# MichaelVorndran/InconsistencyMasks

Hardware: AMD Instinct MI355X
Metric: images/sec per IM generation (ensemble infer + IM build + 1 train epoch), 256x256 (higher is better)
Workload: dtype f16; 1 GPU; ISIC-2018 binary 256x256x3, 2-model IM ensemble, tiny U-Net alpha=0.5 on MI355X (configs[1]); outputs=1, unlabeled_images=2335, unlabeled_images_per_gpu=2335, labeled_images=259, n_models=2, infer_batch=584, infer_batch_rule=functions.infer_batch_size: 584 at alpha<=0.5 else 128; short tail spread, train_batch_per_gpu=32, global_batch=32, parallelism=dp1, epoch_steps=80, kept=2307, train_images=2566

## Files before the change

include/imk.h:

```cpp
#ifndef IMK_H
#define IMK_H

#include <stddef.h>
#include <stdint.h>

#ifdef __cplusplus
extern "C" {
#endif

#define IMK_VERSION 100

#define IMK_API __attribute__((visibility("default")))

enum {
    IMK_OK = 0,
    IMK_EINVAL = -1,
    IMK_EUNSUPPORTED = -2,
    IMK_EWORKSPACE = -3,
};

IMK_API int imk_version(void);
IMK_API const char *imk_error_string(int code);


IMK_API int imk_im_binary(const float *preds, int n_models, int batch, int h, int w, int kb,
                  float thr, int cmp_ge,
                  const uint8_t *img, int c, int block_in, int block_out,
                  uint8_t *img_out, uint8_t *masks_out, uint8_t *im_out,
                  int64_t *im_size, int64_t *pred_size, void *stream);

IMK_API int imk_im_multiclass(const float *probs, int n_models, int batch, int h, int w, int k,
                      const uint8_t *img, int c, int block_in, int block_out,
                      uint8_t *img_out, uint8_t *final_out, uint8_t *im_out,
                      int64_t *im_size, uint8_t *presence, void *stream);

IMK_API int imk_morph(const uint8_t *src, uint8_t *dst, int batch, int h, int w, int ksize, int op, void *stream);

IMK_API int imk_block_apply(const uint8_t *im, uint8_t *img, int c, uint8_t *masks, int n_masks,
                    int batch, int h, int w, void *stream);

enum { IMK_VOTE_HARD = 0, IMK_VOTE_SOFT = 1 };
IMK_API int imk_vote_binary(const float *preds, int n_models, int batch, int h, int w, int kb, double thr, int mode,
                    uint8_t *masks_out, void *stream);

IMK_API int imk_vote_multiclass(const float *probs, int n_models, int batch, int h, int w, int k, int mode,
                        uint8_t *final_out, void *stream);


typedef struct imk_unet_cfg {
    int h, w;
    int c_in;
    int n_out;
    int ch[5];
    int act_out;
} imk_unet_cfg;

typedef struct imk_unet_plan imk_unet_plan;

typedef struct imk_evalnet_cfg {
    int h, w;
    int ca, cb;
    int n_out;
    int two_heads;
    int normalize_a, normalize_b;
    int ch[5];
    int b_onehot;
} imk_evalnet_cfg;

IMK_API int imk_unet_plan_create(const imk_unet_cfg *cfg, imk_unet_plan **out);
IMK_API void imk_unet_plan_destroy(imk_unet_plan *plan);

IMK_API int imk_unet_param_count(const imk_unet_plan *plan, int64_t *total, int64_t *trainable);

typedef struct imk_layer_info {
    char name[16];
    int kind;
    int ksize, cin, cout;
    int64_t off_w, off_b;
    int64_t off_mean, off_var;
} imk_layer_info;
IMK_API int imk_unet_num_layers(const imk_unet_plan *plan);
IMK_API int imk_unet_layer_info(const imk_unet_plan *plan, int idx, imk_layer_info *out);

IMK_API int64_t imk_unet_packed_bytes(const imk_unet_plan *plan);
IMK_API int imk_unet_pack_weights(const imk_unet_plan *plan, const float *params, void *packed, void *stream);

IMK_API int64_t imk_unet_workspace_bytes(const imk_unet_plan *plan, int batch, int mode);

IMK_API int imk_unet_forward(const imk_unet_plan *plan, const float *params, const void *packed,
                     const uint8_t *x, int batch, float *probs, void *workspace, int64_t workspace_bytes,
                     void *stream);

IMK_API int imk_unet_tensor_info(const imk_unet_plan *plan, int batch, int mode, int layer_idx, int which,
                         int64_t *byte_offset, int *h, int *w, int *c, int *c_stride);

IMK_API int64_t imk_unet_forward_im_workspace_bytes(const imk_unet_plan *plan, int n_models, int batch, int n_streams);
IMK_API int imk_unet_forward_im(const imk_unet_plan *plan, int n_models,
                        const float *const *params, const void *const *packed,
                        const uint8_t *x, int batch, float thr, int cmp_ge,
                        const uint8_t *img, int block_in, int block_out,
                        uint8_t *img_out, uint8_t *masks_out, uint8_t *im_out,
                        int64_t *im_size, int64_t *pred_size, uint8_t *presence,
                        void *workspace, int64_t workspace_bytes, void *stream);

IMK_API int imk_unet_forward_vote(const imk_unet_plan *plan, int n_models,
                          const float *const *params, const void *const *packed,
                          const uint8_t *x, int batch, double thr, int mode, uint8_t *masks_out,
                          void *workspace, int64_t workspace_bytes, void *stream);

IMK_API int64_t imk_unet_state_bytes(const imk_unet_plan *plan);
IMK_API int imk_unet_state_init(const imk_unet_plan *plan, void *state, void *stream);
IMK_API int imk_unet_fwd_bwd(const imk_unet_plan *plan, float *params, void *packed, void *state,
                     const uint8_t *x, const uint8_t *y, int batch, int loss_kind,
                     float *grads, float *stats, void *workspace, int64_t workspace_bytes, void *stream);

IMK_API int imk_unet_adamw_step(const imk_unet_plan *plan, float *params, void *packed, void *state,
                        const float *grads, const float *stats, float grad_scale,
                        float lr, float wd, float beta1, float beta2, float eps, void *stream);

IMK_API int64_t imk_unet_consistency_workspace_bytes(const imk_unet_plan *plan, int batch);
IMK_API int imk_unet_consistency_fwd_bwd(const imk_unet_plan *plan, float *params, void *packed, void *state,
                                 const uint8_t *x1, const uint8_t *x2, int batch,
                                 float *grads, float *stats, void *workspace, int64_t workspace_bytes, void *stream);

typedef struct imk_aug_params {
    int flip_v, flip_h;
    int rot;
    int bright_on;
    float alpha, beta;
    int blur_k;
    int noise_max;
    uint32_t seed;
} imk_aug_params;

IMK_API int imk_gather_pairs(const uint8_t *img, int64_t row_img, const uint8_t *mask, int planes, int64_t hw, int div255,
                             const uint8_t *mul, const int64_t *idx, int64_t n, uint8_t *img_out, uint8_t *mask_out,
                             void *stream);

IMK_API int imk_augment(const uint8_t *img, const uint8_t *mask, int batch, int h, int w, int c, int cm,
                const imk_aug_params *params, uint8_t *img_out, uint8_t *mask_out, int any_quarter_turn, void *stream);

#define IMK_VIEWS_MAX 16
typedef struct imk_view_params {
    int op;
    int blur_k;
    int noise_max;
    uint32_t seed;
    int bright_on;
    float alpha, beta;
} imk_view_params;

IMK_API int imk_views(const uint8_t *img, int batch, int h, int w, int c, int n_views, const imk_view_params *params,
                      int chain, int any_quarter_turn, uint8_t *views_out, void *stream);

IMK_API int imk_vote_views_binary(const float *preds, int n_views, int batch, int h, int w, int k, const int *ops,
                                  int any_quarter_turn, double thr, int cmp_ge, uint8_t *masks_out, void *stream);

IMK_API int imk_vote_views_majority(const float *probs, int n_views, int batch, int h, int w, int k, uint8_t *final_out,
                                    void *stream);

enum { IMK_VOTE_MAJORITY = 2 };
IMK_API int64_t imk_unet_forward_views_vote_workspace_bytes(const imk_unet_plan *plan, int n_views, int batch);
IMK_API int imk_unet_forward_views_vote(const imk_unet_plan *plan, const float *params, const void *packed,
                                        const uint8_t *views, int n_views, int batch, const int *ops, int any_quarter_turn,
                                        double thr, int mode, int cmp_ge, uint8_t *masks_out, void *workspace,
                                        int64_t workspace_bytes, void *stream);

IMK_API int64_t imk_unet_forward_student_workspace_bytes(const imk_unet_plan *plan, int batch);
IMK_API int imk_unet_forward_student(const imk_unet_plan *plan, const float *params, const void *packed, const uint8_t *x,
                                     const uint8_t *img, int batch, float thr, int cmp_ge, const imk_aug_params *aug,
                                     int any_quarter_turn, uint8_t *img_out, uint8_t *labels_out, void *workspace,
                                     int64_t workspace_bytes, void *stream);

IMK_API int imk_eval_binary(const float *probs, float thr, int cmp_ge, const uint8_t *gt, int batch, int h, int w,
                    uint8_t *pred_out, int64_t *counts, void *stream);

IMK_API int imk_eval_multiclass(const float *probs, const uint8_t *gt, int batch, int h, int w, int k, uint8_t *pred_out,
                        int64_t *counts, void *stream);

IMK_API int64_t imk_eval_soft_out_doubles(int k);
IMK_API int imk_eval_soft_sums(const float *probs, const uint8_t *gt, int64_t n_pix, int k, int mode, double *out, void *stream);

IMK_API int64_t imk_im_depth_workspace_bytes(int batch, int h, int w);
IMK_API int imk_im_depth(const float *preds, int n_models, int batch, int h, int w, float mult, const uint8_t *img, int c,
                         int block_in, uint8_t *img_out, uint8_t *im_out, int64_t *im_size, float *thr_out, float *std_out,
                         void *workspace, int64_t workspace_bytes, void *stream);

IMK_API int64_t imk_unet_forward_im_depth_workspace_bytes(const imk_unet_plan *plan, int n_models, int batch, int n_streams);
IMK_API int imk_unet_forward_im_depth(const imk_unet_plan *plan, int n_models, const float *const *params,
                                      const void *const *packed, const uint8_t *x, int batch, float mult, const uint8_t *img,
                                      int block_in, uint8_t *img_out, uint8_t *im_out, int64_t *im_size, float *thr_out,
                                      float *std_out, void *workspace, int64_t workspace_bytes, void *stream);

IMK_API int imk_eval_depth(const float *probs, const uint8_t *gt, int batch, int h, int w, uint8_t *pred_out, double *sums,
                           void *stream);

IMK_API int imk_evalnet_plan_create(const imk_evalnet_cfg *cfg, imk_unet_plan **out);
IMK_API int64_t imk_evalnet_workspace_bytes(const imk_unet_plan *plan, int batch, int mode );

IMK_API int imk_evalnet_forward(const imk_unet_plan *plan, const float *params, const void *packed, const uint8_t *xa,
                        const uint8_t *xb, int batch, float *out, void *workspace, int64_t workspace_bytes, void *stream);

IMK_API int imk_evalnet_fwd_bwd(const imk_unet_plan *plan, float *params, void *packed, void *state, const uint8_t *xa,
                        const uint8_t *xb, const float *y, int batch, float *out, float *grads, float *stats,
                        void *workspace, int64_t workspace_bytes, void *stream);

IMK_API int imk_evalnet_tensor_info(const imk_unet_plan *plan, int batch, int mode, int layer_idx, int which,
                            int64_t *byte_offset, int *h, int *w, int *c, int *c_stride);

#define IMK_SELECT_MAX_CAND 16
#define IMK_SELECT_MAX_MODELS 8
enum { IMK_SELECT_IOU = 0, IMK_SELECT_MIOU = 1, IMK_SELECT_CONF_GATED = 2 };

IMK_API int imk_evalnet_select(const float *scores, int n_models, int batch, int n_cand, int n_heads, int n_out,
                               const int32_t *counts, const uint8_t *cand, int64_t cand_bytes, double thr, int mode,
                               int32_t *best_idx, float *best_score, uint8_t *keep, uint8_t *out, void *stream);

IMK_API int64_t imk_evalnet_forward_candidates_workspace_bytes(const imk_unet_plan *plan, int batch, int n_cand);
IMK_API int imk_evalnet_forward_candidates(const imk_unet_plan *plan, int n_models, const float *const *params,
                                           const void *const *packed, const uint8_t *xa, const uint8_t *xb, int batch, int n_cand,
                                           float *scores, void *workspace, int64_t workspace_bytes, void *stream);

IMK_API int imk_evalnet_forward_select(const imk_unet_plan *plan, int n_models, const float *const *params,
                                       const void *const *packed, const uint8_t *xa, const uint8_t *xb, int batch, int n_cand,
                                       const int32_t *counts, const uint8_t *cand, int64_t cand_bytes, double thr, int mode,
                                       float *scores, int32_t *best_idx, float *best_score, uint8_t *keep, uint8_t *out,
                                       void *workspace, int64_t workspace_bytes, void *stream);

IMK_API int imk_unet_plan_set_bn_momentum(imk_unet_plan *plan, float momentum);
IMK_API int imk_unet_plan_get_bn_momentum(const imk_unet_plan *plan, float *momentum);

IMK_API int imk_unet_plan_debug(imk_unet_plan *plan, int materialize, int single_stream);

IMK_API int imk_png_info(const char *path, int *h, int *w, int *color_type, int *bit_depth);
IMK_API int imk_png_read_file(const char *path, int want_c, uint8_t *out, int64_t out_cap, int *h_out, int *w_out);
IMK_API int imk_png_decode(const uint8_t *data, int64_t len, int want_c, uint8_t *out, int64_t out_cap, int *h_out, int *w_out);
IMK_API int imk_png_encode(const uint8_t *pixels, int h, int w, int c, int level, uint8_t *out, int64_t out_cap, int64_t *out_len);
IMK_API int imk_png_write_file(const char *path, const uint8_t *pixels, int h, int w, int c, int level);
// ... 42 lines not shown
```

inconsistencymasks_amd/_lib.py:

```python
import ctypes
import os

PKG = os.path.dirname(os.path.abspath(__file__))
LIB_PATH = os.environ.get("IMK_LIB_PATH", os.path.join(PKG, "libimk.so"))

c_int, c_float, c_void_p, c_int64 = ctypes.c_int, ctypes.c_float, ctypes.c_void_p, ctypes.c_int64


class UnetCfg(ctypes.Structure):
    _fields_ = [("h", c_int), ("w", c_int), ("c_in", c_int), ("n_out", c_int),
                ("ch", c_int * 5), ("act_out", c_int)]


class EvalnetCfg(ctypes.Structure):
    _fields_ = [("h", c_int), ("w", c_int), ("ca", c_int), ("cb", c_int), ("n_out", c_int), ("two_heads", c_int),
                ("normalize_a", c_int), ("normalize_b", c_int), ("ch", c_int * 5), ("b_onehot", c_int)]


class AugParams(ctypes.Structure):
    _fields_ = [("flip_v", c_int), ("flip_h", c_int), ("rot", c_int), ("bright_on", c_int), ("alpha", c_float),
                ("beta", c_float), ("blur_k", c_int), ("noise_max", c_int), ("seed", ctypes.c_uint32)]


class ViewParams(ctypes.Structure):
    _fields_ = [("op", c_int), ("blur_k", c_int), ("noise_max", c_int), ("seed", ctypes.c_uint32), ("bright_on", c_int),
                ("alpha", c_float), ("beta", c_float)]


class PrepItem(ctypes.Structure):
    _fields_ = [("src_off", c_int64), ("src_h", c_int), ("src_w", c_int), ("x0", c_int), ("y0", c_int), ("cw", c_int),
                ("ch", c_int), ("scale_x", ctypes.c_double), ("scale_y", ctypes.c_double)]


class LayerInfo(ctypes.Structure):
    _fields_ = [("name", ctypes.c_char * 16), ("kind", c_int), ("ksize", c_int), ("cin", c_int), ("cout", c_int),
                ("off_w", c_int64), ("off_b", c_int64), ("off_mean", c_int64), ("off_var", c_int64)]


SIGNATURES = {
    "imk_version": (c_int, []),
    "imk_error_string": (ctypes.c_char_p, [c_int]),
    "imk_im_binary": (c_int, [c_void_p, c_int, c_int, c_int, c_int, c_int, c_float, c_int,
                              c_void_p, c_int, c_int, c_int, c_void_p, c_void_p, c_void_p,
                              c_void_p, c_void_p, c_void_p]),
    "imk_im_multiclass": (c_int, [c_void_p, c_int, c_int, c_int, c_int, c_int,
                                  c_void_p, c_int, c_int, c_int, c_void_p, c_void_p, c_void_p,
                                  c_void_p, c_void_p, c_void_p]),
    "imk_morph": (c_int, [c_void_p, c_void_p, c_int, c_int, c_int, c_int, c_int, c_void_p]),
    "imk_block_apply": (c_int, [c_void_p, c_void_p, c_int, c_void_p, c_int, c_int, c_int, c_int, c_void_p]),
    "imk_unet_plan_create": (c_int, [ctypes.POINTER(UnetCfg), ctypes.POINTER(c_void_p)]),
    "imk_unet_plan_destroy": (None, [c_void_p]),
    "imk_unet_param_count": (c_int, [c_void_p, ctypes.POINTER(c_int64), ctypes.POINTER(c_int64)]),
    "imk_unet_num_layers": (c_int, [c_void_p]),
    "imk_unet_layer_info": (c_int, [c_void_p, c_int, ctypes.POINTER(LayerInfo)]),
    "imk_unet_packed_bytes": (c_int64, [c_void_p]),
    "imk_unet_pack_weights": (c_int, [c_void_p, c_void_p, c_void_p, c_void_p]),
    "imk_unet_workspace_bytes": (c_int64, [c_void_p, c_int, c_int]),
    "imk_unet_forward": (c_int, [c_void_p, c_void_p, c_void_p, c_void_p, c_int, c_void_p, c_void_p, c_int64, c_void_p]),
    "imk_unet_tensor_info": (c_int, [c_void_p, c_int, c_int, c_int, c_int, ctypes.POINTER(c_int64),
                                     ctypes.POINTER(c_int), ctypes.POINTER(c_int), ctypes.POINTER(c_int),
                                     ctypes.POINTER(c_int)]),
    "imk_unet_forward_im_workspace_bytes": (c_int64, [c_void_p, c_int, c_int, c_int]),
    "imk_unet_forward_im": (c_int, [c_void_p, c_int, ctypes.POINTER(c_void_p), ctypes.POINTER(c_void_p),
                                    c_void_p, c_int, c_float, c_int, c_void_p, c_int, c_int,
                                    c_void_p, c_void_p, c_void_p, c_void_p, c_void_p, c_void_p,
                                    c_void_p, c_int64, c_void_p]),
    "imk_vote_binary": (c_int, [c_void_p, c_int, c_int, c_int, c_int, c_int, ctypes.c_double, c_int, c_void_p, c_void_p]),
    "imk_vote_multiclass": (c_int, [c_void_p, c_int, c_int, c_int, c_int, c_int, c_int, c_void_p, c_void_p]),
    "imk_unet_forward_vote": (c_int, [c_void_p, c_int, ctypes.POINTER(c_void_p), ctypes.POINTER(c_void_p),
                                      c_void_p, c_int, ctypes.c_double, c_int, c_void_p, c_void_p, c_int64, c_void_p]),
    "imk_views": (c_int, [c_void_p, c_int, c_int, c_int, c_int, c_int, c_void_p, c_int, c_int, c_void_p, c_void_p]),
    "imk_vote_views_binary": (c_int, [c_void_p, c_int, c_int, c_int, c_int, c_int, c_void_p, c_int, ctypes.c_double, c_int,
                                      c_void_p, c_void_p]),
    "imk_vote_views_majority": (c_int, [c_void_p, c_int, c_int, c_int, c_int, c_int, c_void_p, c_void_p]),
    "imk_unet_forward_views_vote_workspace_bytes": (c_int64, [c_void_p, c_int, c_int]),
    "imk_unet_forward_views_vote": (c_int, [c_void_p, c_void_p, c_void_p, c_void_p, c_int, c_int, c_void_p, c_int,
                                            ctypes.c_double, c_int, c_int, c_void_p, c_void_p, c_int64, c_void_p]),
    "imk_unet_forward_student_workspace_bytes": (c_int64, [c_void_p, c_int]),
    "imk_unet_forward_student": (c_int, [c_void_p, c_void_p, c_void_p, c_void_p, c_void_p, c_int, c_float, c_int, c_void_p, c_int,
                                         c_void_p, c_void_p, c_void_p, c_int64, c_void_p]),
    "imk_unet_state_bytes": (c_int64, [c_void_p]),
    "imk_unet_state_init": (c_int, [c_void_p, c_void_p, c_void_p]),
    "imk_unet_fwd_bwd": (c_int, [c_void_p, c_void_p, c_void_p, c_void_p, c_void_p, c_void_p, c_int, c_int,
                                 c_void_p, c_void_p, c_void_p, c_int64, c_void_p]),
    "imk_unet_consistency_workspace_bytes": (c_int64, [c_void_p, c_int]),
    "imk_unet_consistency_fwd_bwd": (c_int, [c_void_p, c_void_p, c_void_p, c_void_p, c_void_p, c_void_p, c_int,
                                             c_void_p, c_void_p, c_void_p, c_int64, c_void_p]),
    "imk_evalnet_plan_create": (c_int, [ctypes.POINTER(EvalnetCfg), ctypes.POINTER(c_void_p)]),
    "imk_evalnet_workspace_bytes": (c_int64, [c_void_p, c_int, c_int]),
    "imk_evalnet_forward": (c_int, [c_void_p, c_void_p, c_void_p, c_void_p, c_void_p, c_int, c_void_p, c_void_p, c_int64,
                                    c_void_p]),
    "imk_evalnet_tensor_info": (c_int, [c_void_p, c_int, c_int, c_int, c_int, ctypes.POINTER(c_int64),
                                        ctypes.POINTER(c_int), ctypes.POINTER(c_int), ctypes.POINTER(c_int),
                                        ctypes.POINTER(c_int)]),
    "imk_evalnet_fwd_bwd": (c_int, [c_void_p, c_void_p, c_void_p, c_void_p, c_void_p, c_void_p, c_void_p, c_int, c_void_p,
                                    c_void_p, c_void_p, c_void_p, c_int64, c_void_p]),
    "imk_evalnet_select": (c_int, [c_void_p, c_int, c_int, c_int, c_int, c_int, c_void_p, c_void_p, c_int64, ctypes.c_double, c_int,
                                   c_void_p, c_void_p, c_void_p, c_void_p, c_void_p]),
    "imk_evalnet_forward_candidates_workspace_bytes": (c_int64, [c_void_p, c_int, c_int]),
    "imk_evalnet_forward_candidates": (c_int, [c_void_p, c_int, ctypes.POINTER(c_void_p), ctypes.POINTER(c_void_p), c_void_p, c_void_p,
                                               c_int, c_int, c_void_p, c_void_p, c_int64, c_void_p]),
    "imk_evalnet_forward_select": (c_int, [c_void_p, c_int, ctypes.POINTER(c_void_p), ctypes.POINTER(c_void_p), c_void_p, c_void_p,
                                           c_int, c_int, c_void_p, c_void_p, c_int64, ctypes.c_double, c_int, c_void_p, c_void_p,
                                           c_void_p, c_void_p, c_void_p, c_void_p, c_int64, c_void_p]),
    "imk_gather_pairs": (c_int, [c_void_p, c_int64, c_void_p, c_int, c_int64, c_int, c_void_p, c_void_p, c_int64, c_void_p, c_void_p, c_void_p]),
    "imk_augment": (c_int, [c_void_p, c_void_p, c_int, c_int, c_int, c_int, c_int, c_void_p, c_void_p, c_void_p, c_int, c_void_p]),
    "imk_eval_binary": (c_int, [c_void_p, c_float, c_int, c_void_p, c_int, c_int, c_int, c_void_p, c_void_p, c_void_p]),
    "imk_eval_multiclass": (c_int, [c_void_p, c_void_p, c_int, c_int, c_int, c_int, c_void_p, c_void_p, c_void_p]),
    "imk_eval_soft_out_doubles": (c_int64, [c_int]),
    "imk_eval_soft_sums": (c_int, [c_void_p, c_void_p, c_int64, c_int, c_int, c_void_p, c_void_p]),
    "imk_im_depth_workspace_bytes": (c_int64, [c_int, c_int, c_int]),
    "imk_im_depth": (c_int, [c_void_p, c_int, c_int, c_int, c_int, c_float, c_void_p, c_int, c_int, c_void_p, c_void_p, c_void_p,
                             c_void_p, c_void_p, c_void_p, c_int64, c_void_p]),
    "imk_unet_forward_im_depth_workspace_bytes": (c_int64, [c_void_p, c_int, c_int, c_int]),
    "imk_unet_forward_im_depth": (c_int, [c_void_p, c_int, ctypes.POINTER(c_void_p), ctypes.POINTER(c_void_p), c_void_p, c_int, c_float,
                                          c_void_p, c_int, c_void_p, c_void_p, c_void_p, c_void_p, c_void_p, c_void_p, c_int64, c_void_p]),
    "imk_eval_depth": (c_int, [c_void_p, c_void_p, c_int, c_int, c_int, c_void_p, c_void_p, c_void_p]),
    "imk_unet_plan_debug": (c_int, [c_void_p, c_int, c_int]),
    "imk_unet_plan_set_bn_momentum": (c_int, [c_void_p, c_float]),
    "imk_unet_plan_get_bn_momentum": (c_int, [c_void_p, ctypes.POINTER(c_float)]),
    "imk_prof_create": (c_int, [c_int, ctypes.POINTER(c_void_p)]),
    "imk_prof_destroy": (None, [c_void_p]),
    "imk_prof_bind": (c_int, [c_void_p]),
    "imk_prof_unbind": (c_int, [c_void_p]),
    "imk_prof_totals_enable": (c_int, [c_void_p, c_int]),
    "imk_prof_totals_dump": (c_int64, [c_void_p, ctypes.c_char_p, c_int64]),
    "imk_prof_mark": (c_int, [c_int, c_void_p]),
    "imk_runtime_warnings": (c_int, []),
    "imk_unet_plan_side_stream": (c_int, [c_void_p, c_int, ctypes.POINTER(c_void_p)]),
    "imk_prof_set_period": (c_int, [c_void_p, c_int]),
    "imk_prof_collect": (c_int, [c_void_p, ctypes.POINTER(c_int64), ctypes.POINTER(ctypes.c_double), ctypes.POINTER(ctypes.c_double),
                                 ctypes.POINTER(ctypes.c_double)]),
    "imk_png_info": (c_int, [ctypes.c_char_p, ctypes.POINTER(c_int), ctypes.POINTER(c_int), ctypes.POINTER(c_int), ctypes.POINTER(c_int)]),
    "imk_png_read_file": (c_int, [ctypes.c_char_p, c_int, c_void_p, c_int64, ctypes.POINTER(c_int), ctypes.POINTER(c_int)]),
    "imk_png_decode": (c_int, [c_void_p, c_int64, c_int, c_void_p, c_int64, ctypes.POINTER(c_int), ctypes.POINTER(c_int)]),
    "imk_png_encode": (c_int, [c_void_p, c_int, c_int, c_int, c_int, c_void_p, c_int64, ctypes.POINTER(c_int64)]),
    "imk_png_write_file": (c_int, [ctypes.c_char_p, c_void_p, c_int, c_int, c_int, c_int]),
    "imk_pos_contours": (c_int, [c_void_p, c_int, c_int, c_int, c_void_p, c_int]),
    "imk_mod_pos_size": (c_int, [c_void_p, c_int, c_int, c_int, c_int, c_int, c_int, c_void_p]),
    "imk_cell_count": (c_int, [c_void_p, c_int, c_void_p, c_void_p, c_int, c_int, c_int, c_void_p]),
    "imk_prep_resize": (c_int, [c_void_p, c_int64, c_void_p, c_int, c_int, c_int, c_int, c_int, c_int, c_void_p, c_void_p]),
    "imk_prep_crops": (c_int, [c_void_p, c_int, c_int, c_int, c_void_p, c_int, c_int, c_int, c_int, c_void_p, c_int, c_void_p,
                               c_void_p]),
    "imk_unet_adamw_step": (c_int, [c_void_p, c_void_p, c_void_p, c_void_p, c_void_p, c_void_p, c_float,
                                    c_float, c_float, c_float, c_float, c_float, c_void_p]),
}


def _load():
    if not os.path.exists(LIB_PATH):
        raise RuntimeError(
            f"{LIB_PATH} is missing: build it with `python -c 'import __graft_entry__ as g; g.build()'` "
            "(hipcc --offload-arch=gfx950).  There is no CPU fallback for the product path.")
    import torch
    lib = ctypes.CDLL(LIB_PATH)
    for name, (res, args) in SIGNATURES.items():
        fn = getattr(lib, name)
        fn.restype = res
        fn.argtypes = args
    return lib


lib = _load()


class ImkError(RuntimeError):
    pass


def check(code, what=""):
    if code != 0:
        msg = lib.imk_error_string(code)
        raise ImkError(f"{what}: imk error {code} ({msg.decode() if msg else '?'})")
```

inconsistencymasks_amd/csrc/imk_conv.hip:

```cpp
#include <cstdlib>
#include "imk_kernels.h"
#include "imk_elem.h"

#include "imk_stage.h"
#include "imk_switches.h"

#ifndef IMK_INF_WAVES
#define IMK_INF_WAVES 4
#endif
IMK_STAMP_TABLE(conv)
IMK_WGSTAMP_TABLE(conv)

namespace {


struct ImkConvGeom { int tiles_x, tiles_y, mt_total, nc8, nc8p, n_pass, ps, nsp; unsigned magic_tx, magic_pi; };
__host__ __device__ inline size_t imk_chain_w2_offset(size_t stage1_bytes, size_t out_bytes) {
    return ((stage1_bytes > out_bytes ? stage1_bytes : out_bytes) + 15) & ~(size_t)15;
}

template <int TH, int MT, int LM, bool CHAIN = false>
__device__ __forceinline__ void conv_mfma_body(const ImkConvArgs &a, const ImkConvGeom &gm, int bx, int by) {
    const int tiles_x = gm.tiles_x, tiles_y = gm.tiles_y, mt_total = gm.mt_total, nc8 = gm.nc8, nc8p = gm.nc8p;
    const int n_pass = gm.n_pass, ps = gm.ps, nsp = gm.nsp;
// ... 1288 lines not shown
    for (int j = 0; j < 8; ++j) { bsum[j] = 0.f; acc[0][j] = acc[1][j] = acc[2][j] = acc[3][j] = 0.f; }
    const float inv = 1.0f / u8_div;
    const long long stride = (long long)gridDim.x * 256;
    struct Px { f16x8 d, zz; uint32_t xb; };
    auto load = [&](long long p, Px &q) {
        q.d = *reinterpret_cast<const f16x8 *>(dy + p * 8);
        q.zz = *reinterpret_cast<const f16x8 *>(z + p * 8);
        typedef uint32_t __attribute__((aligned(1))) u32_unaligned;
        const long long rem = (n_pix - p) * cin;
        const int back = rem >= 4 ? 0 : (int)(4 - rem);
        const uint32_t v = *reinterpret_cast<const u32_unaligned *>(x + p * cin - back) >> (8 * back);
        q.xb = cin >= 4 ? v : (v & ((1u << (8 * cin)) - 1u));
    };
    auto use = [&](const Px &q) {
        float xf[4];
#pragma unroll
        for (int c = 0; c < 4; ++c) xf[c] = (float)(f16)((float)((q.xb >> (8 * c)) & 0xffu) * inv);
#pragma unroll
        for (int j = 0; j < 8; ++j) {
            const float zf = (float)q.zz[j];
            const float g = zf > 0.f ? (float)(f16)(A[j] * (float)q.d[j] + Bc[j] * zf + Cc[j]) : 0.f;
            bsum[j] += g;
#pragma unroll
            for (int c = 0; c < 4; ++c) acc[c][j] += xf[c] * g;
        }
    };
    long long p = (long long)blockIdx.x * 256 + t;
    if (p < n_pix) {
        Px cur, nxt;
        load(p, cur);
        while (true) {
            const long long pn = p + stride;
            const bool more = pn < n_pix;
            load(more ? pn : p, nxt);
            use(cur);
            if (!more) break;
            cur = nxt;
            p = pn;
        }
    }
#pragma unroll
    for (int c = 0; c < 4; ++c)
#pragma unroll
        for (int j = 0; j < 8; ++j) {
            const float v = wave_sum<64>(acc[c][j]);
            if (lane == 0) s_red[wave][c * 8 + j] = v;
        }
#pragma unroll
    for (int j = 0; j < 8; ++j) {
        const float v = wave_sum<64>(bsum[j]);
        if (lane == 0) s_red[wave][32 + j] = v;
    }
    __syncthreads();
    auto tot = [&](int i) { return (s_red[0][i] + s_red[1][i]) + (s_red[2][i] + s_red[3][i]); };
    float *row = partial + (size_t)blockIdx.x * 2 * 256;
    const int r = t >> 6, l = t & 63, ci = 4 * (l >> 4) + r, co = l & 15;
    row[t] = (ci < 4 && co < 8) ? tot(ci * 8 + co) : 0.f;
    row[256 + t] = t < 8 ? tot(32 + t) : 0.f;
}

__device__ __forceinline__ int wgf_find_job(const ImkWgFinalJobs &jobs, int idx, bool stage1) {
    int j = 0;
    for (int k = 1; k < jobs.n; ++k) {
        const int begin = stage1 ? jobs.j[k].work1_begin : jobs.j[k].tile_begin;
        if (idx >= begin) j = k;
    }
    return j;
}

__global__ __launch_bounds__(256) void wgf_stage1_kernel(ImkWgFinalJobs jobs) {
    IMK_STAMP_BEGIN(conv, 21);
    __shared__ float4 s_q[4][64];
    const int jn = wgf_find_job(jobs, blockIdx.x, true);
    const ImkWgFinalJob &jb = jobs.j[jn];
    const int local = blockIdx.x - jb.work1_begin;
    const int tile = local / jb.n_chunks, chunk = local - tile * jb.n_chunks;
    const int t = threadIdx.x, e4 = t & 63, sg = t >> 6;
    const int s0 = chunk * jb.chunk, s1 = min(jb.n_split, s0 + jb.chunk);
    const size_t stride4 = (size_t)jb.n_tiles * 64;
    const float4 *p = reinterpret_cast<const float4 *>(jb.partial) + (size_t)tile * 64 + e4;
    float4 acc = {0.f, 0.f, 0.f, 0.f};
    for (int sb = s0; sb < s1; sb += WG_RED_CHUNK) {
        float4 v[WG_RED_CHUNK / 4];
#pragma unroll
        for (int i = 0; i < WG_RED_CHUNK / 4; ++i) v[i] = p[(size_t)min(sb + sg + 4 * i, s1 - 1) * stride4];
#pragma unroll
        for (int i = 0; i < WG_RED_CHUNK / 4; ++i) {
            const float live = (sb + sg + 4 * i < s1) ? 1.f : 0.f;
            acc.x += live * v[i].x; acc.y += live * v[i].y; acc.z += live * v[i].z; acc.w += live * v[i].w;
        }
    }
    s_q[sg][e4] = acc;
    __syncthreads();
    if (sg == 0) {
        const float4 a = s_q[0][e4], b = s_q[1][e4], c = s_q[2][e4], d = s_q[3][e4];
        float4 r;
        r.x = (a.x + b.x) + (c.x + d.x); r.y = (a.y + b.y) + (c.y + d.y); r.z = (a.z + b.z) + (c.z + d.z); r.w = (a.w + b.w) + (c.w + d.w);
        reinterpret_cast<float4 *>(jb.red)[((size_t)chunk * jb.n_tiles + tile) * 64 + e4] = r;
    }
    IMK_STAMP_END(1);
}

template <int N>
__device__ __forceinline__ float wgf_sum_chunks(const float *p, size_t stride, int sg, int n_chunks) {
    float v[N];
#pragma unroll
    for (int i = 0; i < N; ++i) v[i] = p[(size_t)min(sg + 4 * i, n_chunks - 1) * stride];
    float acc = 0.f;
#pragma unroll
    for (int i = 0; i < N; ++i) acc += (sg + 4 * i < n_chunks) ? v[i] : 0.f;
    return acc;
}

__global__ __launch_bounds__(1024) void wgf_stage2_kernel(ImkWgFinalJobs jobs, const float *__restrict__ inv_scale_ptr,
                                                          float *__restrict__ found_inf) {
    __shared__ float s_p[4][256];
    const int jn = wgf_find_job(jobs, blockIdx.x, false);
    const ImkWgFinalJob &jb = jobs.j[jn];
    const int tile = blockIdx.x - jb.tile_begin;
    const int e = threadIdx.x & 255, sg = threadIdx.x >> 8;
    const size_t stride = (size_t)jb.n_tiles * 256;
    const float *p = jb.red + (size_t)tile * 256 + e;
    const int per = (jb.n_chunks + 3) >> 2;
    float acc;
    if (per <= 1) acc = wgf_sum_chunks<1>(p, stride, sg, jb.n_chunks);
    else if (per <= 2) acc = wgf_sum_chunks<2>(p, stride, sg, jb.n_chunks);
    else if (per <= 4) acc = wgf_sum_chunks<4>(p, stride, sg, jb.n_chunks);
    else if (per <= 8) acc = wgf_sum_chunks<8>(p, stride, sg, jb.n_chunks);
    else acc = wgf_sum_chunks<16>(p, stride, sg, jb.n_chunks);
    s_p[sg][e] = acc;
    __syncthreads();
    if (sg != 0) return;
    float s = ((s_p[0][e] + s_p[1][e]) + (s_p[2][e] + s_p[3][e])) * *inv_scale_ptr;
    const int pair = tile / (jb.T + 1), tap = tile - pair * (jb.T + 1);
    const int cit = pair / jb.cot_n, cot = pair - cit * jb.cot_n;
    const int r = e >> 6, lane = e & 63;
    const int m = 4 * (lane >> 4) + r, nn = lane & 15;
    const int ci = cit * 16 + m, co = cot * 16 + nn;
    if (tap < jb.T) {
        if (ci < jb.cin && co < jb.cout) {
            if (!isfinite(s)) *found_inf = 1.0f;
            jb.dw[((size_t)tap * jb.cin + ci) * jb.cout + co] = s;
        }
    } else if (cit == 0 && m == 0 && co < jb.cout) {
        if (!isfinite(s)) *found_inf = 1.0f;
        jb.db[co] = s;
    }
}

__global__ __launch_bounds__(256) void pack_conv_batched_kernel(ImkPackJobs jobs) {
    IMK_STAMP_BEGIN(conv, 23);
    if (jobs.ctl && blockIdx.x == 0 && blockIdx.y == 0 && threadIdx.x == 0) imk_ctl_end_step(jobs.ctl, jobs.stats);
    const ImkPackJob &jb = jobs.j[blockIdx.y];
    if (jb.transposed == 2) {
        for (int i = blockIdx.x * 256 + threadIdx.x; i < 512; i += gridDim.x * 256) {
            const int j = i & 7, lane = (i >> 3) & 63;
            const int m = lane & 15, g = lane >> 4;
            float v = 0.f;
            if (!jb.pair) {
                const int ci = 4 * g + j;
                if (j < 4 && ci < jb.cin && m < jb.cout) v = jb.w[(size_t)ci * jb.cout + m];
            } else {
                const int ci = 4 * (g & 1) + j, co = m & 7;
                if (j < 4 && (m >> 3) == (g >> 1) && ci < jb.cin && co < jb.cout) v = jb.w[(size_t)ci * jb.cout + co];
            }
            jb.dst[i] = (f16)v;
        }
        return;
    }
    const int T = jb.ksize == 3 ? 9 : 1;
    const int m_dim = jb.transposed ? jb.cin : jb.cout, k_dim = jb.transposed ? jb.cout : jb.cin;
    if (jb.pair && T == 9) {
        const int nc8 = ((k_dim + 7) & ~7) / 8;
        const int ns = 3 * nc8;
        for (int i = blockIdx.x * 256 + threadIdx.x; i < ns * 512; i += gridDim.x * 256) {
            const int j = i & 7, lane = (i >> 3) & 63, st = i >> 9;
            const int m = lane & 15, g = lane >> 4;
            const int q = 4 * st + g;
            const int ut = q / nc8, c8 = q - ut * nc8;
            const int r = ut / 3, c = ut - 3 * r, ky = r - (m >> 3);
            const int mi = m & 7, ki = c8 * 8 + j;
            float v = 0.f;
            if (ky >= 0 && ky <= 2 && mi < m_dim && ki < k_dim) {
                const int tap = ky * 3 + c;
                if (!jb.transposed) v = jb.w[((size_t)tap * jb.cin + ki) * jb.cout + mi];
                else v = jb.w[((size_t)(T - 1 - tap) * jb.cin + mi) * jb.cout + ki];
            }
            jb.dst[i] = (f16)v;
        }
        return;
    }
    if (jb.pair) {
        const int nc8 = ((k_dim + 7) & ~7) / 8;
        const int nq = T * nc8, ns = (nq + 1) / 2;
        for (int i = blockIdx.x * 256 + threadIdx.x; i < ns * 512; i += gridDim.x * 256) {
            const int j = i & 7, lane = (i >> 3) & 63, st = i >> 9;
            const int m = lane & 15, g = lane >> 4;
            const int q = 2 * st + (g & 1);
            const int tap = q / nc8, c8 = q - tap * nc8;
            const int mi = m & 7, ki = c8 * 8 + j;
            float v = 0.f;
            if (q < nq && (m >> 3) == (g >> 1) && mi < m_dim && ki < k_dim) {
                if (!jb.transposed) v = jb.w[((size_t)tap * jb.cin + ki) * jb.cout + mi];
                else v = jb.w[((size_t)(T - 1 - tap) * jb.cin + mi) * jb.cout + ki];
            }
            jb.dst[i] = (f16)v;
        }
        return;
    }
    const int nc8 = ((k_dim + 7) & ~7) / 8;
    const int nc8p = imk_pass_chunks(nc8), nsp = (T * nc8p + 3) / 4;
    const int ns = imk_cdiv_d(nc8, nc8p) * nsp;
    const int total = ((m_dim + 15) / 16) * ns * 512;
    for (int i = blockIdx.x * 256 + threadIdx.x; i < total; i += gridDim.x * 256) {
        const int j = i & 7, lane = (i >> 3) & 63;
        const int cs = i >> 9;
        const int s = cs % ns, ct = cs / ns;
        const int m = lane & 15, g = lane >> 4;
        const int pass = s / nsp, q = 4 * (s - pass * nsp) + g;
        const int tap = q / nc8p, c8 = pass * nc8p + (q - tap * nc8p);
        const int mi = ct * 16 + m, ki = c8 < nc8 ? c8 * 8 + j : k_dim;
        float v = 0.f;
        if (tap < T && mi < m_dim && ki < k_dim) {
            if (!jb.transposed) v = jb.w[((size_t)tap * jb.cin + ki) * jb.cout + mi];
            else v = jb.w[((size_t)(T - 1 - tap) * jb.cin + mi) * jb.cout + ki];
        }
        jb.dst[i] = (f16)v;
    }
    IMK_STAMP_END(1);
}

}

int imk_wgf_add_job(ImkWgFinalJobs &jobs, float *partial, int n_split, int ksize, int cin, int cout, float *dw, float *db) {
    if (jobs.n >= IMK_WGF_MAX_JOBS) return IMK_EUNSUPPORTED;
    const int T = ksize == 3 ? 9 : 1;
    const int cit_n = (imk_pad8(cin) + 15) / 16, cot_n = (imk_pad8(cout) + 15) / 16;
    ImkWgFinalJob &jb = jobs.j[jobs.n++];
    jb.partial = partial;
    jb.n_split = n_split;
    jb.chunk = WG_RED_CHUNK;
    while (imk_cdiv(n_split, jb.chunk) > 64) jb.chunk *= 2;
    jb.n_chunks = imk_cdiv(n_split, jb.chunk);
    jb.n_tiles = cit_n * cot_n * (T + 1);
    jb.red = partial + (size_t)n_split * jb.n_tiles * 256;
    jb.T = T; jb.cin = cin; jb.cout = cout; jb.cot_n = cot_n;
    jb.dw = dw; jb.db = db;
    jb.work1_begin = jobs.total_work1;
    jb.tile_begin = jobs.total_tiles;
    jobs.total_work1 += jb.n_tiles * jb.n_chunks;
    jobs.total_tiles += jb.n_tiles;
    return IMK_OK;
}

int imk_launch_wgrad_finalize_jobs(const ImkWgFinalJobs &jobs, const float *inv_scale_ptr, float *found_inf, hipStream_t stream) {
    if (jobs.n <= 0) return IMK_OK;
    double wgf_bytes = 0;
    for (int i = 0; i < jobs.n; ++i)
        wgf_bytes += ((double)jobs.j[i].n_split + 2.0 * jobs.j[i].n_chunks + 1.0) * jobs.j[i].n_tiles * 256 * 4;
    ImkProfScope prof(PF_WGF, wgf_bytes, stream);
    double b1 = 0, b2 = 0;
    for (int i = 0; i < jobs.n; ++i) {
        b1 += ((double)jobs.j[i].n_split + jobs.j[i].n_chunks) * jobs.j[i].n_tiles * 256 * 4;
        b2 += ((double)jobs.j[i].n_chunks + 1.0) * jobs.j[i].n_tiles * 256 * 4;
    }
    imk_prof_work(b1);
    imk_klaunch(wgf_stage1_kernel, dim3(jobs.total_work1), dim3(256), 0, stream, jobs);
    IMK_LAUNCH_CHECK();
    imk_prof_work(b2);
    imk_klaunch(wgf_stage2_kernel, dim3(jobs.total_tiles), dim3(1024), 0, stream, jobs, inv_scale_ptr, found_inf);
    IMK_LAUNCH_CHECK();
    return IMK_OK;
}

int imk_launch_pack_jobs(const ImkPackJobs &jobs, hipStream_t stream) {
    if (jobs.n <= 0) return IMK_OK;
    double pk_bytes = 0;
    for (int i = 0; i < jobs.n; ++i) pk_bytes += (double)jobs.j[i].ksize * jobs.j[i].ksize * jobs.j[i].cin * jobs.j[i].cout * 6;
    ImkProfScope prof(PF_STEP_TAIL, pk_bytes, stream);
    long long widest = 0;
    for (int i = 0; i < jobs.n; ++i) {
        const long long slots = (long long)jobs.j[i].ksize * jobs.j[i].ksize * ((jobs.j[i].cin + 15) & ~15) * ((jobs.j[i].cout + 15) & ~15);
        widest = slots > widest ? slots : widest;
    }
    int bpj = (int)((widest + 2047) / 2048);
    bpj = bpj < 64 ? 64 : (bpj > 1024 ? 1024 : bpj);
    imk_klaunch(pack_conv_batched_kernel, dim3(dim3(bpj, jobs.n)), dim3(256), 0, stream, jobs);
    IMK_LAUNCH_CHECK();
    return IMK_OK;
}

static inline int odd_ps(int nc8) { return imk_lds_pitch(nc8); }

static inline int conv_tile_h(int cs_in, int ksize) {
    const int halo = ksize == 3 ? 1 : 0;
    const size_t b16 = (size_t)(16 + 2 * halo) * (TW + 2 * halo) * odd_ps(imk_pass_chunks(cs_in / 8)) * 16;
    return b16 > 64 * 1024 ? 8 : 16;
}

int imk_conv_num_tiles(int B, int H, int W, int cs_in, int ksize) {
    const int per_tile = B * imk_cdiv(H, conv_tile_h(cs_in, ksize)) * imk_cdiv(W, TW);
    const int gemm = imk_conv_gemm_num_tiles(B, H, W);
    return per_tile > gemm ? per_tile : gemm;
}

#include <algorithm>
#include <cstdio>
#include <cstring>
#include <cxxabi.h>
#include <map>
#include <mutex>
#include <new>
#include <string>
#include <unordered_map>
#include <vector>
namespace {
struct ProfRec { hipEvent_t e0, e1; int variant; double bytes, flops; };
struct ProfTot { long long launches = 0; double bytes = 0, flops = 0; };
const char *const kFamilyNames[PF_COUNT] = {
    "conv_mfma_kernel<16, 1>", "conv_mfma_kernel<16, 2>", "conv_mfma_kernel<16, 4>", "conv_mfma_kernel<8, 1>", "conv_mfma_kernel<8, 2>",
    "conv_mfma_kernel<8, 4>", "conv_pipe_kernel", "wgrad_mfma_kernel", "bn_bwd_prep_kernel", "bn_bwd_coef_kernel", "bn_finalize_kernel",
    "wgf_stage1+2_kernel", "head_kernel", "head_loss_kernel", "step_tail", "im_kernel", "conv_gemm_kernel", "wgrad_gemm_kernel"};
__global__ void imk_mark_kernel(int id) { (void)id; }
}
struct imk_prof {
    int period = 0;
    long counter = 0;
    std::vector<ProfRec> recs;
    std::vector<hipEvent_t> pool;
    bool totals_on = false;
    std::map<std::string, ProfTot> totals;
    hipEvent_t event() {
        if (!pool.empty()) { hipEvent_t e = pool.back(); pool.pop_back(); return e; }
        hipEvent_t e;
        (void)hipEventCreate(&e);
        return e;
    }
};
static thread_local imk_prof *t_prof = nullptr;

extern "C" int imk_prof_create(int period, imk_prof **out) {
    IMK_CHECK_ARG(out && period >= 0);
    imk_prof *p = new (std::nothrow) imk_prof();
    if (!p) return IMK_EINVAL;
    p->period = period;
    *out = p;
    return IMK_OK;
}
extern "C" void imk_prof_destroy(imk_prof *p) {
    if (!p) return;
    if (t_prof == p) { t_prof = nullptr; imk_tls_totals_on = false; }
    for (auto &r : p->recs) { (void)hipEventDestroy(r.e0); (void)hipEventDestroy(r.e1); }
    for (auto e : p->pool) (void)hipEventDestroy(e);
    delete p;
}
extern "C" int imk_prof_bind(imk_prof *p) { t_prof = p; imk_tls_totals_on = p && p->totals_on; return IMK_OK; }
extern "C" int imk_prof_unbind(imk_prof *p) { if (p && t_prof == p) { t_prof = nullptr; imk_tls_totals_on = false; return 1; } return 0; }
extern "C" int imk_prof_set_period(imk_prof *p, int period) { IMK_CHECK_ARG(p && period >= 0); p->period = period; return IMK_OK; }

static const std::string &kernel_short_name(const void *kern, hipStream_t stream) {
    static std::mutex mu;
    static std::unordered_map<const void *, std::string> names;
    std::lock_guard<std::mutex> lk(mu);
    auto it = names.find(kern);
    if (it != names.end()) return it->second;
    std::string n = "?";
    if (const char *m = hipKernelNameRefByPtr(kern, stream)) {
        int st = 0;
        char *d = abi::__cxa_demangle(m, nullptr, nullptr, &st);
        n = (st == 0 && d) ? d : m;
        free(d);
        if (st != 0) {
            const char *tag = "_ZN12_GLOBAL__N_1";
            const size_t at = n.find(tag);
            if (at != std::string::npos) {
                size_t i = at + strlen(tag), len = 0;
                while (i < n.size() && n[i] >= '0' && n[i] <= '9') len = 10 * len + (size_t)(n[i++] - '0');
                if (len > 0 && i + len <= n.size()) n = n.substr(i, len);
            }
        }
        for (const char *drop : {"void ", "(anonymous namespace)::"})
            for (size_t at; (at = n.find(drop)) != std::string::npos;) n.erase(at, strlen(drop));
        int depth = 0;
        for (size_t i = 0; i < n.size(); ++i) {
            if (n[i] == '<') ++depth;
            else if (n[i] == '>') --depth;
            else if (n[i] == '(' && depth == 0) { n.resize(i); break; }
        }
        if (n.size() > 90) n.resize(90);
    }
    return names.emplace(kern, n).first->second;
}
static thread_local struct { double bytes, flops; bool armed; } t_work = {0.0, 0.0, false};
void imk_prof_work(double bytes, double flops) { t_work.bytes = bytes; t_work.flops = flops; t_work.armed = true; }
void imk_prof_note_launch(const void *kern, hipStream_t stream) {
    imk_prof *p = t_prof;
    if (!p || !p->totals_on) return;
    ProfTot &t = p->totals[kernel_short_name(kern, stream)];
    t.launches += 1;
    if (t_work.armed) { t.bytes += t_work.bytes; t.flops += t_work.flops; t_work.armed = false; }
}

int imk_prof_begin(int family, double bytes, hipStream_t stream, double flops, const char *variant) {
    imk_prof *p = t_prof;
    (void)variant;
    if (p && p->totals_on && family >= 0 && family < PF_COUNT) imk_prof_work(bytes, flops);
    if (!p || p->period <= 0 || (p->counter++ % p->period) != 0) return -1;
    ProfRec pr{p->event(), p->event(), family, bytes, flops};
    if (hipEventRecord(pr.e0, stream) != hipSuccess) { p->pool.push_back(pr.e0); p->pool.push_back(pr.e1); return -1; }
    p->recs.push_back(pr);
    return (int)p->recs.size() - 1;
}
void imk_prof_end(int slot, hipStream_t stream) {
    imk_prof *p = t_prof;
    if (p && slot >= 0 && slot < (int)p->recs.size()) (void)hipEventRecord(p->recs[slot].e1, stream);
}

extern "C" int imk_prof_totals_enable(imk_prof *p, int on) {
    IMK_CHECK_ARG(p);
    p->totals.clear();
    p->totals_on = on != 0;
    if (t_prof == p) imk_tls_totals_on = p->totals_on;
    t_work.armed = false;
    return IMK_OK;
}
// ... 381 lines not shown
    if ((sw.gemm_over_chain == 2 || (sw.gemm_over_chain == 1 && store_mid)) && imk_conv_gemm_ok(plain)) return false;
    if (pipe_choice(a).ok || a.epi != EP_RELU || a.ksize != 3 || a.cout > 64 || cout2 > 64) return false;
    if (a.x.lmode != LM_POOL && a.x.lmode != LM_AFFINE) return false;
    const bool wide = a.x.cs_in <= 32 && a.cout <= 32 && a.x.lmode != LM_POOL;
    const bool wide_chain = sw.wide_chain_train && wide && a.x.lmode == LM_AFFINE && a.x.cs_in >= 16 && cout2 <= a.cout && pipe_fits(a);
    if (sw.conv_chain_tile == 1 && wide && store_mid && !wide_chain && (long long)a.B * imk_cdiv(a.H, 16) * imk_cdiv(a.W, TW) > 2048)
        return false;
    const int mt1 = (a.cout + 15) / 16, mt2 = (cout2 + 15) / 16, mt = (mt1 <= 2 && mt2 <= 2) ? 2 : 4;
    return mt1 <= mt && mt2 <= mt && conv_tile_h(a.x.cs_in, 3) == 16;
}

bool imk_conv_can_fuse_wgrad(const ImkConvArgs &a) {
    const PipeChoice p = pipe_choice(a);
    if (!p.ok || a.wpk2) return false;
    const bool form1 = a.ksize == 1 && a.x.lmode == LM_BNBWD && a.epi == EP_MASK && a.mask && !(a.dystat_z && a.stats_partial);
    const bool form2 = a.x.lmode == LM_RAW && a.epi == EP_PLAIN && a.dystat_z && a.stats_partial;
    if (!form1 && !form2) return false;
    const bool all_ch = p.pair ? a.cs_out == 8 : a.cs_out == 16;
    return (a.H % 16 == 0) && (a.W % TW == 0) && all_ch;
}
int imk_conv_fused_wgrad_rows_max() { return 256 * 8; }

bool imk_conv_can_sum2(const ImkConvArgs &a) {
    const PipeChoice p = pipe_choice(a);
    if (!p.ok || a.wpk2 || a.wg_partial) return false;
    if (a.ksize != 1 || a.x.lmode != LM_BNBWD || a.epi != EP_PLAIN || (a.dystat_z && a.stats_partial)) return false;
    const bool all_ch = p.pair ? a.cs_out == 8 : a.cs_out == 16;
    return (a.H % 16 == 0) && (a.W % TW == 0) && all_ch;
}

int imk_launch_conv(const ImkConvArgs &a_in, hipStream_t stream) {
    ImkConvArgs a = a_in;
    IMK_CHECK_ARG(a.x.in && a.wpk && (a.out || a.wpk2) && a.B > 0 && a.H > 0 && a.W > 0);
    IMK_CHECK_ARG(a.ksize == 1 || a.ksize == 3);
    IMK_CHECK_ARG(a.x.cs_in % 8 == 0 && a.cs_out % 8 == 0 && a.x.cs_in >= a.x.cin && a.cs_out >= a.cout);
    IMK_CHECK_ARG(a.x.lmode != LM_U8 || (a.x.cs_in == 8 && a.x.cin <= 8));
    if (a.x.cs_in > 512) return IMK_EUNSUPPORTED;
    const PipeChoice p = pipe_choice(a);
    a.pair = p.pair;
    if (a.pre_wpk && !(p.ok && a.wpk2 && a.pre_bias && a.pre_sc && a.pre_sh && a.pre_cout > 0)) return IMK_EUNSUPPORTED;
    if (a.wpk2 && a.pair && a.cout2 > 8) return IMK_EUNSUPPORTED;
    if (a.wpk2) {
        if (a.epi != EP_RELU || !a.out2 || !a.bias2 || a.cs_out2 % 8) return IMK_EUNSUPPORTED;
        if (p.ok) return a.cout2 > 16 ? IMK_EUNSUPPORTED : launch_conv_pipe_any(a, stream);
        if (!imk_conv_can_chain_tile(a, a.cout2, a.out != nullptr)) return IMK_EUNSUPPORTED;
        if (conv_wide_chain_ok(a)) return launch_conv_wide_chain(a, stream);
        if (imk_conv_gemm_chain_ok(a)) return imk_launch_conv_gemm(a, stream);
        return launch_conv_mfma(a, stream);
    }
    if (p.ok) return launch_conv_pipe_any(a, stream);
    if (a.x.lmode == LM_STEM) return IMK_EUNSUPPORTED;
    if (conv_wide_ok(a)) return launch_conv_wide_any(a, stream);
    if (imk_conv_gemm_ok(a)) return imk_launch_conv_gemm(a, stream);
    return launch_conv_mfma(a, stream);
}

int imk_wgrad_splits(int B, int H, int W, int cin, int cout) {
    const int n_tiles = B * imk_cdiv(H, 16) * imk_cdiv(W, TW);
    const int n_pairs = ((imk_pad8(cin) + 15) / 16) * ((imk_pad8(cout) + 15) / 16);
    constexpr int target = 768;
    int s = target / n_pairs;
    if (s < 1) s = 1;
    if (s > n_tiles) s = n_tiles;
    return s;
}

size_t imk_wgrad_partial_floats(int B, int H, int W, int ksize, int cin, int cout) {
    const int n_pairs = ((imk_pad8(cin) + 15) / 16) * ((imk_pad8(cout) + 15) / 16);
    const int T = ksize == 3 ? 9 : 1;
    size_t ns = (size_t)imk_wgrad_splits(B, H, W, cin, cout);
    if (imk_pad8(cin) <= 16 && imk_pad8(cout) <= 16 && ns < (size_t)imk_conv_fused_wgrad_rows_max())
        ns = (size_t)imk_conv_fused_wgrad_rows_max();
    if (imk_wgrad_gemm_wide(imk_pad8(cin), imk_pad8(cout), (long long)B * H * W)) {
        for (int lm : {(int)LM_RAW, (int)LM_POOL, (int)LM_AFFINE}) {
            const size_t ng = (size_t)imk_wgrad_gemm_splits(lm, B, H, W, ksize, imk_pad8(cin), imk_pad8(cout));
            if (ns < ng) ns = ng;
        }
    }
    if (ksize == 1 && imk_pad8(cin) >= 24 && imk_pad8(cin) <= 64 && imk_pad8(cout) >= 24 && imk_pad8(cout) <= 64 &&
        ns < (size_t)imk_bwd1x1_rows((long long)B * H * W, imk_pad8(cin), imk_pad8(cout)))
        ns = (size_t)imk_bwd1x1_rows((long long)B * H * W, imk_pad8(cin), imk_pad8(cout));
    if (ksize == 1 && n_pairs <= 8 && ns < (size_t)imk_loss_blocks((long long)B * H * W)) ns = (size_t)imk_loss_blocks((long long)B * H * W);
    return (ns + (ns + WG_RED_CHUNK - 1) / WG_RED_CHUNK) * n_pairs * (T + 1) * 256;
}

struct WgradLaunch { ImkWgradGeom gm; int gx, gy; size_t lds; };

static int plan_wgrad(const ImkWgradArgs &a, WgradLaunch &L) {
    IMK_CHECK_ARG(a.x.in && a.dA && a.partial && a.B > 0 && a.H > 0 && a.W > 0 && a.n_split > 0);
    IMK_CHECK_ARG(a.ksize == 1 || a.ksize == 3);
    IMK_CHECK_ARG(a.x.cs_in % 8 == 0 && a.cs_out % 8 == 0);
    if (a.x.lmode == LM_BNBWD) return IMK_EUNSUPPORTED;
    if (a.x.lmode == LM_U8 && a.x.cin > 4) return IMK_EUNSUPPORTED;
    const int cit_n = (a.x.cs_in + 15) / 16, cot_n = (a.cs_out + 15) / 16;
    const int tiles_x = imk_cdiv(a.W, TW), tiles_y = imk_cdiv(a.H, 16);
    size_t lds = ((size_t)18 * 18 + 256) * WG_STRIDE_H * sizeof(f16) + (4 * (size_t)a.x.cs_in + 3 * (size_t)a.cs_out) * sizeof(float);
    const size_t red = 4 * (size_t)(a.ksize == 3 ? 10 : 2) * 256 * sizeof(float);
    if (lds < red) lds = red;
    L.gm = ImkWgradGeom{tiles_x, tiles_y, a.B * tiles_x * tiles_y, cit_n, cot_n, a.x.cs_in / 8, a.cs_out / 8, ImkWalk{}};
    L.gx = a.n_split; L.gy = cit_n * cot_n; L.lds = lds;
    {
        int g = a.n_split;
        L.gm.wk = imk_walk_make(g, L.gm.n_tiles, tiles_x * tiles_y);
        if (g != a.n_split) { g = a.n_split; L.gm.wk = ImkWalk{L.gm.n_tiles, 0, g, 0, 0}; }
    }
    return IMK_OK;
}

static double wgrad_algorithmic_bytes(const ImkWgradArgs &a, const WgradLaunch &L) {
    const double px = (double)a.B * a.H * a.W;
    double in_b;
    switch (a.x.lmode) {
        case LM_POOL: in_b = 4.0 * px * a.x.cs_in * 2; break;
        case LM_UPADD: in_b = 1.25 * px * a.x.cs_in * 2; break;
        case LM_U8: in_b = px * a.x.cin; break;
        default: in_b = px * a.x.cs_in * 2;
    }
    const int T = a.ksize == 3 ? 9 : 1;
    return in_b + px * a.cs_out * 2 * (a.dA_z ? 2 : 1) + (double)L.gx * L.gy * (T + 1) * 256 * 4;
}

int imk_launch_wgrad(const ImkWgradArgs &a, hipStream_t stream) {
    if (a.x.lmode == LM_U8 && a.ksize == 1 && a.dA_z && a.dA_coef && a.cs_out == 8 && a.x.cin <= 4 && a.n_split >= 1) {
        const long long n_pix = (long long)a.B * a.H * a.W;
        ImkProfScope prof(PF_WGRAD, (double)n_pix * (a.x.cin + 32) + (double)a.n_split * 2 * 1024, stream, imk_wgrad_flops(a));
        imk_klaunch(stem_wgrad_kernel, dim3(a.n_split), dim3(256), 0, stream, reinterpret_cast<const uint8_t *>(a.x.in), a.x.cin, a.x.u8_div, a.dA, a.dA_z, a.dA_coef,
                                                        n_pix, a.partial);
        IMK_LAUNCH_CHECK();
        return IMK_OK;
    }
    if (imk_wgrad_gemm_ok(a.x.lmode, a.dA_z != nullptr, a.ksize, a.x.cs_in, a.cs_out, (long long)a.B * a.H * a.W)) return imk_launch_wgrad_gemm(a, stream);
    WgradLaunch L{};
    int rc = plan_wgrad(a, L);
    if (rc) return rc;
    const dim3 grid(L.gx, L.gy);
    ImkProfScope prof(PF_WGRAD, wgrad_algorithmic_bytes(a, L), stream, imk_wgrad_flops(a));
    switch (a.x.lmode) {
#define IMK_WG(LM) do { if (a.ksize == 3) { if (a.dA_z) imk_klaunch(wgrad_mfma_kernel<LM, true, true>, dim3(grid), dim3(256), L.lds, stream, a, L.gm); \
                                           else imk_klaunch(wgrad_mfma_kernel<LM, false, true>, dim3(grid), dim3(256), L.lds, stream, a, L.gm); } \
                        else { if (a.dA_z) imk_klaunch(wgrad_mfma_kernel<LM, true, false>, dim3(grid), dim3(256), L.lds, stream, a, L.gm); \
                               else imk_klaunch(wgrad_mfma_kernel<LM, false, false>, dim3(grid), dim3(256), L.lds, stream, a, L.gm); } } while (0)
        case LM_RAW: IMK_WG(LM_RAW); break;
        case LM_AFFINE: IMK_WG(LM_AFFINE); break;
        case LM_POOL: IMK_WG(LM_POOL); break;
        case LM_UPADD: IMK_WG(LM_UPADD); break;
        default: IMK_WG(LM_U8); break;
#undef IMK_WG
    }
    IMK_LAUNCH_CHECK();
    return IMK_OK;
}

size_t imk_packed_conv_halfs(int ksize, int cin, int cout, int transposed, bool pair) {
    if (transposed == 2) return 512;
    const int T = ksize == 3 ? 9 : 1;
    const int m_dim = transposed ? cin : cout, k_dim = transposed ? cout : cin;
    const int nc8 = imk_pad8(k_dim) / 8;
    if (pair) return (size_t)(T == 9 ? 3 * nc8 : (nc8 + 1) / 2) * 512;
    const int nc8p = imk_pass_chunks(nc8);
    const int ns = imk_cdiv_d(nc8, nc8p) * ((T * nc8p + 3) / 4);
    return (size_t)((m_dim + 15) / 16) * ns * 512;
}
```

inconsistencymasks_amd/csrc/imk_elem.h:

```cpp
#pragma once
#include "imk_common.h"

struct ImkCtl {
    float loss_scale;
    float inv_loss_scale;
    int good_steps;
    int step;
    float found_inf;
    float pad[3];
};

int imk_launch_bn_finalize(const float *partial, int n_part, int c, int cs, double count, const float *gamma,
                           const float *beta, float *mov_mean, float *mov_var, float *scale, float *shift,
                           float *save_mean, float *save_invstd, hipStream_t stream, float momentum = 0.99f);
int imk_bn_prep_blocks(int B, int H, int W, int cs);
int imk_launch_bn_bwd_prep(int mode, const f16 *g_direct, const f16 *g_other, const f16 *z, const float *sc,
                           const float *sh, f16 *dy_out, float *partial, int B, int H, int W, int cs, hipStream_t stream,
                           int g_other_cs = 0);
int imk_launch_bn_bwd_coef(const float *partial, int n_part, int c, int cs, double count, const float *gamma,
                           const float *save_mean, const float *save_invstd, const float *inv_scale_ptr, float *coef,
                           float *dgamma, float *dbeta, float *found_inf, hipStream_t stream);
int imk_launch_head(const f16 *z, const float *sc, const float *sh, const float *w, const float *bias, int cin, int cs,
                    int K, int softmax, long long n_pix, float *probs, hipStream_t stream);
int imk_loss_blocks(long long n_pix);
int imk_launch_head_loss(const f16 *z, const float *sc, const float *sh, const float *w, const float *bias, int cin, int cs,
                         int K, int softmax, long long n_pix, const uint8_t *y, const ImkCtl *ctl, float *stats,
                         f16 *dlogit, float *loss_partial, hipStream_t stream, int y255 = 0);
bool imk_head_cce_fused_ok(int cs, int K, long long n_pix, int rows_cap);
int imk_head_cce_fused_rows(long long n_pix);
int imk_launch_head_cce_fused(const f16 *z, const float *sc, const float *sh, const float *w, const float *bias, int cin, int cs,
                              int K, long long n_pix, const uint8_t *y, const ImkCtl *ctl, float *stats, f16 *dy,
                              float *loss_partial, float *dystat_partial, float *wg_partial, hipStream_t stream);
bool imk_head_mse_fused_ok(int cs, int K, long long n_pix, int rows_cap);
int imk_launch_head_mse_fused(const f16 *z, const float *sc, const float *sh, const float *w, const float *bias, int cin, int cs,
                              int K, long long n_pix, const uint8_t *y, const ImkCtl *ctl, float *stats, f16 *dy,
                              float *loss_partial, float *dystat_partial, float *wg_partial, hipStream_t stream, int y255 = 0);
int imk_launch_rmse_scale(const float *loss_partial, long long n_pix, int K, float *grads, long long n_grads, float *stats,
                          hipStream_t stream);
int imk_launch_loss_finalize(const float *loss_partial, long long n_pix, int K, int kind, float *stats, hipStream_t stream);
bool imk_consistency_fused_ok(int cs, int K, int softmax, long long n_pix, int rows_cap);
int imk_launch_consistency_head(const f16 *zA, const f16 *zB, const float *scA, const float *shA, const float *scB,
                                const float *shB, const float *w, const float *bias, int cin, int cs, int K, long long n_pix,
                                const ImkCtl *ctl, float *stats, f16 *dyA, f16 *dyB, float *loss_partial, float *dystatA,
                                float *dystatB, float *wg_partial, hipStream_t stream);
int imk_launch_consistency_dlogit(const float *pA, const float *pB, int K, int softmax, long long n_pix, const ImkCtl *ctl,
                                  float *stats, f16 *dlogitA, f16 *dlogitB, float *loss_partial, hipStream_t stream);
int imk_launch_grad_add(float *g, const float *g2, long long n, float *found_inf, hipStream_t stream);
int imk_launch_ctl_init(ImkCtl *ctl, hipStream_t stream);
int imk_launch_adamw(float *p, float *m, float *v, const float *g, long long n, ImkCtl *ctl, const float *stats,
                     float grad_scale, float lr, float wd, float b1, float b2, float eps, hipStream_t stream);

int imk_launch_concat_pool(const f16 *za, const float *sca, const float *sha, int csa, const f16 *zb, const float *scb,
                           const float *shb, int csb, int B, int Hh, int Wh, f16 *cat, hipStream_t stream, int a_div = 1);
int imk_launch_onehot(const uint8_t *cls, long long n_pix, int cs, f16 *out, hipStream_t stream);
size_t imk_evalnet_head_partial_floats(int B, int n_heads, int K, int C);
int imk_launch_evalnet_head(const f16 *z, const float *sc, const float *sh, const float *const *w, const float *const *bias,
                            int n_heads, int K, int C, int cs, int B, int H, int W, float *out, const float *y,
                            const ImkCtl *ctl, float *stats, f16 *dP, float *partial, hipStream_t stream);
int imk_launch_evalnet_head_reduce(const float *partial, int B, int n_heads, int K, int C, const float *inv_scale_ptr,
                                   float *dw0, float *db0, float *dw1, float *db1, float *found_inf, float *stats,
                                   hipStream_t stream);

__device__ __forceinline__ void imk_ctl_end_step(ImkCtl *ctl, const float *stats) {
    if (stats[1] != 0.f) {
        ctl->loss_scale = fmaxf(ctl->loss_scale * 0.5f, 1.0f);
        ctl->good_steps = 0;
    } else {
        ctl->step += 1;
        if (++ctl->good_steps >= 2000) { ctl->loss_scale *= 2.0f; ctl->good_steps = 0; }
    }
    ctl->inv_loss_scale = 1.0f / ctl->loss_scale;
}

#define IMK_FOLD_MAX_JOBS 32
struct ImkFoldJob { const float *gamma, *beta, *mean, *var; float *scale; int c, cs; };
struct ImkFoldJobs { ImkFoldJob j[IMK_FOLD_MAX_JOBS]; int n; };
int imk_launch_bn_fold_jobs(const ImkFoldJobs &jobs, hipStream_t stream);
```

inconsistencymasks_amd/csrc/imk_elem.hip:

```cpp
#include "imk_elem.h"
#include "imk_head.h"

IMK_STAMP_TABLE(elem)

namespace {

constexpr float BN_EPS = 1e-3f;

__device__ __forceinline__ void block_sum_rows(const float *__restrict__ partial, int n_part, int cs, int ch, int t,
                                               double &o1, double &o2) {
    double s1 = 0.0, s2 = 0.0;
    for (int i0 = t; i0 < n_part; i0 += 8 * 256) {
        float v1[8], v2[8];
#pragma unroll
        for (int u = 0; u < 8; ++u) {
            const int i = min(i0 + u * 256, n_part - 1);
            v1[u] = partial[(size_t)i * 2 * cs + ch];
            v2[u] = partial[(size_t)i * 2 * cs + cs + ch];
        }
#pragma unroll
        for (int u = 0; u < 8; ++u) {
            const double live = (i0 + u * 256 < n_part) ? 1.0 : 0.0;
            s1 += live * (double)v1[u];
            s2 += live * (double)v2[u];
// ... 303 lines not shown
    head_stage<CS>(w, bias, sc, sh, cin, K, s_w);
    __syncthreads();
    const long long p0 = (long long)blockIdx.x * 256;
    const long long p = p0 + threadIdx.x;
    float *row = s_out + threadIdx.x * pitch;
    if (p < n_pix) {
        float xin[CS];
        head_input<CS>(z, p, s_w, K, xin);
        if (!softmax) {
            for (int k = 0; k < K; ++k) row[k] = head_sigmoid(head_logit<CS>(xin, s_w, K, k));
        } else {
            head_softmax_row<CS>(xin, s_w, K, row);
        }
    }
    __syncthreads();
    const long long n_here = (n_pix - p0 < 256 ? n_pix - p0 : 256) * K;
    float *dst = probs + p0 * K;
    for (long long i = threadIdx.x; i < n_here; i += 256) {
        const int px = (int)(i / K), k = (int)(i - (long long)px * K);
        dst[i] = s_out[px * pitch + k];
    }
}

template <int CS, bool Y255 = false>
__global__ __launch_bounds__(256) void head_loss_kernel(const f16 *__restrict__ z, const float *__restrict__ sc,
                                                        const float *__restrict__ sh, const float *__restrict__ w,
                                                        const float *__restrict__ bias, int cin, int K, int softmax,
                                                        long long n_pix, const uint8_t *__restrict__ y,
                                                        const ImkCtl *__restrict__ ctl, float *__restrict__ stats,
                                                        int cs_out, f16 *__restrict__ dlogit,
                                                        float *__restrict__ loss_partial) {
    extern __shared__ float s_w[];
    float *s_b = s_w + K * CS, *s_sc = s_b + K, *s_sh = s_sc + CS, *s_rows = s_sh + CS;
    for (int i = threadIdx.x; i < K * CS; i += 256) {
        const int k = i / CS, c = i - k * CS;
        s_w[i] = (c < cin) ? w[(size_t)c * K + k] : 0.f;
    }
    for (int i = threadIdx.x; i < K; i += 256) s_b[i] = bias[i];
    for (int i = threadIdx.x; i < CS; i += 256) { s_sc[i] = sc[i]; s_sh[i] = sh[i]; }
    __syncthreads();
    const float S = ctl->loss_scale;
    if (blockIdx.x == 0 && threadIdx.x == 0) { stats[1] = 0.f; stats[2] = S; stats[3] = (float)ctl->step; }
    float l = 0.f;
    for (long long p = (long long)blockIdx.x * 256 + threadIdx.x; p < n_pix; p += (long long)gridDim.x * 256) {
        float xin[CS];
#pragma unroll
        for (int q = 0; q < CS / 8; ++q) {
            const f16x8 v = *reinterpret_cast<const f16x8 *>(z + p * CS + q * 8);
#pragma unroll
            for (int j = 0; j < 8; j += 2) {
                const f16x2 r2 = imk_affine2(f16x2{v[j], v[j + 1]}, f32x2{s_sc[q * 8 + j], s_sc[q * 8 + j + 1]}, f32x2{s_sh[q * 8 + j], s_sh[q * 8 + j + 1]});
                xin[q * 8 + j] = (float)r2[0]; xin[q * 8 + j + 1] = (float)r2[1];
            }
        }
        auto logit = [&](int k) {
            float acc = s_b[k];
#pragma unroll
            for (int c = 0; c < CS; ++c) acc += xin[c] * s_w[k * CS + c];
            return acc;
        };
        f16 *d = dlogit + p * cs_out;
        if (!softmax) {
            const float inv_n = 1.0f / ((float)n_pix * (float)K);
            for (int k0 = 0; k0 < cs_out; k0 += 8) {
                f16x8 g8 = {0, 0, 0, 0, 0, 0, 0, 0};
#pragma unroll
                for (int j = 0; j < 8; ++j) {
                    const int k = k0 + j;
                    if (k < K) {
                        float t = (float)y[p * K + k];
                        if constexpr (Y255) t = t / 255.0f;
                        const float pk = 1.0f / (1.0f + expf(-logit(k)));
                        const float e = pk - t;
                        l += e * e;
                        g8[j] = (f16)(S * 2.0f * e * inv_n * pk * (1.0f - pk));
                    }
                }
                *reinterpret_cast<f16x8 *>(d + k0) = g8;
            }
        } else {
            float *row = s_rows + threadIdx.x * (K | 1);
            float mx = -INFINITY;
            for (int k = 0; k < K; ++k) { const float lg = logit(k); row[k] = lg; mx = fmaxf(mx, lg); }
            float sum = 0.f;
            for (int k = 0; k < K; ++k) { const float e = expf(row[k] - mx); row[k] = e; sum += e; }
            const float inv = 1.0f / sum;
            const int t = y[p];
            const float inv_n = 1.0f / (float)n_pix;
            for (int k0 = 0; k0 < cs_out; k0 += 8) {
                f16x8 g8 = {0, 0, 0, 0, 0, 0, 0, 0};
#pragma unroll
                for (int j = 0; j < 8; ++j) {
                    const int k = k0 + j;
                    if (k < K) {
                        const float pk = row[k] * inv;
                        if (k == t) l += -logf(fmaxf(pk, 1.17549435e-38f));
                        g8[j] = (f16)(S * (pk - (k == t ? 1.0f : 0.0f)) * inv_n);
                    }
                }
                *reinterpret_cast<f16x8 *>(d + k0) = g8;
            }
        }
    }
    __shared__ float s_l[4];
    l = wave_sum<64>(l);
    if ((threadIdx.x & 63) == 0) s_l[threadIdx.x >> 6] = l;
    __syncthreads();
    if (threadIdx.x == 0) loss_partial[blockIdx.x] = (s_l[0] + s_l[1]) + (s_l[2] + s_l[3]);
}

__device__ __forceinline__ double loss_partials_sum(const float *__restrict__ partial, int n) {
    __shared__ double r[256];
    double s = 0;
    for (int i0 = threadIdx.x; i0 < n; i0 += 8 * 256) {
        float v[8];
#pragma unroll
        for (int u = 0; u < 8; ++u) v[u] = (i0 + u * 256 < n) ? partial[i0 + u * 256] : 0.f;
#pragma unroll
        for (int u = 0; u < 8; ++u) s += (double)v[u];
    }
    r[threadIdx.x] = s;
    __syncthreads();
    for (int o = 128; o > 0; o >>= 1) {
        if (threadIdx.x < o) r[threadIdx.x] += r[threadIdx.x + o];
        __syncthreads();
    }
    return r[0];
}

__global__ __launch_bounds__(256) void loss_finalize_kernel(const float *__restrict__ partial, int n, double denom,
                                                            float *__restrict__ stats) {
    const double tot = loss_partials_sum(partial, n);
    if (threadIdx.x == 0) stats[0] = (float)(tot / denom);
}

__global__ __launch_bounds__(256) void rmse_scale_kernel(const float *__restrict__ partial, int n, double denom,
                                                         float *__restrict__ grads, long long n_grads, float *__restrict__ stats) {
    const float mse = (float)(loss_partials_sum(partial, n) / denom);
    const float root = sqrtf(mse);
    const float s = 0.5f / root;
    for (long long i = (long long)blockIdx.x * 256 + threadIdx.x; i < n_grads; i += (long long)gridDim.x * 256) grads[i] *= s;
    if (blockIdx.x == 0 && threadIdx.x == 0) {
        stats[0] = root;
        if (!(mse > 0.f)) stats[1] = 1.0f;
    }
}

__global__ void ctl_init_kernel(ImkCtl *ctl) {
    ctl->loss_scale = 32768.0f;
    ctl->inv_loss_scale = 1.0f / 32768.0f;
    ctl->good_steps = 0;
    ctl->step = 0;
    ctl->found_inf = 0.f;
}

__global__ __launch_bounds__(256) void adamw_kernel(float *__restrict__ p, float *__restrict__ m, float *__restrict__ v,
                                                    const float *__restrict__ g, long long n, const ImkCtl *__restrict__ ctl,
                                                    const float *__restrict__ stats, float grad_scale, float lr, float wd,
                                                    float b1, float b2, float eps) {
    if (stats[1] != 0.f) return;
    const long long i = (long long)blockIdx.x * 256 + threadIdx.x;
    if (i >= n) return;
    const float t = (float)(ctl->step + 1);
    const float lr_t = lr * sqrtf(1.0f - powf(b2, t)) / (1.0f - powf(b1, t));
    const float gi = g[i] * grad_scale;
    float pi = p[i];
    pi -= wd * pi;
    const float mi = b1 * m[i] + (1.0f - b1) * gi;
    const float vi = b2 * v[i] + (1.0f - b2) * gi * gi;
    pi -= lr_t * mi / (sqrtf(vi) + eps);
    p[i] = pi; m[i] = mi; v[i] = vi;
}

__global__ __launch_bounds__(256) void concat_pool_kernel(const f16 *__restrict__ za, const float *__restrict__ sca,
                                                          const float *__restrict__ sha, int csa,
                                                          const f16 *__restrict__ zb, const float *__restrict__ scb,
                                                          const float *__restrict__ shb, int csb, int B, int Hh, int Wh,
                                                          f16 *__restrict__ cat, int a_div) {
    const int nc8 = (csa + csb) / 8;
    const long long n = (long long)B * Hh * Wh * nc8;
    const long long i = (long long)blockIdx.x * 256 + threadIdx.x;
    if (i >= n) return;
    const int c8 = (int)(i % nc8);
    const long long pix = i / nc8;
    const int x = (int)(pix % Wh);
    const long long r = pix / Wh;
    const int y = (int)(r % Hh), b = (int)(r / Hh);
    const bool second = c8 * 8 >= csa;
    const f16 *z = second ? zb : za;
    const int cs = second ? csb : csa, c0 = second ? c8 * 8 - csa : c8 * 8;
    const float *sc = (second ? scb : sca) + c0, *sh = (second ? shb : sha) + c0;
    const int W = 2 * Wh;
    const int bz = second ? b : b / a_div;
    const f16 *p = z + ((size_t)(bz * 2 * Hh + 2 * y) * W + 2 * x) * cs + c0;
    const f16x8 v0 = *reinterpret_cast<const f16x8 *>(p), v1 = *reinterpret_cast<const f16x8 *>(p + cs);
    const f16x8 v2 = *reinterpret_cast<const f16x8 *>(p + (size_t)W * cs), v3 = *reinterpret_cast<const f16x8 *>(p + (size_t)W * cs + cs);
    const f16x8 o = imk_affine_pool8(v0, v1, v2, v3, sc, sh);
    *reinterpret_cast<f16x8 *>(cat + (size_t)pix * (csa + csb) + c8 * 8) = o;
}

__global__ __launch_bounds__(256) void onehot_kernel(const uint8_t *__restrict__ cls, long long n_pix, int cs,
                                                     f16 *__restrict__ out) {
    const int nc8 = cs / 8;
    const long long i = (long long)blockIdx.x * 256 + threadIdx.x;
    if (i >= n_pix * nc8) return;
    const long long pix = i / nc8;
    const int c0 = (int)(i - pix * nc8) * 8, k = cls[pix];
    f16x8 o;
#pragma unroll
    for (int j = 0; j < 8; ++j) o[j] = (f16)(c0 + j == k ? 1.0f : 0.0f);
    *reinterpret_cast<f16x8 *>(out + pix * cs + c0) = o;
}

struct EvalHeadArgs {
    const f16 *z;
    const float *sc, *sh;
    const float *w[2], *bias[2];
    int n_heads, K, C, cs, B, H, W;
    float *out;
    const float *y;
    const ImkCtl *ctl;
    float *stats;
    f16 *dP;
    float *partial;
};

__global__ __launch_bounds__(256) void evalnet_head_kernel(EvalHeadArgs a) {
    extern __shared__ float s_f[];
    float *s_o = s_f + a.cs;
    const int b = blockIdx.x, t = threadIdx.x;
    const int Hh = a.H / 2, Wh = a.W / 2, NO = a.n_heads * a.K;
    const bool train = a.y != nullptr;
    if (train && b == 0 && t == 0) { a.stats[1] = 0.f; a.stats[2] = a.ctl->loss_scale; a.stats[3] = (float)a.ctl->step; }
    for (int c = t; c < a.cs; c += 256) {
        float acc = 0.f;
        if (c < a.C) {
            const float sc = a.sc[c], sh = a.sh[c];
            for (int y = 0; y < Hh; ++y)
                for (int x = 0; x < Wh; ++x) {
                    const f16 *p = a.z + ((size_t)(b * a.H + 2 * y) * a.W + 2 * x) * a.cs + c;
                    const float v0 = (float)imk_affine1(p[0], sc, sh), v1 = (float)imk_affine1(p[a.cs], sc, sh);
                    const float v2 = (float)imk_affine1(p[(size_t)a.W * a.cs], sc, sh), v3 = (float)imk_affine1(p[(size_t)a.W * a.cs + a.cs], sc, sh);
                    acc += fmaxf(fmaxf(v0, v1), fmaxf(v2, v3));
                }
            acc /= (float)(Hh * Wh);
        }
        s_f[c] = acc;
    }
    __syncthreads();
    for (int o = t >> 6; o < NO; o += 4) {
        const int h = o / a.K, k = o - h * a.K;
        float acc = 0.f;
        for (int c = t & 63; c < a.C; c += 64) acc += s_f[c] * a.w[h][(size_t)c * a.K + k];
        acc = wave_sum<64>(acc);
        if ((t & 63) == 0) s_o[o] = acc + a.bias[h][k];
    }
    __syncthreads();
    float loss_h[2] = {0.f, 0.f};
    if (t < NO) {
        const float lg = s_o[t], p = 1.0f / (1.0f + expf(-lg));
        a.out[(size_t)b * NO + t] = p;
        if (train) {
            const int h = t / a.K;
            const float yv = a.y[(size_t)b * NO + t], S = a.ctl->loss_scale, inv_n = 1.0f / ((float)a.B * (float)a.K);
            float g;
            if (h == 0) {
                const float e = p - yv;
                loss_h[0] = e * e;
                g = 2.0f * e * p * (1.0f - p);
            } else {
                loss_h[1] = fmaxf(lg, 0.f) - lg * yv + log1pf(expf(-fabsf(lg)));
                g = p - yv;
            }
            s_o[t] = S * g * inv_n;
        }
    }
    if (!train) return;
    __syncthreads();
    float *part = a.partial + (size_t)b * ((size_t)NO * (a.C + 1) + 2);
    __shared__ float s_l[2][2];
    if (t < 128) {
        const float l0 = wave_sum<64>(loss_h[0]), l1 = wave_sum<64>(loss_h[1]);
        if ((t & 63) == 0) { s_l[t >> 6][0] = l0; s_l[t >> 6][1] = l1; }
    }
    __syncthreads();
    if (t == 0) { part[(size_t)NO * (a.C + 1)] = s_l[0][0] + s_l[1][0]; part[(size_t)NO * (a.C + 1) + 1] = s_l[0][1] + s_l[1][1]; }
    for (int i = t; i < NO * a.C; i += 256) { const int o = i / a.C, c = i - o * a.C; part[i] = s_o[o] * s_f[c]; }
    if (t < NO) part[(size_t)NO * a.C + t] = s_o[t];
    for (int c = t; c < a.cs; c += 256) {
        float g = 0.f;
        if (c < a.C)
            for (int o = 0; o < NO; ++o) { const int h = o / a.K, k = o - h * a.K; g += s_o[o] * a.w[h][(size_t)c * a.K + k]; }
        const f16 gv = (f16)(g / (float)(Hh * Wh));
        for (int q = 0; q < Hh * Wh; ++q) a.dP[((size_t)b * Hh * Wh + q) * a.cs + c] = gv;
    }
}

__global__ __launch_bounds__(256) void evalnet_head_reduce_kernel(const float *__restrict__ partial, int B, int n_heads, int K,
                                                                 int C, const float *__restrict__ inv_scale_ptr,
                                                                 float *__restrict__ dw0, float *__restrict__ db0,
                                                                 float *__restrict__ dw1, float *__restrict__ db1,
                                                                 float *__restrict__ found_inf, float *__restrict__ stats) {
    const int NO = n_heads * K, per = NO * (C + 1) + 2;
    const int i = blockIdx.x * 256 + threadIdx.x;
    if (i < NO * (C + 1)) {
        float s = 0.f;
        for (int b = 0; b < B; ++b) s += partial[(size_t)b * per + i];
        s *= *inv_scale_ptr;
        if (!isfinite(s)) *found_inf = 1.0f;
        if (i < NO * C) {
            const int o = i / C, c = i - o * C, h = o / K, k = o - h * K;
            (h ? dw1 : dw0)[(size_t)c * K + k] = s;
        } else {
            const int o = i - NO * C, h = o / K, k = o - h * K;
            (h ? db1 : db0)[k] = s;
        }
    }
    if (i == 0) {
        double l0 = 0, l1 = 0;
        for (int b = 0; b < B; ++b) { l0 += partial[(size_t)b * per + per - 2]; l1 += partial[(size_t)b * per + per - 1]; }
        const float m0 = (float)(l0 / ((double)B * K)), m1 = (float)(l1 / ((double)B * K));
        stats[0] = m0 + m1; stats[4] = m0; stats[5] = m1;
    }
}
// ... 65 lines not shown
__global__ __launch_bounds__(256) void head_softmax_kernel(const f16 *__restrict__ z, const float *__restrict__ sc,
                                                           const float *__restrict__ sh, const float *__restrict__ w,
                                                           const float *__restrict__ bias, int cin, int cs, int K,
                                                           long long n_pix, float *__restrict__ probs, int vec) {
    extern __shared__ __attribute__((aligned(16))) float s_slab[];
    const int lane = threadIdx.x & 63, wave = threadIdx.x >> 6, p16 = lane & 15, g = lane >> 4;
    float *so = s_slab + (size_t)wave * 64 * K;
    HeadMfma<KT> h;
    h.load(w, bias, sc, sh, cin, cs, K);
    const long long n_grp = (n_pix + 63) / 64;
    for (long long grp = (long long)blockIdx.x * 4 + wave; grp < n_grp; grp += (long long)gridDim.x * 4) {
        f16x8 zr[4];
#pragma unroll
        for (int u = 0; u < 4; ++u) {
            const long long px = grp * 64 + u * 16 + p16;
            zr[u] = h.load_z(z, px < n_pix ? px : n_pix - 1, cs);
        }
#pragma unroll
        for (int u = 0; u < 4; ++u) {
            f32x4 pr[KT];
            h.probs(zr[u], K, pr);
#pragma unroll
            for (int kt = 0; kt < KT; ++kt)
#pragma unroll
                for (int r = 0; r < 4; ++r) {
                    const int k = 16 * kt + 4 * g + r;
                    if (k < K) so[(u * 16 + p16) * K + k] = pr[kt][r];
                }
        }
        __builtin_amdgcn_wave_barrier();
        __builtin_amdgcn_fence(__ATOMIC_RELEASE, "wavefront");
        const long long left = n_pix - grp * 64;
        const int n_here = (int)(left < 64 ? left : 64) * K;
        float *dst = probs + grp * 64 * K;
        if (vec && (n_here & 3) == 0) {
            for (int i = lane; i < n_here / 4; i += 64) reinterpret_cast<float4 *>(dst)[i] = reinterpret_cast<const float4 *>(so)[i];
        } else {
            for (int i = lane; i < n_here; i += 64) dst[i] = so[i];
        }
        __builtin_amdgcn_wave_barrier();
        __builtin_amdgcn_fence(__ATOMIC_ACQUIRE, "wavefront");
    }
}

static int launch_head_softmax(const f16 *z, const float *sc, const float *sh, const float *w, const float *bias, int cin, int cs,
                               int K, long long n_pix, float *probs, hipStream_t stream) {
    constexpr int cap = 2048;
    const long long want = (n_pix + 255) / 256;
    const int nb = (int)(want < cap ? want : cap);
    const size_t lds = (size_t)4 * 64 * K * sizeof(float);
    const int vec = (reinterpret_cast<uintptr_t>(probs) & 15) == 0;
    const int kt = (K + 15) / 16;
#define IMK_HS(KT) imk_klaunch(head_softmax_kernel<KT>, dim3(nb), dim3(256), lds, stream, z, sc, sh, w, bias, cin, cs, K, n_pix, probs, vec)
    switch (kt) {
        case 1: IMK_HS(1); break;
        case 2: IMK_HS(2); break;
        case 3: IMK_HS(3); break;
        default: IMK_HS(4); break;
    }
#undef IMK_HS
    IMK_LAUNCH_CHECK();
    return IMK_OK;
}

int imk_launch_head(const f16 *z, const float *sc, const float *sh, const float *w, const float *bias, int cin, int cs,
                    int K, int softmax, long long n_pix, float *probs, hipStream_t stream) {
    if (K > 64) return IMK_EUNSUPPORTED;
    if (softmax && (cs == 8 || cs == 16 || cs == 24 || cs == 32)) {
        ImkProfScope prof(PF_HEAD, (double)n_pix * (cs * 2 + K * 4), stream);
        return launch_head_softmax(z, sc, sh, w, bias, cin, cs, K, n_pix, probs, stream);
    }
    const int nb = (int)((n_pix + 255) / 256);
    const size_t lds = ((size_t)K * cs + K + 2 * cs + 256 * (size_t)(K | 1)) * sizeof(float);
    ImkProfScope prof(PF_HEAD, (double)n_pix * (cs * 2 + K * 4), stream);
#define IMK_HEAD(CS)                                                                                                     \
    do {                                                                                                                 \
        if (lds > 64 * 1024)                                                                                             \
            IMK_HIP(hipFuncSetAttribute(reinterpret_cast<const void *>(head_kernel<CS>),                                  \
                                        hipFuncAttributeMaxDynamicSharedMemorySize, (int)lds));                          \
        imk_klaunch(head_kernel<CS>, dim3(nb), dim3(256), lds, stream, z, sc, sh, w, bias, cin, K, softmax, n_pix, probs);                    \
    } while (0)
    switch (cs) {
        case 8: IMK_HEAD(8); break;
        case 16: IMK_HEAD(16); break;
        case 24: IMK_HEAD(24); break;
        case 32: IMK_HEAD(32); break;
        default: return IMK_EUNSUPPORTED;
    }
#undef IMK_HEAD
    IMK_LAUNCH_CHECK();
    return IMK_OK;
}

int imk_loss_blocks(long long n_pix) {
    constexpr int cap = 1024;
    const long long nb = (n_pix + 255) / 256;
    return (int)(nb > cap ? cap : nb);
}

int imk_launch_head_loss(const f16 *z, const float *sc, const float *sh, const float *w, const float *bias, int cin, int cs,
                         int K, int softmax, long long n_pix, const uint8_t *y, const ImkCtl *ctl, float *stats,
                         f16 *dlogit, float *loss_partial, hipStream_t stream, int y255) {
    if (K > 64) return IMK_EUNSUPPORTED;
    if (y255 && softmax) return IMK_EINVAL;
    const int nb = imk_loss_blocks(n_pix);
    const size_t lds = ((size_t)K * cs + K + 2 * cs + (softmax ? 256 * (size_t)(K | 1) : 0)) * sizeof(float);
    const int cs_out = imk_pad8(K);
    ImkProfScope prof(PF_HEAD_LOSS, (double)n_pix * (cs * 2 + (softmax ? 1 : K) + cs_out * 2), stream);
#define IMK_HL1(KERN) do { if (lds > 64 * 1024) IMK_HIP(hipFuncSetAttribute(reinterpret_cast<const void *>(KERN), hipFuncAttributeMaxDynamicSharedMemorySize, (int)lds)); \
    imk_klaunch(KERN, dim3(nb), dim3(256), lds, stream, z, sc, sh, w, bias, cin, K, softmax, n_pix, y, ctl, stats, cs_out, dlogit, loss_partial); } while (0)
#define IMK_HL(CS) if (y255) IMK_HL1((head_loss_kernel<CS, true>)); else IMK_HL1((head_loss_kernel<CS>))
    switch (cs) {
        case 8: IMK_HL(8); break;
        case 16: IMK_HL(16); break;
        case 24: IMK_HL(24); break;
        case 32: IMK_HL(32); break;
        default: return IMK_EUNSUPPORTED;
    }
#undef IMK_HL
#undef IMK_HL1
    IMK_LAUNCH_CHECK();
    return IMK_OK;
}


int imk_launch_loss_finalize(const float *loss_partial, long long n_pix, int K, int kind, float *stats, hipStream_t stream) {
    const double denom = kind == 0 ? (double)n_pix * K : (double)n_pix;
    ImkProfScope prof(PF_STEP_TAIL, (double)imk_loss_blocks(n_pix) * 4, stream);
    imk_klaunch(loss_finalize_kernel, dim3(1), dim3(256), 0, stream, loss_partial, imk_loss_blocks(n_pix), denom, stats);
    IMK_LAUNCH_CHECK();
    return IMK_OK;
}

int imk_launch_rmse_scale(const float *loss_partial, long long n_pix, int K, float *grads, long long n_grads, float *stats,
                          hipStream_t stream) {
    ImkProfScope prof(PF_STEP_TAIL, (double)n_grads * 8, stream);
    long long nb = (n_grads + 1023) / 1024;
    if (nb < 1) nb = 1;
    if (nb > 1024) nb = 1024;
    imk_klaunch(rmse_scale_kernel, dim3((int)nb), dim3(256), 0, stream, loss_partial, imk_loss_blocks(n_pix), (double)n_pix * K, grads, n_grads, stats);
    IMK_LAUNCH_CHECK();
    return IMK_OK;
}

int imk_launch_ctl_init(ImkCtl *ctl, hipStream_t stream) {
    imk_klaunch(ctl_init_kernel, dim3(1), dim3(1), 0, stream, ctl);
    IMK_LAUNCH_CHECK();
    return IMK_OK;
}

int imk_launch_adamw(float *p, float *m, float *v, const float *g, long long n, ImkCtl *ctl, const float *stats,
                     float grad_scale, float lr, float wd, float b1, float b2, float eps, hipStream_t stream) {
    ImkProfScope prof(PF_STEP_TAIL, (double)n * 28, stream);
    imk_klaunch(adamw_kernel, dim3((int)((n + 255) / 256)), dim3(256), 0, stream, p, m, v, g, n, ctl, stats, grad_scale, lr, wd, b1, b2, eps);
    IMK_LAUNCH_CHECK();
    return IMK_OK;
}

int imk_launch_concat_pool(const f16 *za, const float *sca, const float *sha, int csa, const f16 *zb, const float *scb,
                           const float *shb, int csb, int B, int Hh, int Wh, f16 *cat, hipStream_t stream, int a_div) {
    IMK_CHECK_ARG(a_div >= 1 && B % a_div == 0);
    const long long n = (long long)B * Hh * Wh * ((csa + csb) / 8);
    imk_klaunch(concat_pool_kernel, dim3((int)((n + 255) / 256)), dim3(256), 0, stream, za, sca, sha, csa, zb, scb, shb, csb, B, Hh, Wh, cat,
                a_div);
    IMK_LAUNCH_CHECK();
    return IMK_OK;
}

int imk_launch_onehot(const uint8_t *cls, long long n_pix, int cs, f16 *out, hipStream_t stream) {
    const long long n = n_pix * (cs / 8);
    imk_klaunch(onehot_kernel, dim3((int)((n + 255) / 256)), dim3(256), 0, stream, cls, n_pix, cs, out);
    IMK_LAUNCH_CHECK();
    return IMK_OK;
}

size_t imk_evalnet_head_partial_floats(int B, int n_heads, int K, int C) { return (size_t)B * ((size_t)n_heads * K * (C + 1) + 2); }

int imk_launch_evalnet_head(const f16 *z, const float *sc, const float *sh, const float *const *w, const float *const *bias,
                            int n_heads, int K, int C, int cs, int B, int H, int W, float *out, const float *y,
                            const ImkCtl *ctl, float *stats, f16 *dP, float *partial, hipStream_t stream) {
    if (n_heads < 1 || n_heads > 2 || n_heads * K > 128 || H < 2 || W < 2) return IMK_EUNSUPPORTED;
    EvalHeadArgs a{z, sc, sh, {w[0], n_heads > 1 ? w[1] : nullptr}, {bias[0], n_heads > 1 ? bias[1] : nullptr},
                   n_heads, K, C, cs, B, H, W, out, y, ctl, stats, dP, partial};
    imk_klaunch(evalnet_head_kernel, dim3(B), dim3(256), (size_t)(cs + 128) * sizeof(float), stream, a);
    IMK_LAUNCH_CHECK();
    return IMK_OK;
}

int imk_launch_evalnet_head_reduce(const float *partial, int B, int n_heads, int K, int C, const float *inv_scale_ptr,
                                   float *dw0, float *db0, float *dw1, float *db1, float *found_inf, float *stats,
                                   hipStream_t stream) {
    const int n = n_heads * K * (C + 1);
    imk_klaunch(evalnet_head_reduce_kernel, dim3((n + 255) / 256), dim3(256), 0, stream, partial, B, n_heads, K, C, inv_scale_ptr, dw0, db0, dw1, db1,
                                                                   found_inf, stats);
    IMK_LAUNCH_CHECK();
    return IMK_OK;
}
```

inconsistencymasks_amd/csrc/imk_kernels.h:

```cpp
#pragma once
#include "imk_common.h"

enum ImkLoadMode {
    LM_RAW = 0,
    LM_AFFINE = 1,
    LM_POOL = 2,
    LM_UPADD = 3,
    LM_U8 = 4,
    LM_BNBWD = 5,
    LM_STEM = 6,
};
enum ImkEpilogue {
    EP_RELU = 0,
    EP_PLAIN = 1,
    EP_MASK = 2,
};

struct ImkInput {
    const void *in;
    const void *in2;
    const float *sc, *sh;
    const float *sc2, *sh2;
    int lmode;
    int cin, cs_in;
    float u8_div;
    int u8_c;
    int src_h, src_w;
};

#define IMK_SCHED_HEADS 32
#define IMK_SCHED_STRIDE 256
#define IMK_SCHED_BYTES (IMK_SCHED_HEADS * IMK_SCHED_STRIDE)
struct ImkConvArgs {
    ImkInput x;
    int B, H, W;
    int ksize;
    int cout, cs_out;
    const f16 *wpk;
    const float *bias;
    f16 *out;
    const f16 *mask;
    const f16 *wpk2;
    const float *bias2;
    f16 *out2;
    int cout2, cs_out2;
    const f16 *dystat_z;
    float *stats_partial;
    int *stats_rows;
    int epi;
    int pair;
    const f16 *pre_wpk;
    const float *pre_bias, *pre_sc, *pre_sh;
    int pre_cout;
    float *wg_partial;
    const float *wg_sc, *wg_sh;
    f16 *sum2_out;
    const f16 *sum2_z;
    unsigned *sched;
};
inline double imk_conv_flops(const ImkConvArgs &a) {
    const double px = (double)a.B * a.H * a.W;
    const int cin_main = a.pre_wpk ? a.pre_cout : a.x.cin;
    double f = 2.0 * px * (a.ksize == 3 ? 9 : 1) * cin_main * a.cout;
    if (a.wpk2) f += 2.0 * px * a.cout * a.cout2;
    if (a.pre_wpk) f += 2.0 * px * a.x.cin * a.pre_cout;
    return f;
}
bool imk_conv_can_fuse_wgrad(const ImkConvArgs &dgrad_args);
bool imk_conv_can_sum2(const ImkConvArgs &dgrad_args);
bool imk_conv_gemm_ok(const ImkConvArgs &a);
int imk_launch_conv_gemm(const ImkConvArgs &a, hipStream_t stream);
bool imk_conv_gemm_chain_ok(const ImkConvArgs &a);
int imk_conv_gemm_num_tiles(int B, int H, int W);
inline double imk_conv_algorithmic_bytes(const ImkConvArgs &a) {
    const double px = (double)a.B * a.H * a.W;
    double in_b;
    switch (a.x.lmode) {
        case LM_POOL: in_b = 4.0 * px * a.x.cs_in * 2; break;
        case LM_UPADD: in_b = px * a.x.cs_in * 2 + 0.25 * px * a.x.cs_in * 2; break;
        case LM_BNBWD: in_b = 2.0 * px * a.x.cs_in * 2; break;
        case LM_U8: in_b = px * a.x.cin; break;
        case LM_STEM: in_b = px * a.x.u8_c; break;
        default: in_b = px * a.x.cs_in * 2;
    }
    double out_b = (a.wpk2 && !a.out) ? 0.0 : px * a.cs_out * 2;
    if (a.wpk2) out_b += px * a.cs_out2 * 2;
    if (a.epi == EP_MASK) out_b += px * a.cs_out * 2;
    if (a.epi != EP_RELU && a.dystat_z) out_b += px * a.cs_out * 2;
    return in_b + out_b;
}
int imk_conv_fused_wgrad_rows_max();
int imk_conv_num_tiles(int B, int H, int W, int cs_in, int ksize);
int imk_launch_conv(const ImkConvArgs &a, hipStream_t stream);

struct ImkWgradArgs {
    ImkInput x;
    const f16 *dA;
    const f16 *dA_z;
    const float *dA_coef;
    int B, H, W, ksize, cout, cs_out;
    float *partial;
    int n_split;
};
inline double imk_wgrad_flops(const ImkWgradArgs &a) {
    return 2.0 * a.B * a.H * a.W * (a.ksize == 3 ? 9 : 1) * (double)a.x.cin * a.cout;
}
bool imk_bwd1x1_ok(int lmode, int cs_in, int cs_out, bool masked);
int imk_bwd1x1_rows(long long n_pix, int cs_in, int cs_out);
int imk_launch_bwd1x1(const ImkInput &x, const f16 *dy, const f16 *z, const float *coef, const f16 *wpk_bwd, f16 *dx,
                      float *wg_partial, int B, int H, int W, int cout, hipStream_t stream);
int imk_wgrad_splits(int B, int H, int W, int cin, int cout);
bool imk_wgrad_gemm_ok(int lmode, bool bnb, int ksize, int cs_in, int cs_out, long long pixels);
bool imk_wgrad_gemm_wide(int cs_in, int cs_out, long long pixels);
int imk_wgrad_gemm_splits(int lmode, int B, int H, int W, int ksize, int cs_in, int cs_out);
int imk_launch_wgrad_gemm(const ImkWgradArgs &a, hipStream_t stream);
size_t imk_wgrad_partial_floats(int B, int H, int W, int ksize, int cin, int cout);
int imk_launch_wgrad(const ImkWgradArgs &a, hipStream_t stream);

inline long long imk_conv_max_pixels() { return 1ll << 24; }
bool imk_conv_can_chain(const ImkConvArgs &first, int cout2);
bool imk_conv_can_prestage(const ImkConvArgs &main, int lm_pre, int cin_pre, int cout_pre);
bool imk_conv_can_chain_tile(const ImkConvArgs &first, int cout2, bool store_intermediate);
bool imk_conv_stem_fusable(int u8_c, int ch0, int cout_next);
bool imk_conv_pair_layout(int k_in, int m_out, bool u8_input);
size_t imk_packed_conv_halfs(int ksize, int cin, int cout, int transposed, bool pair);

#define IMK_PACK_MAX_JOBS 80
struct ImkPackJob { const float *w; f16 *dst; int ksize, cin, cout, transposed, pair; };
struct ImkCtl;
struct ImkPackJobs {
    ImkPackJob j[IMK_PACK_MAX_JOBS];
    int n;
    ImkCtl *ctl;
    const float *stats;
};
int imk_launch_pack_jobs(const ImkPackJobs &jobs, hipStream_t stream);

#define IMK_WGF_MAX_JOBS 32
struct ImkWgFinalJob {
    const float *partial;
    float *red;
    float *dw, *db;
    int n_split, n_chunks, chunk, n_tiles, T, cin, cout, cot_n;
    int work1_begin;
    int tile_begin;
};
struct ImkWgFinalJobs { ImkWgFinalJob j[IMK_WGF_MAX_JOBS]; int n, total_work1, total_tiles; };
int imk_wgf_add_job(ImkWgFinalJobs &jobs, float *partial, int n_split, int ksize, int cin, int cout, float *dw, float *db);
int imk_launch_wgrad_finalize_jobs(const ImkWgFinalJobs &jobs, const float *inv_scale_ptr, float *found_inf, hipStream_t stream);

struct ImkSelectArgs {
    const float *scores;
    const int32_t *counts;
    const uint8_t *cand;
    int n_models, batch, n_cand, n_heads, n_out, miou;
    long long cand_bytes;
    float thr;
    int32_t *best_idx;
    float *best_score;
    uint8_t *keep, *out;
    int gated;
};
int imk_launch_evalnet_select(const ImkSelectArgs &a, hipStream_t stream);
int imk_select_check(int n_models, int batch, int n_cand, int n_heads, int n_out, const int32_t *counts, const uint8_t *cand,
                     int64_t cand_bytes, int mode, const uint8_t *out, hipStream_t stream);
int imk_launch_repeat_rows(const uint8_t *src, int batch, int n_rep, long long row_bytes, uint8_t *dst, hipStream_t stream);

hipStream_t imk_side_pool_stream(int i);
```

inconsistencymasks_amd/csrc/imk_net.h:

```cpp
#pragma once
#include <algorithm>
#include <cstdlib>
#include <cstring>
#include <mutex>
#include <new>
#include "imk_elem.h"
#include "imk_kernels.h"
#include "imk_plan.h"


namespace {

constexpr size_t ALIGN = 256;
inline size_t up(size_t v) { return (v + ALIGN - 1) / ALIGN * ALIGN; }

inline int add_conv(imk_unet_plan *p, const char *name, int k, int cin, int cout, int res) {
    ImkLayer l{};
    l.name = name; l.kind = 0; l.ksize = k; l.cin = cin; l.cout = cout; l.res = res;
    p->layers.push_back(l);
    return (int)p->layers.size() - 1;
}
inline int add_bn(imk_unet_plan *p, const char *name, int c, int res, int producer) {
    ImkLayer l{};
    l.name = name; l.kind = 1; l.ksize = 0; l.cin = c; l.cout = c; l.res = res; l.producer = producer;
    p->layers.push_back(l);
    const int idx = (int)p->layers.size() - 1;
    p->layers[producer].bn_after = idx;
    return idx;
}
inline void set_src(imk_unet_plan *p, int conv, int lmode, int src, int src_bn = -1, int src2 = -1, int src2_bn = -1) {
    ImkLayer &l = p->layers[conv];
    l.lmode = lmode; l.src = src; l.src_bn = src_bn; l.src2 = src2; l.src2_bn = src2_bn;
}

inline void finish_layout(imk_unet_plan *p) {
    int64_t off = 0;
    for (auto &l : p->layers) {
        if (l.kind == 0) { l.off_w = off; off += (int64_t)l.ksize * l.ksize * l.cin * l.cout; l.off_b = off; off += l.cout; }
        else { l.off_w = off; off += l.cout; l.off_b = off; off += l.cout; }
        l.off_mean = l.off_var = -1;
    }
    p->n_trainable = off;
    for (auto &l : p->layers)
        if (l.kind == 1) { l.off_mean = off; off += l.cout; l.off_var = off; off += l.cout; }
    p->n_total = off;

    size_t pk = 0;
    for (auto &l : p->layers) {
        l.pk_fwd = l.pk_bwd = l.pk_chain = -1;
        if (l.kind == 0) {
            if (l.flags & IMK_LF_DENSE) continue;
            const bool u8 = l.lmode == LM_U8;
            l.pk_bytes_fwd = (int64_t)imk_packed_conv_halfs(l.ksize, l.cin, l.cout, 0, imk_conv_pair_layout(l.cin, l.cout, u8)) * 2;
            l.pk_bytes_bwd = (int64_t)imk_packed_conv_halfs(l.ksize, l.cin, l.cout, 1, imk_conv_pair_layout(l.cout, l.cin, false)) * 2;
            l.pk_fwd = (int64_t)pk; pk = up(pk + l.pk_bytes_fwd);
            l.pk_bwd = (int64_t)pk; pk = up(pk + l.pk_bytes_bwd);
            if (l.ksize == 1 && l.cin <= 16 && l.cout <= 16) { l.pk_chain = (int64_t)pk; pk = up(pk + 1024); }
        } else {
            l.pk_scale = (int64_t)pk; pk = up(pk + 2 * (size_t)imk_pad8(l.cout) * sizeof(float));
        }
    }
    p->packed_bytes = (int64_t)pk;
}

struct LayerWs {
    size_t out = 0;
    size_t dA = 0;
    size_t dy = 0;
    size_t stats_partial = 0;
    size_t scale = 0;
    size_t save = 0;
    size_t bwd_partial = 0;
    size_t coef = 0;
    size_t wg_partial = 0;
    int n_stats_tiles = 0;
    int n_bwd_rows = 0;
};
struct Ws {
    std::vector<LayerWs> L;
    size_t dU[4] = {0, 0, 0, 0};
    size_t dP[8] = {0, 0, 0, 0, 0, 0, 0, 0};
    size_t probs = 0, dlogit = 0, loss_partial = 0;
    size_t cat = 0, dcat = 0;
    size_t onehot = 0;
    size_t head_partial = 0;
    size_t sched = 0;
    bool has_sched = false;
    size_t total = 0;
};

struct Dim { int h, w; };
inline Dim res_dim(const imk_unet_cfg &c, int res) { return Dim{c.h >> res, c.w >> res}; }

template <typename Take>
inline void make_ws_layers(const imk_unet_plan *p, int B, int mode, Ws &w, Take &&take) {
    const int n = (int)p->layers.size();
    w.L.resize(n);
    for (int i = 0; i < n; ++i) {
        const ImkLayer &l = p->layers[i];
        const Dim d = res_dim(p->cfg, l.res);
        const size_t px = (size_t)B * d.h * d.w;
        if (l.kind == 0) {
            if (l.flags & IMK_LF_DENSE) continue;
            if (!(l.flags & IMK_LF_HEAD)) w.L[i].out = take(px * imk_pad8(l.cout) * 2);
            if (mode == 1) {
                w.L[i].dA = take(px * imk_pad8(l.cout) * 2);
                w.L[i].wg_partial = take(imk_wgrad_partial_floats(B, d.h, d.w, l.ksize, l.cin, l.cout) * sizeof(float));
            }
        } else if (mode == 1) {
            const int cs = imk_pad8(l.cout);
            const ImkLayer &pc = p->layers[l.producer];
            w.L[i].n_stats_tiles = imk_conv_num_tiles(B, d.h, d.w, imk_pad8(pc.cin), pc.ksize);
            w.L[i].stats_partial = take((size_t)w.L[i].n_stats_tiles * 2 * cs * sizeof(float));
            w.L[i].scale = take(2 * (size_t)cs * sizeof(float));
            w.L[i].save = take(2 * (size_t)cs * sizeof(float));
            w.L[i].n_bwd_rows = imk_bn_prep_blocks(B, d.h, d.w, cs);
            const int conv_rows = B * imk_cdiv(d.h, 8) * imk_cdiv(d.w, 16);
            if (conv_rows > w.L[i].n_bwd_rows) w.L[i].n_bwd_rows = conv_rows;
            const int up_rows = std::min(imk_conv_fused_wgrad_rows_max(), B * imk_cdiv(2 * d.h, 16) * imk_cdiv(2 * d.w, 16));
            if (up_rows > w.L[i].n_bwd_rows) w.L[i].n_bwd_rows = up_rows;
            w.L[i].bwd_partial = take((size_t)w.L[i].n_bwd_rows * 2 * cs * sizeof(float));
            w.L[i].coef = take(3 * (size_t)cs * sizeof(float));
            w.L[i].dy = take(px * cs * 2);
        }
    }
}

struct Ctx {
    const imk_unet_plan *p;
    Ws ws;
    uint8_t *base;
    const float *params;
    const uint8_t *packed;
    int B;
    bool train;
    hipStream_t stream;
    const uint8_t *x_in[2] = {nullptr, nullptr};
    unsigned *sched(int conv) const {
        return (!train && ws.has_sched) ? reinterpret_cast<unsigned *>(base + ws.sched + IMK_SCHED_BYTES * (size_t)conv) : nullptr;
    }
    int ovr_conv = -1;
    f16 *ovr_out = nullptr;
    f16 *act(int conv) const { return conv == ovr_conv ? ovr_out : reinterpret_cast<f16 *>(base + ws.L[conv].out); }
    f16 *dA(int conv) const { return reinterpret_cast<f16 *>(base + ws.L[conv].dA); }
    f16 *dy(int bn) const { return reinterpret_cast<f16 *>(base + ws.L[bn].dy); }
    const float *bn_scale(int bn) const {
        return train ? reinterpret_cast<const float *>(base + ws.L[bn].scale)
                     : reinterpret_cast<const float *>(packed + p->layers[bn].pk_scale);
    }
    const float *bn_shift(int bn) const { return bn_scale(bn) + imk_pad8(p->layers[bn].cout); }
    const f16 *wfwd(int conv) const { return reinterpret_cast<const f16 *>(packed + p->layers[conv].pk_fwd); }
    const f16 *wbwd(int conv) const { return reinterpret_cast<const f16 *>(packed + p->layers[conv].pk_bwd); }
};

inline ImkInput conv_input(const Ctx &c, int conv) {
    const ImkLayer &l = c.p->layers[conv];
    ImkInput in{};
    in.cin = l.cin;
// ... 226 lines not shown
            pending[n_pending++] = Pending{conv, dA_override};
            return (l.res == 0 && !last) ? flush_wgrads() : IMK_OK;
        }
        return launch_wgrad(conv, dA_override, c.stream);
    }
    int flush_block() { return flush_wgrads(); }
    int flush_wgrads() {
        if (n_pending == 0) return IMK_OK;
        const int si = n_fork % n_side;
        hipStream_t ws = c.p->side[si];
        ImkStopRing *ring = imk_tls_stop_ring;
        if (ring && ring->stream == c.stream && ring->last) {
            IMK_HIP(hipStreamWaitEvent(ws, ring->last, 0));
            ++n_fork;
        } else {
            hipEvent_t ev = c.p->ev_fork[n_fork++];
            IMK_HIP(hipEventRecord(ev, c.stream));
            IMK_HIP(hipStreamWaitEvent(ws, ev, 0));
        }
        used_side[si] = true;
        for (int i = 0; i < n_pending; ++i) {
            int rc = launch_wgrad(pending[i].conv, pending[i].dA_override, ws);
            if (rc) return rc;
        }
        n_pending = 0;
        if (defer_finalize) return IMK_OK;
        int rc = imk_launch_wgrad_finalize_jobs(jobs, &ctl->inv_loss_scale, found_inf, ws);
        jobs = ImkWgFinalJobs{};
        return rc;
    }
    int wgrad_dgrad(int conv, f16 *dst, const f16 *mask, int stat_bn = -1) {
        const int s2_bn = sum2_bn;
        sum2_bn = -1;
        const ImkLayer &l = c.p->layers[conv];
        if (mask && stat_bn < 0 && l.ksize == 1 && l.lmode == LM_RAW && l.src >= 0 && mask == c.act(l.src)) {
            ImkConvArgs a{};
            int rows = 0;
            dgrad_args(conv, dst, mask, -1, nullptr, a);
            if (imk_conv_can_fuse_wgrad(a)) {
                a.wg_partial = reinterpret_cast<float *>(c.base + c.ws.L[conv].wg_partial);
                a.stats_rows = &rows;
                int rc = imk_launch_conv(a, c.stream);
                if (rc) return rc;
                if (rows <= 0 || rows > imk_conv_fused_wgrad_rows_max()) return IMK_EWORKSPACE;
                return imk_wgf_add_job(jobs, a.wg_partial, rows, l.ksize, l.cin, l.cout, grads + l.off_w, grads + l.off_b);
            }
        }
        if (stat_bn < 0 && l.ksize == 1 && l.bn_after >= 0 && l.src >= 0 &&
            ((l.lmode == LM_RAW && mask && mask == c.act(l.src)) || (l.lmode == LM_UPADD && !mask)) &&
            imk_bwd1x1_ok(l.lmode, imk_pad8(l.cin), imk_pad8(l.cout), mask != nullptr)) {
            const Dim d = res_dim(c.p->cfg, l.res);
            const int rows = imk_bwd1x1_rows((long long)c.B * d.h * d.w, imk_pad8(l.cin), imk_pad8(l.cout));
            float *wgp = reinterpret_cast<float *>(c.base + c.ws.L[conv].wg_partial);
            const int bn = l.bn_after;
            int rc = imk_launch_bwd1x1(conv_input(c, conv), c.dy(bn), c.act(conv), reinterpret_cast<const float *>(c.base + c.ws.L[bn].coef),
                                       c.wbwd(conv), dst, wgp, c.B, d.h, d.w, l.cout, c.stream);
            if (rc) return rc;
            return imk_wgf_add_job(jobs, wgp, rows, l.ksize, l.cin, l.cout, grads + l.off_w, grads + l.off_b);
        }
        if (!mask && stat_bn >= 0 && l.ksize == 3 && l.lmode == LM_AFFINE && l.src_bn == stat_bn &&
            l.src == c.p->layers[stat_bn].producer) {
            ImkConvArgs a{};
            int rows = 0;
            dgrad_args(conv, dst, nullptr, stat_bn, &rows, a);
            a.wg_sc = c.bn_scale(stat_bn); a.wg_sh = c.bn_shift(stat_bn);
            if (imk_conv_can_fuse_wgrad(a)) {
                a.wg_partial = reinterpret_cast<float *>(c.base + c.ws.L[conv].wg_partial);
                int rc = imk_launch_conv(a, c.stream);
                if (rc) return rc;
                rc = dgrad_done(stat_bn, rows);
                if (rc) return rc;
                if (rows > imk_conv_fused_wgrad_rows_max()) return IMK_EWORKSPACE;
                return imk_wgf_add_job(jobs, a.wg_partial, rows, l.ksize, l.cin, l.cout, grads + l.off_w, grads + l.off_b);
            }
        }
        const bool wide = imk_pad8(l.cin) >= 24 || imk_pad8(l.cout) >= 24;
        if (l.res == 0 && !tail_early && wide) {
            int rc = dgrad(conv, dst, mask, stat_bn, s2_bn);
            if (rc) return rc;
            return wgrad(conv);
        }
        int rc = wgrad(conv);
        if (rc) return rc;
        return dgrad(conv, dst, mask, stat_bn, s2_bn);
    }
    int finish_wgrads() {
        for (int i = 0; i < n_pending; ++i) {
            int rc = launch_wgrad(pending[i].conv, pending[i].dA_override, c.stream);
            if (rc) return rc;
        }
        n_pending = 0;
        for (int si = 0; si < n_side; ++si) {
            if (!used_side[si]) continue;
            IMK_HIP(hipEventRecord(c.p->ev_join[si], c.p->side[si]));
            IMK_HIP(hipStreamWaitEvent(c.stream, c.p->ev_join[si], 0));
        }
        return imk_launch_wgrad_finalize_jobs(jobs, &ctl->inv_loss_scale, found_inf, c.stream);
    }
    int bn_bwd(int bn, int mode, const f16 *g_direct, const f16 *g_other, int g_other_cs = 0) {
        const ImkLayer &b = c.p->layers[bn];
        const Dim d = res_dim(c.p->cfg, b.res);
        const int cs = imk_pad8(b.cout);
        const int prod = b.producer;
        const LayerWs &lw = c.ws.L[bn];
        float *partial = reinterpret_cast<float *>(c.base + lw.bwd_partial);
        float *coef = reinterpret_cast<float *>(c.base + lw.coef);
        const float *save = reinterpret_cast<const float *>(c.base + lw.save);
        const f16 *z = c.act(prod);
        int rows = dy_rows[bn];
        if (mode == 1 || rows == 0) {
            int rc = imk_launch_bn_bwd_prep(mode, mode == 0 ? c.dy(bn) : g_direct, g_other, z, c.bn_scale(bn), c.bn_shift(bn),
                                            c.dy(bn), partial, c.B, d.h, d.w, cs, c.stream, g_other_cs);
            if (rc) return rc;
            rows = imk_bn_prep_blocks(c.B, d.h, d.w, cs);
        }
        return imk_launch_bn_bwd_coef(partial, rows, b.cout, cs, (double)c.B * d.h * d.w, c.params + b.off_w, save, save + cs,
                                      &ctl->inv_loss_scale, coef, grads + b.off_w, grads + b.off_b, found_inf, c.stream);
    }
};

struct ImkStopRingScope {
    ImkStopRing ring{};
    ImkStopRing *prev = nullptr;
    bool on = false;
    ImkStopRingScope(const imk_unet_plan *plan, hipStream_t stream, int n_side) {
        if (n_side <= 0 || !plan->ev_ring[0]) return;
        ring = ImkStopRing{plan->ev_ring, 128, 0, stream, nullptr};
        prev = imk_tls_stop_ring;
        imk_tls_stop_ring = &ring;
        on = true;
    }
    ~ImkStopRingScope() { if (on) imk_tls_stop_ring = prev; }
    ImkStopRingScope(const ImkStopRingScope &) = delete;
    ImkStopRingScope &operator=(const ImkStopRingScope &) = delete;
};

inline bool ensure_side_streams(const imk_unet_plan *plan, int n = 1) {
    std::call_once(plan->side_once, [plan]() {
        bool ok = true;
        for (int i = 0; i < imk_unet_plan::MAX_SIDE; ++i)
            ok = ok && hipEventCreateWithFlags(&plan->ev_join[i], hipEventDisableTiming) == hipSuccess;
        for (auto &e : plan->ev_fork) ok = ok && hipEventCreateWithFlags(&e, hipEventDisableTiming) == hipSuccess;
        for (auto &e : plan->ev_ring) ok = ok && hipEventCreateWithFlags(&e, hipEventDisableTiming) == hipSuccess;
        plan->side_ok = ok;
    });
    if (!plan->side_ok) return false;
    for (int i = 0; i < n && i < imk_unet_plan::MAX_SIDE; ++i) {
        if (!plan->side[i]) plan->side[i] = imk_side_pool_stream(i);
        if (!plan->side[i]) return false;
    }
    return true;
}

inline int pack_weights(const imk_unet_plan *plan, const float *params, void *packed, hipStream_t stream, ImkCtl *ctl,
                        const float *stats, bool fold_bn) {
    IMK_CHECK_ARG(plan && params && packed);
    uint8_t *pk = (uint8_t *)packed;
    ImkPackJobs pj{};
    ImkFoldJobs fj{};
    pj.ctl = ctl; pj.stats = stats;
    auto flush_pack = [&]() -> int { int rc = imk_launch_pack_jobs(pj, stream); pj.n = 0; pj.ctl = nullptr; return rc; };
    for (size_t i = 0; i < plan->layers.size(); ++i) {
        const ImkLayer &l = plan->layers[i];
        if (l.kind == 0) {
            if (l.flags & IMK_LF_DENSE) continue;
            for (int tr = 0; tr < 3; ++tr) {
                if (tr == 0 && (l.flags & IMK_LF_HEAD)) continue;
                if (tr == 2 && (l.pk_chain < 0 || (l.flags & IMK_LF_HEAD))) continue;
                f16 *dst = (f16 *)(pk + (tr == 2 ? l.pk_chain : (tr ? l.pk_bwd : l.pk_fwd)));
                const int pair = tr == 2 ? (imk_conv_pair_layout(l.cin, l.cout, false) && l.cin <= 8)
                                         : (tr ? imk_conv_pair_layout(l.cout, l.cin, false) : imk_conv_pair_layout(l.cin, l.cout, l.lmode == LM_U8));
                pj.j[pj.n++] = ImkPackJob{params + l.off_w, dst, l.ksize, l.cin, l.cout, tr, pair};
                if (pj.n == IMK_PACK_MAX_JOBS) { int rc = flush_pack(); if (rc) return rc; }
            }
        } else {
            if (fj.n == IMK_FOLD_MAX_JOBS) return IMK_EUNSUPPORTED;
            fj.j[fj.n++] = ImkFoldJob{params + l.off_w, params + l.off_b, params + l.off_mean, params + l.off_var,
                                      (float *)(pk + l.pk_scale), l.cout, imk_pad8(l.cout)};
        }
    }
    int rc = flush_pack();
    if (rc) return rc;
    if (pj.ctl) return IMK_EINVAL;
    return fold_bn ? imk_launch_bn_fold_jobs(fj, stream) : IMK_OK;
}

}
```

inconsistencymasks_amd/csrc/imk_plan.h:

```cpp
#pragma once
#include <mutex>
#include <string>
#include <vector>
#include "imk_common.h"

struct ImkLayer {
    std::string name;
    int kind;
    int ksize, cin, cout;
    int64_t off_w, off_b;
    int64_t off_mean, off_var;
    int res;
    int64_t pk_fwd, pk_bwd;
    int64_t pk_bytes_fwd, pk_bytes_bwd;
    int64_t pk_chain;
    int64_t pk_scale;
    int src = -1;
    int src_bn = -1;
    int src2 = -1, src2_bn = -1;
    int lmode = 0;
    int bn_after = -1;
    int producer = -1;
    int flags = 0;
};
enum { IMK_SRC_XA = -2, IMK_SRC_XB = -3, IMK_SRC_CAT = -4, IMK_SRC_ONEHOT = -5 };
enum {
    IMK_LF_HEAD = 1,
    IMK_LF_DENSE = 4,
    IMK_LF_U8_RAW = 2,
};

struct imk_unet_plan {
    imk_unet_cfg cfg;
    int net = 0;
    imk_evalnet_cfg ecfg{};
    std::vector<ImkLayer> layers;
    int64_t n_total, n_trainable;
    int64_t packed_bytes;
    mutable std::once_flag side_once;
    static constexpr int MAX_SIDE = 2;
    mutable hipStream_t side[MAX_SIDE] = {};
    mutable hipEvent_t ev_fork[40] = {};
    mutable hipEvent_t ev_join[MAX_SIDE] = {};
    mutable hipEvent_t ev_ring[128] = {};
    mutable bool side_ok = false;
    bool dbg_materialize = false, dbg_single_stream = false;
    float bn_momentum = 0.99f;
    int find(const char *name) const {
        for (size_t i = 0; i < layers.size(); ++i) if (layers[i].name == name) return (int)i;
        return -1;
    }
};
```

inconsistencymasks_amd/csrc/imk_stage.h:

```cpp
#pragma once
#include <cstdlib>
#include "imk_kernels.h"
#include "imk_elem.h"

typedef __attribute__((__vector_size__(4 * sizeof(__fp16)))) __fp16 h4;
#define LDS_PTR(T, p) ((__attribute__((address_space(3))) T *)(p))

namespace {

constexpr int TW = 16;
constexpr int WG_STRIDE_H = 16;
constexpr int WG_RED_CHUNK = 16;

__host__ __device__ constexpr int imk_lds_pitch(int nc8) { return nc8 <= 1 ? 1 : ((nc8 + 1) & ~3) + 2; }

struct TileCoord { int b, ty0, tx0; };

__device__ __forceinline__ TileCoord tile_coord(int tile, int tiles_x, int tiles_y, int th) {
    TileCoord c;
    const int per_img = tiles_x * tiles_y;
    c.b = tile / per_img;
    const int r = tile - c.b * per_img;
    const int ty = r / tiles_x;
    c.ty0 = ty * th;
    c.tx0 = (r - ty * tiles_x) * TW;
    return c;
}

__host__ __device__ inline int imk_cdiv_d(int a, int b) { return (a + b - 1) / b; }
#ifndef IMK_PASS_CAP
#define IMK_PASS_CAP 4
#endif
__host__ __device__ inline int imk_pass_chunks(int nc8) {
    if (nc8 <= IMK_PASS_CAP) return nc8;
    const int n_pass = imk_cdiv_d(nc8, IMK_PASS_CAP);
    return imk_cdiv_d(nc8, n_pass);
}

__device__ __forceinline__ unsigned fast_div(unsigned n, unsigned d, float inv_d) {
    unsigned q = (unsigned)((float)n * inv_d);
    const int r = (int)n - (int)(q * d);
    if (r < 0) --q; else if (r >= (int)d) ++q;
    return q;
}

__device__ __forceinline__ TileCoord tile_coord_fast(int tile, int tiles_x, int per_img, float inv_tx, float inv_pi) {
    TileCoord c;
    c.b = (int)fast_div((unsigned)tile, (unsigned)per_img, inv_pi);
    const int r = tile - c.b * per_img;
    const int ty = (int)fast_div((unsigned)r, (unsigned)tiles_x, inv_tx);
    c.ty0 = ty * 16;
    c.tx0 = (r - ty * tiles_x) * TW;
    return c;
}

__device__ __forceinline__ f16x8 affine8(f16x8 z, const float *sc, const float *sh) { return imk_affine8(z, sc, sh); }

__device__ __forceinline__ f16x8 load_chunk(const ImkInput &in, int b, int y, int x, int H, int W, int c8,
                                            const float *s_aff) {
    const int cs = in.cs_in;
    switch (in.lmode) {
        case LM_RAW: {
            const f16 *p = (const f16 *)in.in + ((size_t)(b * H + y) * W + x) * cs + c8 * 8;
            return *(const f16x8 *)p;
        }
        case LM_AFFINE: {
            const f16 *p = (const f16 *)in.in + ((size_t)(b * H + y) * W + x) * cs + c8 * 8;
            return affine8(*(const f16x8 *)p, s_aff + c8 * 8, s_aff + cs + c8 * 8);
        }
        case LM_POOL: {
            const int H2 = in.src_h ? in.src_h : 2 * H, W2 = in.src_w ? in.src_w : 2 * W;
            const f16 *p = (const f16 *)in.in + ((size_t)(b * H2 + 2 * y) * W2 + 2 * x) * cs + c8 * 8;
            const f16x8 z00 = *(const f16x8 *)p, z01 = *(const f16x8 *)(p + cs);
            const f16x8 z10 = *(const f16x8 *)(p + (size_t)W2 * cs), z11 = *(const f16x8 *)(p + (size_t)W2 * cs + cs);
            return imk_affine_pool8(z00, z01, z10, z11, s_aff + c8 * 8, s_aff + cs + c8 * 8);
        }
        case LM_UPADD: {
            const int Hl = H / 2, Wl = W / 2;
            const f16 *pl = (const f16 *)in.in + ((size_t)(b * Hl + (y >> 1)) * Wl + (x >> 1)) * cs + c8 * 8;
            const f16 *ps = (const f16 *)in.in2 + ((size_t)(b * H + y) * W + x) * cs + c8 * 8;
            const f16x8 lo = affine8(*(const f16x8 *)pl, s_aff + c8 * 8, s_aff + cs + c8 * 8);
            const f16x8 sk = affine8(*(const f16x8 *)ps, s_aff + 2 * cs + c8 * 8, s_aff + 3 * cs + c8 * 8);
            f16x8 o;
#pragma unroll
            for (int j = 0; j < 8; ++j) o[j] = (f16)((float)lo[j] + (float)sk[j]);
            return o;
        }
        case LM_BNBWD: {
            const size_t o = ((size_t)(b * H + y) * W + x) * cs + c8 * 8;
            const f16x8 dy = *(const f16x8 *)((const f16 *)in.in + o), z = *(const f16x8 *)((const f16 *)in.in2 + o);
            const float *A = s_aff + c8 * 8, *Bc = s_aff + cs + c8 * 8, *Cc = s_aff + 2 * cs + c8 * 8;
            f16x8 o8;
#pragma unroll
            for (int j = 0; j < 8; ++j) {
                const float zf = (float)z[j];
                o8[j] = zf > 0.f ? (f16)(A[j] * (float)dy[j] + Bc[j] * zf + Cc[j]) : (f16)0.f;
            }
            return o8;
        }
        default: {
            const uint8_t *p = (const uint8_t *)in.in + ((size_t)(b * H + y) * W + x) * in.cin;
            f16x8 o;
#pragma unroll
            for (int j = 0; j < 8; ++j) o[j] = (f16)(j < in.cin ? (float)p[j] / in.u8_div : 0.0f);
            return o;
        }
    }
}

__device__ __forceinline__ void stage_affine_table(const ImkInput &in, float *s_aff) {
    const int cs = in.cs_in;
    if (in.lmode == LM_AFFINE || in.lmode == LM_POOL || in.lmode == LM_UPADD)
        for (int i = threadIdx.x; i < cs; i += 256) { s_aff[i] = in.sc[i]; s_aff[cs + i] = in.sh[i]; }
    if (in.lmode == LM_UPADD)
        for (int i = threadIdx.x; i < cs; i += 256) { s_aff[2 * cs + i] = in.sc2[i]; s_aff[3 * cs + i] = in.sh2[i]; }
    if (in.lmode == LM_BNBWD)
        for (int i = threadIdx.x; i < 3 * cs; i += 256) s_aff[i] = in.sc[i];
    if (in.lmode == LM_STEM) {
        for (int i = threadIdx.x; i < cs; i += 256) {
            const bool real = i < in.cin;
            s_aff[i] = in.sc[i]; s_aff[cs + i] = in.sh[i];
            for (int c = 0; c < 4; ++c) s_aff[(2 + c) * cs + i] = (real && c < in.u8_c) ? (float)(f16)in.sc2[c * in.cin + i] : 0.f;
            s_aff[6 * cs + i] = real ? in.sh2[i] : 0.f;
        }
    }
}

template <int LM> struct RawChunk { f16x8 v[LM == LM_POOL ? 4 : ((LM == LM_UPADD || LM == LM_BNBWD) ? 2 : 1)]; };
template <> struct RawChunk<LM_U8> { uint32_t b[4]; };
template <> struct RawChunk<LM_STEM> { uint32_t b[4]; };

template <int LM>
__device__ __forceinline__ void raw_load(const ImkInput &in, int b, int y, int x, int H, int W, int c8, RawChunk<LM> &r) {
    const int cs = in.cs_in;
    if constexpr (LM == LM_RAW || LM == LM_AFFINE) {
        r.v[0] = *(const f16x8 *)((const f16 *)in.in + ((size_t)(b * H + y) * W + x) * cs + c8 * 8);
    } else if constexpr (LM == LM_POOL) {
        const int H2 = in.src_h ? in.src_h : 2 * H, W2 = in.src_w ? in.src_w : 2 * W;
        const f16 *p = (const f16 *)in.in + ((size_t)(b * H2 + 2 * y) * W2 + 2 * x) * cs + c8 * 8;
        r.v[0] = *(const f16x8 *)p;
        r.v[1] = *(const f16x8 *)(p + cs);
        r.v[2] = *(const f16x8 *)(p + (size_t)W2 * cs);
        r.v[3] = *(const f16x8 *)(p + (size_t)W2 * cs + cs);
    } else if constexpr (LM == LM_UPADD) {
        r.v[0] = *(const f16x8 *)((const f16 *)in.in + ((size_t)(b * (H / 2) + (y >> 1)) * (W / 2) + (x >> 1)) * cs + c8 * 8);
        r.v[1] = *(const f16x8 *)((const f16 *)in.in2 + ((size_t)(b * H + y) * W + x) * cs + c8 * 8);
    } else if constexpr (LM == LM_BNBWD) {
        const size_t o = ((size_t)(b * H + y) * W + x) * cs + c8 * 8;
        r.v[0] = *(const f16x8 *)((const f16 *)in.in + o);
        r.v[1] = *(const f16x8 *)((const f16 *)in.in2 + o);
    } else {
        const int nb = LM == LM_STEM ? in.u8_c : in.cin;
        const uint8_t *p = (const uint8_t *)in.in + ((size_t)(b * H + y) * W + x) * nb;
        typedef uint32_t __attribute__((aligned(1))) u32_unaligned;
        const int rem = (H * W - (y * W + x)) * nb;
        const int back = rem >= 4 ? 0 : 4 - rem;
        const uint32_t v = *reinterpret_cast<const u32_unaligned *>(p - back) >> (8 * back);
#pragma unroll
        for (int j = 0; j < 4; ++j) r.b[j] = (j < nb) ? ((v >> (8 * j)) & 0xffu) : 0u;
    }
}

template <int LM>
__device__ __forceinline__ f16x8 raw_transform(const RawChunk<LM> &r, const float *s_aff, int cs, int c8, int cin,
                                               float u8_div, int u8_c = 4) {
    if constexpr (LM == LM_RAW) {
        return r.v[0];
    } else if constexpr (LM == LM_AFFINE) {
        return affine8(r.v[0], s_aff + c8 * 8, s_aff + cs + c8 * 8);
    } else if constexpr (LM == LM_POOL) {
        return imk_affine_pool8(r.v[0], r.v[1], r.v[2], r.v[3], s_aff + c8 * 8, s_aff + cs + c8 * 8);
    } else if constexpr (LM == LM_UPADD) {
        const f16x8 lo = affine8(r.v[0], s_aff + c8 * 8, s_aff + cs + c8 * 8);
        const f16x8 sk = affine8(r.v[1], s_aff + 2 * cs + c8 * 8, s_aff + 3 * cs + c8 * 8);
        f16x8 o;
#pragma unroll
        for (int j = 0; j < 8; ++j) o[j] = (f16)((float)lo[j] + (float)sk[j]);
        return o;
    } else if constexpr (LM == LM_BNBWD) {
        const float *A = s_aff + c8 * 8, *Bc = s_aff + cs + c8 * 8, *Cc = s_aff + 2 * cs + c8 * 8;
        f16x8 o;
#pragma unroll
        for (int j = 0; j < 8; ++j) {
            const float zf = (float)r.v[1][j];
            o[j] = zf > 0.f ? (f16)(A[j] * (float)r.v[0][j] + Bc[j] * zf + Cc[j]) : (f16)0.f;
        }
        return o;
    } else if constexpr (LM == LM_STEM) {
        float xin[4];
// ... 148 lines not shown
```

inconsistencymasks_amd/csrc/imk_switches.cpp:

```cpp
#include "imk_switches.h"
#include <cstdlib>
#include "imk_plan.h"

namespace {
bool on_unless_zero(const char *name) {
    const char *e = getenv(name);
    return !(e && e[0] == '0');
}
int int_or(const char *name, int dflt) {
    const char *e = getenv(name);
    return e ? atoi(e) : dflt;
}
}

const ImkSwitches &imk_switches() {
    static const ImkSwitches s = []() {
        ImkSwitches v{};
        v.conv_wide = on_unless_zero("IMK_CONV_WIDE");
        v.conv_gemm = on_unless_zero("IMK_CONV_GEMM");
        v.conv_chain_tile = int_or("IMK_CONV_CHAIN_TILE", 1);
        v.conv_prestage = on_unless_zero("IMK_CONV_PRESTAGE");
        v.wide_chain = on_unless_zero("IMK_WIDE_CHAIN");
        v.wide_chain_train = on_unless_zero("IMK_WIDE_CHAIN_TRAIN");
        v.gemm_chain = on_unless_zero("IMK_GEMM_CHAIN");
        v.gemm_over_chain = int_or("IMK_GEMM_OVER_CHAIN", 1);
        v.gemm_ad3_wgs = int_or("IMK_GEMM_AD3_WGS", 1024);
        v.wgrad_gemm_min = int_or("IMK_WGRAD_GEMM_MIN", 0);
        v.wgrad_nfo2 = on_unless_zero("IMK_WGRAD_NFO2");
        v.student_fused = on_unless_zero("IMK_STUDENT_FUSED");
        v.consistency_fused = on_unless_zero("IMK_CONSISTENCY_FUSED");
        v.select_shared = on_unless_zero("IMK_SELECT_SHARED");
        const int n = int_or("IMK_SIDE_STREAMS", 1);
        v.side_streams = n < 0 ? 0 : (n > imk_unet_plan::MAX_SIDE ? imk_unet_plan::MAX_SIDE : n);
        return v;
    }();
    return s;
}
```

inconsistencymasks_amd/csrc/imk_switches.h:

```cpp
#pragma once

struct ImkSwitches {
    bool conv_wide;
    bool conv_gemm;
    int conv_chain_tile;
    bool conv_prestage;
    bool wide_chain;
    bool wide_chain_train;
    bool gemm_chain;
    int gemm_over_chain;
    int gemm_ad3_wgs;
    int wgrad_gemm_min;
    bool wgrad_nfo2;
    bool student_fused;
    bool consistency_fused;
    bool select_shared;
    int side_streams;
};

const ImkSwitches &imk_switches();
```

inconsistencymasks_amd/csrc/imk_unet.hip:

```cpp
#include <atomic>
#include <cstdio>
#include "imk_net.h"
#include "imk_head.h"
#include "imk_switches.h"

namespace {


struct Topo {
    int in_c, in_bn;
    int e_c3[4], e_c1[4], e_bn[4];
    int b_c3, b_c1, b_bn;
    int d_ca[4], d_bna[4], d_c3[4], d_c1[4], d_bnb[4];
    int out;
};

Topo make_topo(const imk_unet_plan *p) {
    Topo t{};
    t.in_c = p->find("in.c"); t.in_bn = p->find("in.bn");
    char nm[16];
    for (int i = 0; i < 4; ++i) {
        snprintf(nm, sizeof nm, "e%d.c3", i + 1); t.e_c3[i] = p->find(nm);
        snprintf(nm, sizeof nm, "e%d.c1", i + 1); t.e_c1[i] = p->find(nm);
        snprintf(nm, sizeof nm, "e%d.bn", i + 1); t.e_bn[i] = p->find(nm);
    }
    t.b_c3 = p->find("b.c3"); t.b_c1 = p->find("b.c1"); t.b_bn = p->find("b.bn");
    for (int j = 0; j < 4; ++j) {
        snprintf(nm, sizeof nm, "d%d.ca", j + 6); t.d_ca[j] = p->find(nm);
        snprintf(nm, sizeof nm, "d%d.bna", j + 6); t.d_bna[j] = p->find(nm);
        snprintf(nm, sizeof nm, "d%d.c3", j + 6); t.d_c3[j] = p->find(nm);
        snprintf(nm, sizeof nm, "d%d.c1", j + 6); t.d_c1[j] = p->find(nm);
        snprintf(nm, sizeof nm, "d%d.bnb", j + 6); t.d_bnb[j] = p->find(nm);
    }
    t.out = p->find("out");
    return t;
}

void build_layers(imk_unet_plan *p) {
    const int *ch = p->cfg.ch;
    int c = add_conv(p, "in.c", 1, p->cfg.c_in, ch[0], 0);
    add_bn(p, "in.bn", ch[0], 0, c);
    const int enc_in[4] = {ch[0], ch[0], ch[1], ch[2]};
    const int enc_f[4] = {ch[0], ch[1], ch[2], ch[3]};
    char nm[16];
    for (int i = 0; i < 4; ++i) {
        snprintf(nm, sizeof nm, "e%d.c3", i + 1); add_conv(p, nm, 3, enc_in[i], enc_f[i], i);
        snprintf(nm, sizeof nm, "e%d.c1", i + 1); c = add_conv(p, nm, 1, enc_f[i], enc_f[i], i);
        snprintf(nm, sizeof nm, "e%d.bn", i + 1); add_bn(p, nm, enc_f[i], i, c);
    }
    add_conv(p, "b.c3", 3, ch[3], ch[4], 4);
    c = add_conv(p, "b.c1", 1, ch[4], ch[3], 4);
    add_bn(p, "b.bn", ch[3], 4, c);
    const int dec_in[4] = {ch[3], ch[2], ch[1], ch[0]};
    const int dec_f1[4] = {ch[3], ch[2], ch[1], ch[0]};
    const int dec_f2[4] = {ch[2], ch[1], ch[0], ch[0]};
    for (int j = 0; j < 4; ++j) {
        const int res = 3 - j;
        snprintf(nm, sizeof nm, "d%d.ca", j + 6); c = add_conv(p, nm, 1, dec_in[j], dec_f1[j], res);
        snprintf(nm, sizeof nm, "d%d.bna", j + 6); add_bn(p, nm, dec_f1[j], res, c);
        snprintf(nm, sizeof nm, "d%d.c3", j + 6); add_conv(p, nm, 3, dec_f1[j], dec_f1[j], res);
        snprintf(nm, sizeof nm, "d%d.c1", j + 6); c = add_conv(p, nm, 1, dec_f1[j], dec_f2[j], res);
        snprintf(nm, sizeof nm, "d%d.bnb", j + 6); add_bn(p, nm, dec_f2[j], res, c);
    }
    c = add_conv(p, "out", 1, ch[0], p->cfg.n_out, 0);
    p->layers[c].flags = IMK_LF_HEAD;

    const Topo t = make_topo(p);
    set_src(p, t.in_c, LM_U8, IMK_SRC_XA);
    set_src(p, t.e_c3[0], LM_AFFINE, t.in_c, t.in_bn);
    for (int i = 1; i < 4; ++i) set_src(p, t.e_c3[i], LM_POOL, t.e_c1[i - 1], t.e_bn[i - 1]);
    for (int i = 0; i < 4; ++i) set_src(p, t.e_c1[i], LM_RAW, t.e_c3[i]);
    set_src(p, t.b_c3, LM_POOL, t.e_c1[3], t.e_bn[3]);
    set_src(p, t.b_c1, LM_RAW, t.b_c3);
    for (int j = 0; j < 4; ++j) {
        const int lo_c = j == 0 ? t.b_c1 : t.d_c1[j - 1], lo_bn = j == 0 ? t.b_bn : t.d_bnb[j - 1];
        set_src(p, t.d_ca[j], LM_UPADD, lo_c, lo_bn, t.e_c1[3 - j], t.e_bn[3 - j]);
        set_src(p, t.d_c3[j], LM_AFFINE, t.d_ca[j], t.d_bna[j]);
        set_src(p, t.d_c1[j], LM_RAW, t.d_c3[j]);
    }
    set_src(p, t.out, LM_AFFINE, t.d_c1[3], t.d_bnb[3]);
    finish_layout(p);
}

Ws make_ws(const imk_unet_plan *p, int B, int mode) {
    Ws w;
    const Topo t = make_topo(p);
    size_t off = 0;
    auto take = [&](size_t bytes) { size_t o = off; off = up(off + bytes); return o; };
    make_ws_layers(p, B, mode, w, take);
    if (mode == 0) { w.sched = take(IMK_SCHED_BYTES * p->layers.size()); w.has_sched = true; }

    if (mode == 1) {
        for (int j = 0; j < 4; ++j) {
            const ImkLayer &ca = p->layers[t.d_ca[j]];
            const Dim d = res_dim(p->cfg, ca.res);
            w.dU[j] = take((size_t)B * d.h * d.w * imk_pad8(ca.cin) * 2);
        }
        for (int i = 0; i < 4; ++i) {
            const ImkLayer &e = p->layers[t.e_c1[i]];
            const Dim d = res_dim(p->cfg, i + 1);
            w.dP[i] = take((size_t)B * d.h * d.w * imk_pad8(e.cout) * 2);
        }
        const size_t px = (size_t)B * p->cfg.h * p->cfg.w;
        w.dlogit = take(px * imk_pad8(p->cfg.n_out) * 2);
        w.loss_partial = take((size_t)imk_loss_blocks((long long)px) * sizeof(float));
        w.probs = take(px * p->cfg.n_out * sizeof(float));
    }
    w.total = off;
    return w;
}

int run_forward(Ctx &c, const Topo &t, float *probs, float *params_rw) {
    int rc;
    if (!c.train && c.ws.has_sched) IMK_HIP(hipMemsetAsync(c.base + c.ws.sched, 0, IMK_SCHED_BYTES * c.p->layers.size(), c.stream));
#define RUN(conv) do { rc = run_conv_fwd(c, (conv), params_rw); if (rc) return rc; } while (0)
#define RUN_PAIR(c3, c1) do { rc = run_conv_pair(c, (c3), (c1), params_rw); if (rc) return rc; } while (0)
    bool stem_fused = false;
    {
        const ImkLayer &st = c.p->layers[t.in_c], &c3 = c.p->layers[t.e_c3[0]];
        if (!c.train && !c.p->dbg_materialize && imk_conv_stem_fusable(st.cin, st.cout, c3.cout)) {
            ImkInput x{};
            x.in = c.x_in[0]; x.lmode = LM_STEM; x.cin = c3.cin; x.cs_in = imk_pad8(c3.cin); x.u8_c = st.cin;
            x.sc = c.bn_scale(t.in_bn); x.sh = c.bn_shift(t.in_bn);
            x.sc2 = c.params + st.off_w; x.sh2 = c.params + st.off_b;
            bool f = false;
            rc = run_conv_fwd(c, t.e_c3[0], params_rw, t.e_c1[0], &f, &x);
            if (rc == IMK_OK) stem_fused = true;
            else if (rc != IMK_EUNSUPPORTED) return rc;
        }
    }
    if (!stem_fused) { RUN(t.in_c); RUN_PAIR(t.e_c3[0], t.e_c1[0]); }
    for (int i = 1; i < 4; ++i) RUN_PAIR(t.e_c3[i], t.e_c1[i]);
    RUN_PAIR(t.b_c3, t.b_c1);
    for (int j = 0; j < 4; ++j) {
        rc = run_conv_pre_pair(c, t.d_ca[j], t.d_c3[j], t.d_c1[j]);
        if (rc == IMK_OK) continue;
        if (rc != IMK_EUNSUPPORTED) return rc;
        RUN(t.d_ca[j]); RUN_PAIR(t.d_c3[j], t.d_c1[j]);
    }
#undef RUN_PAIR
#undef RUN
    if (!probs) return IMK_OK;
    const ImkLayer &o = c.p->layers[t.out];
    const int bn = t.d_bnb[3];
    return imk_launch_head(c.act(t.d_c1[3]), c.bn_scale(bn), c.bn_shift(bn), c.params + o.off_w, c.params + o.off_b,
                           o.cin, imk_pad8(o.cin), o.cout, c.p->cfg.act_out, (long long)c.B * c.p->cfg.h * c.p->cfg.w,
                           probs, c.stream);
}

bool cfg_ok(const imk_unet_cfg *c) {
    if (!c) return false;
    if (c->h <= 0 || c->w <= 0 || (c->h % 16) || (c->w % 16)) return false;
    if (c->c_in < 1 || c->c_in > 8 || c->n_out < 1 || c->n_out > 64) return false;
    for (int i = 0; i < 5; ++i) if (c->ch[i] < 1 || c->ch[i] > 512) return false;
    if (imk_pad8(c->ch[0]) > 32) return false;
    return c->act_out == 0 || c->act_out == 1;
}

}

static std::atomic<int> g_runtime_warnings{0};
hipStream_t imk_side_pool_stream(int i) {
    struct Pool { std::mutex mu; hipStream_t s[imk_unet_plan::MAX_SIDE] = {}; };
    static Pool pools[64];
    if (i < 0 || i >= imk_unet_plan::MAX_SIDE) return nullptr;
    static std::once_flag hwq_once;
    std::call_once(hwq_once, []() {
        const char *e = getenv("GPU_MAX_HW_QUEUES");
        if (!e || atoi(e) < 8) {
            g_runtime_warnings.fetch_or(IMK_WARN_HW_QUEUES);
            fprintf(stderr, "libimk: GPU_MAX_HW_QUEUES=%s (< 8): side streams may serialise behind the caller's stream; "
                            "export GPU_MAX_HW_QUEUES=8 before the HIP runtime starts\n", e ? e : "unset");
        }
    });
    int dev = 0;
    (void)hipGetDevice(&dev);
    Pool &pool = pools[dev & 63];
    std::lock_guard<std::mutex> lock(pool.mu);
    if (!pool.s[i] && hipStreamCreateWithFlags(&pool.s[i], hipStreamNonBlocking) != hipSuccess) pool.s[i] = nullptr;
    return pool.s[i];
}

extern "C" int imk_runtime_warnings(void) { return g_runtime_warnings.load(); }

extern "C" int imk_unet_plan_side_stream(const imk_unet_plan *plan, int i, void **stream_out) {
    IMK_CHECK_ARG(plan && stream_out && i >= 0 && i < imk_unet_plan::MAX_SIDE);
    if (!ensure_side_streams(plan, i + 1)) return IMK_EINVAL;
    *stream_out = (void *)plan->side[i];
    return IMK_OK;
}

extern "C" int imk_unet_plan_create(const imk_unet_cfg *cfg, imk_unet_plan **out) {
    IMK_CHECK_ARG(out);
    if (!cfg_ok(cfg)) return IMK_EINVAL;
    if ((long long)cfg->h * cfg->w >= imk_conv_max_pixels() || cfg->w >= (1 << 16)) return IMK_EUNSUPPORTED;
    imk_unet_plan *p = new (std::nothrow) imk_unet_plan();
    if (!p) return IMK_EINVAL;
    p->cfg = *cfg;
    build_layers(p);
    *out = p;
    return IMK_OK;
}

extern "C" void imk_unet_plan_destroy(imk_unet_plan *plan) {
    if (!plan) return;
    for (int i = 0; i < imk_unet_plan::MAX_SIDE; ++i) {
        if (!plan->side[i]) continue;
        (void)hipStreamSynchronize(plan->side[i]);
        if (plan->ev_join[i]) (void)hipEventDestroy(plan->ev_join[i]);
    }
    for (auto &e : plan->ev_fork) if (e) (void)hipEventDestroy(e);
    for (auto &e : plan->ev_ring) if (e) (void)hipEventDestroy(e);
    delete plan;
}

extern "C" int imk_unet_param_count(const imk_unet_plan *plan, int64_t *total, int64_t *trainable) {
    IMK_CHECK_ARG(plan);
    if (total) *total = plan->n_total;
    if (trainable) *trainable = plan->n_trainable;
    return IMK_OK;
}

extern "C" int imk_unet_num_layers(const imk_unet_plan *plan) { return plan ? (int)plan->layers.size() : IMK_EINVAL; }

extern "C" int imk_unet_layer_info(const imk_unet_plan *plan, int idx, imk_layer_info *out) {
    IMK_CHECK_ARG(plan && out && idx >= 0 && idx < (int)plan->layers.size());
    const ImkLayer &l = plan->layers[idx];
    memset(out, 0, sizeof *out);
    strncpy(out->name, l.name.c_str(), sizeof(out->name) - 1);
    out->kind = l.kind; out->ksize = l.ksize; out->cin = l.cin; out->cout = l.cout;
    out->off_w = l.off_w; out->off_b = l.off_b; out->off_mean = l.off_mean; out->off_var = l.off_var;
    return IMK_OK;
}

extern "C" int imk_unet_plan_set_bn_momentum(imk_unet_plan *plan, float momentum) {
    IMK_CHECK_ARG(plan && momentum >= 0.f && momentum < 1.f);
    plan->bn_momentum = momentum;
    return IMK_OK;
}

extern "C" int imk_unet_plan_get_bn_momentum(const imk_unet_plan *plan, float *momentum) {
    IMK_CHECK_ARG(plan && momentum);
    *momentum = plan->bn_momentum;
    return IMK_OK;
}

extern "C" int imk_unet_plan_debug(imk_unet_plan *plan, int materialize, int single_stream) {
    IMK_CHECK_ARG(plan);
    if (materialize >= 0) plan->dbg_materialize = materialize != 0;
    if (single_stream >= 0) plan->dbg_single_stream = single_stream != 0;
    return IMK_OK;
}

extern "C" int64_t imk_unet_packed_bytes(const imk_unet_plan *plan) { return plan ? plan->packed_bytes : IMK_EINVAL; }


extern "C" int imk_unet_pack_weights(const imk_unet_plan *plan, const float *params, void *packed, void *stream_) {
    IMK_CHECK_ARG(plan && params && packed);
    IMK_HIP(hipMemsetAsync(packed, 0, (size_t)plan->packed_bytes, (hipStream_t)stream_));
    return pack_weights(plan, params, packed, (hipStream_t)stream_, nullptr, nullptr, true);
}

extern "C" int64_t imk_unet_workspace_bytes(const imk_unet_plan *plan, int batch, int mode) {
    if (!plan || batch <= 0 || (mode != 0 && mode != 1)) return IMK_EINVAL;
    return (int64_t)make_ws(plan, batch, mode).total;
}

extern "C" int imk_unet_forward(const imk_unet_plan *plan, const float *params, const void *packed, const uint8_t *x,
                                int batch, float *probs, void *workspace, int64_t workspace_bytes, void *stream_) {
    IMK_CHECK_ARG(plan && params && packed && x && probs && workspace && batch > 0);
    Ctx c{plan, make_ws(plan, batch, 0), (uint8_t *)workspace, params, (const uint8_t *)packed, batch, false,
          (hipStream_t)stream_};
    if ((int64_t)c.ws.total > workspace_bytes) return IMK_EWORKSPACE;
    c.x_in[0] = x;
    return run_forward(c, make_topo(plan), probs, nullptr);
}

extern "C" int imk_unet_tensor_info(const imk_unet_plan *plan, int batch, int mode, int layer_idx, int which,
                                    int64_t *byte_offset, int *h, int *w, int *c, int *c_stride) {
    IMK_CHECK_ARG(plan && batch > 0 && layer_idx >= 0 && layer_idx < (int)plan->layers.size());
    IMK_CHECK_ARG(mode == 0 || mode == 1);
    const Ws ws = make_ws(plan, batch, mode);
    const ImkLayer &l = plan->layers[layer_idx];
    const Dim d = res_dim(plan->cfg, l.res);
    size_t off = 0;
    if (which == 0 && l.kind == 0 && layer_idx != plan->find("out")) off = ws.L[layer_idx].out;
    else if (which == 1 && l.kind == 0 && mode == 1) off = ws.L[layer_idx].dA;
    else if (which == 2 && l.kind == 1 && mode == 1) off = ws.L[layer_idx].dy;
    else return IMK_EINVAL;
    if (byte_offset) *byte_offset = (int64_t)off;
    if (h) *h = d.h;
    if (w) *w = d.w;
    if (c) *c = l.cout;
    if (c_stride) *c_stride = imk_pad8(l.cout);
    return IMK_OK;
}

static size_t head_slab_bytes(const imk_unet_plan *plan, int batch, bool fused) {
    const imk_unet_cfg &cf = plan->cfg;
    const size_t px = (size_t)batch * cf.h * cf.w;
    const size_t probs = px * cf.n_out * sizeof(float), zlast = px * imk_pad8(cf.ch[0]) * sizeof(f16);
    return up(fused && zlast > probs ? zlast : probs);
}

extern "C" int64_t imk_unet_forward_im_workspace_bytes(const imk_unet_plan *plan, int n_models, int batch, int n_streams) {
    if (!plan || plan->net != 0 || n_models <= 0 || batch <= 0 || n_streams <= 0) return IMK_EINVAL;
    return (int64_t)(head_slab_bytes(plan, batch, true) * n_models + make_ws(plan, batch, 0).total * n_streams);
}

struct EnsembleHeads {
    const f16 **z;
    const float **sc, **sh, **w, **bias;
};

static int run_ensemble_forwards(const imk_unet_plan *plan, const Topo &topo, const Ws &ws, int n_models, const float *const *params,
                                 const void *const *packed, const uint8_t *x, int batch, size_t slab, uint8_t *base,
                                 int64_t workspace_bytes, const EnsembleHeads *heads, hipStream_t main_stream) {
    const imk_unet_cfg &cf = plan->cfg;
    const bool fused = heads != nullptr;
    const size_t probs_exact = (size_t)batch * cf.h * cf.w * cf.n_out * sizeof(float);
    const int max_streams = 1 + imk_unet_plan::MAX_SIDE;
    int n_slabs = (int)(((size_t)workspace_bytes - slab * n_models) / ws.total);
    if (n_slabs > n_models) n_slabs = n_models;
    if (n_slabs > max_streams) n_slabs = max_streams;
    if (n_slabs > 1 && (plan->dbg_single_stream || !ensure_side_streams(plan, n_slabs - 1))) n_slabs = 1;
    if (n_slabs > 1) {
        IMK_HIP(hipEventRecord(plan->ev_fork[0], main_stream));
        for (int s = 1; s < n_slabs; ++s) IMK_HIP(hipStreamWaitEvent(plan->side[s - 1], plan->ev_fork[0], 0));
    }
    const ImkLayer &o = plan->layers[topo.out];
    for (int m = 0; m < n_models; ++m) {
        const int sl = m % n_slabs;
        Ctx c{plan, ws, base + slab * n_models + ws.total * sl, params[m], (const uint8_t *)packed[m], batch, false,
              sl == 0 ? main_stream : plan->side[sl - 1]};
        c.x_in[0] = x;
        if (fused) {
            c.ovr_conv = topo.d_c1[3];
            c.ovr_out = reinterpret_cast<f16 *>(base + slab * m);
            heads->z[m] = c.ovr_out;
            heads->sc[m] = c.bn_scale(topo.d_bnb[3]); heads->sh[m] = c.bn_shift(topo.d_bnb[3]);
            heads->w[m] = params[m] + o.off_w; heads->bias[m] = params[m] + o.off_b;
        }
        int rc = run_forward(c, topo, fused ? nullptr : (float *)(base + probs_exact * m), nullptr);
        if (rc) return rc;
    }
    for (int s = 1; s < n_slabs; ++s) {
        IMK_HIP(hipEventRecord(plan->ev_join[s - 1], plan->side[s - 1]));
        IMK_HIP(hipStreamWaitEvent(main_stream, plan->ev_join[s - 1], 0));
    }
    return IMK_OK;
}

extern "C" int imk_unet_forward_im(const imk_unet_plan *plan, int n_models, const float *const *params,
                                   const void *const *packed, const uint8_t *x, int batch, float thr, int cmp_ge,
                                   const uint8_t *img, int block_in, int block_out, uint8_t *img_out, uint8_t *masks_out,
                                   uint8_t *im_out, int64_t *im_size, int64_t *pred_size, uint8_t *presence,
                                   void *workspace, int64_t workspace_bytes, void *stream_) {
    IMK_CHECK_ARG(plan && params && packed && x && workspace && batch > 0 && n_models > 0);
    const imk_unet_cfg &cf = plan->cfg;
    const Ws ws = make_ws(plan, batch, 0);
    const Topo topo = make_topo(plan);
    ImkHeadImArgs ha{};
    ha.n_models = n_models; ha.cin = cf.ch[0]; ha.cs = imk_pad8(cf.ch[0]); ha.K = cf.n_out; ha.softmax = cf.act_out;
    ha.batch = batch; ha.hw = cf.h * cf.w; ha.thr = thr; ha.cmp_ge = cmp_ge; ha.img = img; ha.c = cf.c_in;
    ha.block_in = block_in; ha.block_out = block_out; ha.img_out = img_out; ha.masks_out = masks_out; ha.im_out = im_out;
    ha.im_size = im_size; ha.pred_size = pred_size; ha.presence = presence;
    bool fused = !plan->dbg_materialize && imk_head_im_supported(ha) &&
                 (int64_t)(head_slab_bytes(plan, batch, true) * n_models + ws.total) <= workspace_bytes;
    const size_t slab = head_slab_bytes(plan, batch, fused);
    if ((int64_t)(slab * n_models + ws.total) > workspace_bytes) return IMK_EWORKSPACE;
    uint8_t *base = (uint8_t *)workspace;
    hipStream_t main_stream = (hipStream_t)stream_;
    const EnsembleHeads heads{ha.z, ha.sc, ha.sh, ha.w, ha.bias};
    int rc = run_ensemble_forwards(plan, topo, ws, n_models, params, packed, x, batch, slab, base, workspace_bytes,
                                   fused ? &heads : nullptr, main_stream);
    if (rc) return rc;
    if (fused) return imk_launch_head_im(ha, main_stream);
    if (cf.act_out == 0)
        return imk_im_binary((const float *)base, n_models, batch, cf.h, cf.w, cf.n_out, thr, cmp_ge, img, cf.c_in, block_in,
                             block_out, img_out, masks_out, im_out, im_size, pred_size, stream_);
    return imk_im_multiclass((const float *)base, n_models, batch, cf.h, cf.w, cf.n_out, img, cf.c_in, block_in, block_out,
                             img_out, masks_out, im_out, im_size, presence, stream_);
}

static size_t depth_map_bytes(const imk_unet_plan *plan, int batch) {
    return up((size_t)batch * plan->cfg.h * plan->cfg.w * sizeof(float));
}

extern "C" int64_t imk_unet_forward_im_depth_workspace_bytes(const imk_unet_plan *plan, int n_models, int batch, int n_streams) {
    const int64_t fwd = imk_unet_forward_im_workspace_bytes(plan, n_models, batch, n_streams);
    return fwd < 0 ? fwd : fwd + (int64_t)depth_map_bytes(plan, batch);
}

extern "C" int imk_unet_forward_im_depth(const imk_unet_plan *plan, int n_models, const float *const *params,
                                         const void *const *packed, const uint8_t *x, int batch, float mult, const uint8_t *img,
                                         int block_in, uint8_t *img_out, uint8_t *im_out, int64_t *im_size, float *thr_out,
                                         float *std_out, void *workspace, int64_t workspace_bytes, void *stream_) {
    IMK_CHECK_ARG(plan && plan->net == 0 && params && packed && x && workspace && batch > 0);
    IMK_CHECK_ARG(im_out && im_size && thr_out && (!img || img_out));
    const imk_unet_cfg &cf = plan->cfg;
    if (n_models < 2 || n_models > 16 || cf.act_out != 0 || cf.n_out != 1 || batch > 65535) return IMK_EUNSUPPORTED;
    const Ws ws = make_ws(plan, batch, 0);
    const Topo topo = make_topo(plan);
    const size_t map_bytes = depth_map_bytes(plan, batch);
    uint8_t *base = (uint8_t *)workspace + map_bytes;
    const int64_t fwd_bytes = workspace_bytes - (int64_t)map_bytes;
    float *map = std_out ? std_out : (float *)workspace;
    ImkDepthHeadArgs da{};
    da.n_models = n_models; da.cin = cf.ch[0]; da.cs = imk_pad8(cf.ch[0]); da.K = cf.n_out; da.softmax = cf.act_out;
    da.batch = batch; da.hw = cf.h * cf.w; da.map = map;
    const bool fused = !plan->dbg_materialize && imk_depth_head_supported(da) &&
                       (int64_t)(head_slab_bytes(plan, batch, true) * n_models + ws.total) <= fwd_bytes;
    const size_t slab = head_slab_bytes(plan, batch, fused);
// ... 315 lines not shown
    const bool head_mse_pass = cf.act_out == 0 && imk_head_mse_fused_ok(imk_pad8(ol.cin), ol.cout, n_pix, c.ws.L[obn].n_bwd_rows);
    if (!head_one_pass && !head_mse_pass)
        OK(imk_launch_head_loss(c.act(t.d_c1[3]), c.bn_scale(obn), c.bn_shift(obn), params + ol.off_w, params + ol.off_b, ol.cin,
                                imk_pad8(ol.cin), ol.cout, cf.act_out, n_pix, y, sv.ctl, stats, dlogit, loss_partial, stream, y255));

    const int n_side = imk_switches().side_streams;
    const bool side_on = !plan->dbg_single_stream && n_side > 0 && ensure_side_streams(plan, n_side);
    Bwd b{c, grads, sv.ctl, stats + 1, side_on ? n_side : 0};
    ImkStopRingScope stop_ring(plan, stream, b.n_side);
    bool loss_done = false;
    auto loss_on_side = [&]() -> int {
        if (loss_done || b.n_side <= 0 || b.n_fork <= 0 || loss_kind == 3) return IMK_OK;
        loss_done = true;
        return imk_launch_loss_finalize(loss_partial, n_pix, cf.n_out, fin_kind, stats, plan->side[(b.n_fork - 1) % b.n_side]);
    };
    int head_rows = 0;
    HeadWgJob head_job{};
    if (head_mse_pass) {
        const int rows = imk_head_cce_fused_rows(n_pix);
        float *wgp = reinterpret_cast<float *>(c.base + c.ws.L[t.out].wg_partial);
        OK(imk_launch_head_mse_fused(c.act(t.d_c1[3]), c.bn_scale(obn), c.bn_shift(obn), params + ol.off_w, params + ol.off_b,
                                     ol.cin, imk_pad8(ol.cin), ol.cout, n_pix, y, sv.ctl, stats, c.dy(obn), loss_partial,
                                     reinterpret_cast<float *>(c.base + c.ws.L[obn].bwd_partial), wgp, stream, y255));
        head_rows = rows;
        head_job = HeadWgJob{wgp, rows};
    } else if (head_one_pass) {
        const int rows = imk_head_cce_fused_rows(n_pix);
        float *wgp = reinterpret_cast<float *>(c.base + c.ws.L[t.out].wg_partial);
        OK(imk_launch_head_cce_fused(c.act(t.d_c1[3]), c.bn_scale(obn), c.bn_shift(obn), params + ol.off_w, params + ol.off_b,
                                     ol.cin, imk_pad8(ol.cin), ol.cout, n_pix, y, sv.ctl, stats, c.dy(obn), loss_partial,
                                     reinterpret_cast<float *>(c.base + c.ws.L[obn].bwd_partial), wgp, stream));
        head_rows = rows;
        head_job = HeadWgJob{wgp, rows};
    } else {
        OK(head_dgrad(b, t, dlogit, loss_on_side, &head_rows, &head_job));
    }
    OK(run_backward(b, t, head_rows, head_job.partial ? &head_job : nullptr, loss_on_side));
    if (!loss_done) OK(imk_launch_loss_finalize(loss_partial, n_pix, cf.n_out, fin_kind, stats, stream));
    if (loss_kind == 3) {
        int64_t n_total = 0, n_train = 0;
        OK(imk_unet_param_count(plan, &n_total, &n_train));
        OK(imk_launch_rmse_scale(loss_partial, n_pix, cf.n_out, grads, n_train, stats, stream));
    }
#undef OK
    return IMK_OK;
}

namespace {
struct ConsistLayout {
    Ws ws;
    size_t view[2], grads2, loss_partial, total;
};
ConsistLayout consist_layout(const imk_unet_plan *plan, int batch) {
    ConsistLayout l{make_ws(plan, batch, 1), {0, 0}, 0, 0, 0};
    const int rows = imk_loss_blocks((long long)batch * plan->cfg.h * plan->cfg.w);
    size_t off = 0;
    auto take = [&](size_t bytes) { size_t o = off; off = up(off + bytes); return o; };
    l.view[0] = take(l.ws.total);
    l.view[1] = take(l.ws.total);
    l.grads2 = take((size_t)plan->n_trainable * sizeof(float));
    l.loss_partial = take((size_t)rows * sizeof(float));
    l.total = off;
    return l;
}
}

extern "C" int64_t imk_unet_consistency_workspace_bytes(const imk_unet_plan *plan, int batch) {
    if (!plan || plan->net != 0 || batch <= 0) return IMK_EINVAL;
    return (int64_t)consist_layout(plan, batch).total;
}

extern "C" int imk_unet_consistency_fwd_bwd(const imk_unet_plan *plan, float *params, void *packed, void *state,
                                            const uint8_t *x1, const uint8_t *x2, int batch, float *grads, float *stats,
                                            void *workspace, int64_t workspace_bytes, void *stream_) {
    IMK_CHECK_ARG(plan && plan->net == 0 && params && packed && state && x1 && x2 && grads && stats && workspace && batch > 0);
    const ConsistLayout lay = consist_layout(plan, batch);
    if ((int64_t)lay.total > workspace_bytes) return IMK_EWORKSPACE;
    hipStream_t stream = (hipStream_t)stream_;
    uint8_t *base = (uint8_t *)workspace;
    Ctx c1{plan, lay.ws, base + lay.view[0], params, (const uint8_t *)packed, batch, true, stream};
    Ctx c2{plan, lay.ws, base + lay.view[1], params, (const uint8_t *)packed, batch, true, stream};
    c1.x_in[0] = x1;
    c2.x_in[0] = x2;
    const StateView sv = state_view(plan, state);
    const imk_unet_cfg &cf = plan->cfg;
    const Topo t = make_topo(plan);
    const long long n_pix = (long long)batch * cf.h * cf.w;
    const ImkLayer &ol = plan->layers[t.out];
    const int obn = t.d_bnb[3], cs = imk_pad8(ol.cin);
    float *grads2 = reinterpret_cast<float *>(base + lay.grads2);
    float *loss_partial = reinterpret_cast<float *>(base + lay.loss_partial);
    int rc;
#define OK(e) do { rc = (e); if (rc) return rc; } while (0)
    OK(run_forward(c1, t, nullptr, params));
    OK(run_forward(c2, t, nullptr, params));

    const bool fused = !plan->dbg_materialize && imk_switches().consistency_fused &&
                       ol.off_b + ol.cout == plan->n_trainable &&
                       imk_consistency_fused_ok(cs, ol.cout, cf.act_out, n_pix, lay.ws.L[obn].n_bwd_rows);
    const int head_rows = imk_loss_blocks(n_pix);
    HeadWgJob fused_job{reinterpret_cast<float *>(c1.base + lay.ws.L[t.out].wg_partial), head_rows};
    f16 *dlogit1 = reinterpret_cast<f16 *>(c1.base + lay.ws.dlogit), *dlogit2 = reinterpret_cast<f16 *>(c2.base + lay.ws.dlogit);
    if (fused) {
        OK(imk_launch_consistency_head(c1.act(t.d_c1[3]), c2.act(t.d_c1[3]), c1.bn_scale(obn), c1.bn_shift(obn), c2.bn_scale(obn),
                                       c2.bn_shift(obn), params + ol.off_w, params + ol.off_b, ol.cin, cs, ol.cout, n_pix, sv.ctl,
                                       stats, c1.dy(obn), c2.dy(obn), loss_partial,
                                       reinterpret_cast<float *>(c1.base + lay.ws.L[obn].bwd_partial),
                                       reinterpret_cast<float *>(c2.base + lay.ws.L[obn].bwd_partial), fused_job.partial, stream));
    } else {
        float *p1 = reinterpret_cast<float *>(c1.base + lay.ws.probs), *p2 = reinterpret_cast<float *>(c2.base + lay.ws.probs);
        OK(imk_launch_head(c1.act(t.d_c1[3]), c1.bn_scale(obn), c1.bn_shift(obn), params + ol.off_w, params + ol.off_b, ol.cin, cs,
                           ol.cout, cf.act_out, n_pix, p1, stream));
        OK(imk_launch_head(c2.act(t.d_c1[3]), c2.bn_scale(obn), c2.bn_shift(obn), params + ol.off_w, params + ol.off_b, ol.cin, cs,
                           ol.cout, cf.act_out, n_pix, p2, stream));
        OK(imk_launch_consistency_dlogit(p1, p2, ol.cout, cf.act_out, n_pix, sv.ctl, stats, dlogit1, dlogit2, loss_partial, stream));
    }

    const int n_side = imk_switches().side_streams;
    const bool side_on = !plan->dbg_single_stream && n_side > 0 && ensure_side_streams(plan, n_side);
    {
        Bwd b{c1, grads, sv.ctl, stats + 1, side_on ? n_side : 0};
        ImkStopRingScope stop_ring(plan, stream, b.n_side);
        bool loss_done = false;
        auto loss_on_side = [&]() -> int {
            if (loss_done || b.n_side <= 0 || b.n_fork <= 0) return IMK_OK;
            loss_done = true;
            return imk_launch_loss_finalize(loss_partial, n_pix, cf.n_out, 0, stats, plan->side[(b.n_fork - 1) % b.n_side]);
        };
        int rows = head_rows;
        HeadWgJob job = fused ? fused_job : HeadWgJob{};
        if (!fused) OK(head_dgrad(b, t, dlogit1, loss_on_side, &rows, &job));
        OK(run_backward(b, t, rows, job.partial ? &job : nullptr, loss_on_side));
        if (!loss_done) OK(imk_launch_loss_finalize(loss_partial, n_pix, cf.n_out, 0, stats, stream));
    }
    {
        Bwd b{c2, grads2, sv.ctl, stats + 1, side_on ? n_side : 0};
        ImkStopRingScope stop_ring(plan, stream, b.n_side);
        auto no_loss = []() -> int { return IMK_OK; };
        int rows = head_rows;
        HeadWgJob job{};
        if (!fused) OK(head_dgrad(b, t, dlogit2, no_loss, &rows, &job));
        OK(run_backward(b, t, rows, job.partial ? &job : nullptr, no_loss));
    }
    OK(imk_launch_grad_add(grads, grads2, fused ? ol.off_w : plan->n_trainable, stats + 1, stream));
#undef OK
    return IMK_OK;
}

extern "C" int imk_unet_adamw_step(const imk_unet_plan *plan, float *params, void *packed, void *state,
                                   const float *grads, const float *stats, float grad_scale, float lr, float wd,
                                   float beta1, float beta2, float eps, void *stream_) {
    IMK_CHECK_ARG(plan && params && packed && state && grads && stats);
    const StateView sv = state_view(plan, state);
    int rc = imk_launch_adamw(params, sv.m, sv.v, grads, plan->n_trainable, sv.ctl, stats, grad_scale, lr, wd, beta1, beta2,
                              eps, (hipStream_t)stream_);
    if (rc) return rc;
    return pack_weights(plan, params, packed, (hipStream_t)stream_, sv.ctl, stats, false);
}
```

Measured before the change: 25310 images/s.

## Fuse AdamW update with packed-weight scatter via precomputed inverse pack map

Builds a host-side inverse map from each trainable parameter to the f16 packed-weight slots it feeds, caches it on the device, and adds an AdamW kernel that writes the updated value straight into those slots. The separate pack_weights launch after each optimizer step goes away. The ctl end-of-step bookkeeping moves to a last-block ticket counter. This removes one kernel launch and a full re-read of params per training step, at the cost of scattered stores, a one-time map build, and a changed FMA order in the weight-decay update.

```diff
diff --git a/include/imk.h b/include/imk.h
--- a/include/imk.h
+++ b/include/imk.h
@@ -84,6 +84,7 @@
 
 IMK_API int64_t imk_unet_packed_bytes(const imk_unet_plan *plan);
 IMK_API int imk_unet_pack_weights(const imk_unet_plan *plan, const float *params, void *packed, void *stream);
+IMK_API int64_t imk_unet_pack_maps(const imk_unet_plan *plan, int32_t *forward, uint32_t *begin, uint32_t *slots, int64_t slots_cap);
 
 IMK_API int64_t imk_unet_workspace_bytes(const imk_unet_plan *plan, int batch, int mode);
 
diff --git a/inconsistencymasks_amd/_lib.py b/inconsistencymasks_amd/_lib.py
--- a/inconsistencymasks_amd/_lib.py
+++ b/inconsistencymasks_amd/_lib.py
@@ -55,6 +55,7 @@
     "imk_unet_layer_info": (c_int, [c_void_p, c_int, ctypes.POINTER(LayerInfo)]),
     "imk_unet_packed_bytes": (c_int64, [c_void_p]),
     "imk_unet_pack_weights": (c_int, [c_void_p, c_void_p, c_void_p, c_void_p]),
+    "imk_unet_pack_maps": (c_int64, [c_void_p, c_void_p, c_void_p, c_void_p, c_int64]),
     "imk_unet_workspace_bytes": (c_int64, [c_void_p, c_int, c_int]),
     "imk_unet_forward": (c_int, [c_void_p, c_void_p, c_void_p, c_void_p, c_int, c_void_p, c_void_p, c_int64, c_void_p]),
     "imk_unet_tensor_info": (c_int, [c_void_p, c_int, c_int, c_int, c_int, ctypes.POINTER(c_int64),
diff --git a/inconsistencymasks_amd/csrc/imk_conv.hip b/inconsistencymasks_amd/csrc/imk_conv.hip
--- a/inconsistencymasks_amd/csrc/imk_conv.hip
+++ b/inconsistencymasks_amd/csrc/imk_conv.hip
@@ -1464,80 +1464,10 @@
     IMK_STAMP_BEGIN(conv, 23);
     if (jobs.ctl && blockIdx.x == 0 && blockIdx.y == 0 && threadIdx.x == 0) imk_ctl_end_step(jobs.ctl, jobs.stats);
     const ImkPackJob &jb = jobs.j[blockIdx.y];
-    if (jb.transposed == 2) {
-        for (int i = blockIdx.x * 256 + threadIdx.x; i < 512; i += gridDim.x * 256) {
-            const int j = i & 7, lane = (i >> 3) & 63;
-            const int m = lane & 15, g = lane >> 4;
-            float v = 0.f;
-            if (!jb.pair) {
-                const int ci = 4 * g + j;
-                if (j < 4 && ci < jb.cin && m < jb.cout) v = jb.w[(size_t)ci * jb.cout + m];
-            } else {
-                const int ci = 4 * (g & 1) + j, co = m & 7;
-                if (j < 4 && (m >> 3) == (g >> 1) && ci < jb.cin && co < jb.cout) v = jb.w[(size_t)ci * jb.cout + co];
-            }
-            jb.dst[i] = (f16)v;
-        }
-        return;
-    }
-    const int T = jb.ksize == 3 ? 9 : 1;
-    const int m_dim = jb.transposed ? jb.cin : jb.cout, k_dim = jb.transposed ? jb.cout : jb.cin;
-    if (jb.pair && T == 9) {
-        const int nc8 = ((k_dim + 7) & ~7) / 8;
-        const int ns = 3 * nc8;
-        for (int i = blockIdx.x * 256 + threadIdx.x; i < ns * 512; i += gridDim.x * 256) {
-            const int j = i & 7, lane = (i >> 3) & 63, st = i >> 9;
-            const int m = lane & 15, g = lane >> 4;
-            const int q = 4 * st + g;
-            const int ut = q / nc8, c8 = q - ut * nc8;
-            const int r = ut / 3, c = ut - 3 * r, ky = r - (m >> 3);
-            const int mi = m & 7, ki = c8 * 8 + j;
-            float v = 0.f;
-            if (ky >= 0 && ky <= 2 && mi < m_dim && ki < k_dim) {
-                const int tap = ky * 3 + c;
-                if (!jb.transposed) v = jb.w[((size_t)tap * jb.cin + ki) * jb.cout + mi];
-                else v = jb.w[((size_t)(T - 1 - tap) * jb.cin + mi) * jb.cout + ki];
-            }
-            jb.dst[i] = (f16)v;
-        }
-        return;
-    }
-    if (jb.pair) {
-        const int nc8 = ((k_dim + 7) & ~7) / 8;
-        const int nq = T * nc8, ns = (nq + 1) / 2;
-        for (int i = blockIdx.x * 256 + threadIdx.x; i < ns * 512; i += gridDim.x * 256) {
-            const int j = i & 7, lane = (i >> 3) & 63, st = i >> 9;
-            const int m = lane & 15, g = lane >> 4;
-            const int q = 2 * st + (g & 1);
-            const int tap = q / nc8, c8 = q - tap * nc8;
-            const int mi = m & 7, ki = c8 * 8 + j;
-            float v = 0.f;
-            if (q < nq && (m >> 3) == (g >> 1) && mi < m_dim && ki < k_dim) {
-                if (!jb.transposed) v = jb.w[((size_t)tap * jb.cin + ki) * jb.cout + mi];
-                else v = jb.w[((size_t)(T - 1 - tap) * jb.cin + mi) * jb.cout + ki];
-            }
-            jb.dst[i] = (f16)v;
-        }
-        return;
-    }
-    const int nc8 = ((k_dim + 7) & ~7) / 8;
-    const int nc8p = imk_pass_chunks(nc8), nsp = (T * nc8p + 3) / 4;
-    const int ns = imk_cdiv_d(nc8, nc8p) * nsp;
-    const int total = ((m_dim + 15) / 16) * ns * 512;
+    const int total = (int)imk_pack_slots(jb.ksize, jb.cin, jb.cout, jb.transposed, jb.pair);
     for (int i = blockIdx.x * 256 + threadIdx.x; i < total; i += gridDim.x * 256) {
-        const int j = i & 7, lane = (i >> 3) & 63;
-        const int cs = i >> 9;
-        const int s = cs % ns, ct = cs / ns;
-        const int m = lane & 15, g = lane >> 4;
-        const int pass = s / nsp, q = 4 * (s - pass * nsp) + g;
-        const int tap = q / nc8p, c8 = pass * nc8p + (q - tap * nc8p);
-        const int mi = ct * 16 + m, ki = c8 < nc8 ? c8 * 8 + j : k_dim;
-        float v = 0.f;
-        if (tap < T && mi < m_dim && ki < k_dim) {
-            if (!jb.transposed) v = jb.w[((size_t)tap * jb.cin + ki) * jb.cout + mi];
-            else v = jb.w[((size_t)(T - 1 - tap) * jb.cin + mi) * jb.cout + ki];
-        }
-        jb.dst[i] = (f16)v;
+        const long long src = imk_pack_slot_source(jb.ksize, jb.cin, jb.cout, jb.transposed, jb.pair, i);
+        jb.dst[i] = (f16)(src >= 0 ? jb.w[src] : 0.f);
     }
     IMK_STAMP_END(1);
 }
@@ -1583,6 +1513,21 @@
     imk_klaunch(wgf_stage2_kernel, dim3(jobs.total_tiles), dim3(1024), 0, stream, jobs, inv_scale_ptr, found_inf);
     IMK_LAUNCH_CHECK();
     return IMK_OK;
+}
+
+long long imk_pack_slot_source_host(int ksize, int cin, int cout, int transposed, int pair, long long i) {
+    return imk_pack_slot_source(ksize, cin, cout, transposed, pair, (int)i);
+}
+
+void imk_pack_inverse_add(int ksize, int cin, int cout, int transposed, int pair, int64_t w_off, int64_t dst_half, uint32_t *count_or_cursor,
+                          uint32_t *slots) {
+    const long long total = imk_pack_slots(ksize, cin, cout, transposed, pair);
+    for (long long i = 0; i < total; ++i) {
+        const long long src = imk_pack_slot_source(ksize, cin, cout, transposed, pair, (int)i);
+        if (src < 0) continue;
+        if (!slots) count_or_cursor[w_off + src] += 1;
+        else slots[count_or_cursor[w_off + src]++] = (uint32_t)(dst_half + i);
+    }
 }
 
 int imk_launch_pack_jobs(const ImkPackJobs &jobs, hipStream_t stream) {
@@ -2270,12 +2215,5 @@
 }
 
 size_t imk_packed_conv_halfs(int ksize, int cin, int cout, int transposed, bool pair) {
-    if (transposed == 2) return 512;
-    const int T = ksize == 3 ? 9 : 1;
-    const int m_dim = transposed ? cin : cout, k_dim = transposed ? cout : cin;
-    const int nc8 = imk_pad8(k_dim) / 8;
-    if (pair) return (size_t)(T == 9 ? 3 * nc8 : (nc8 + 1) / 2) * 512;
-    const int nc8p = imk_pass_chunks(nc8);
-    const int ns = imk_cdiv_d(nc8, nc8p) * ((T * nc8p + 3) / 4);
-    return (size_t)((m_dim + 15) / 16) * ns * 512;
-}
+    return (size_t)imk_pack_slots(ksize, cin, cout, transposed, pair ? 1 : 0);
+}
diff --git a/inconsistencymasks_amd/csrc/imk_elem.h b/inconsistencymasks_amd/csrc/imk_elem.h
--- a/inconsistencymasks_amd/csrc/imk_elem.h
+++ b/inconsistencymasks_amd/csrc/imk_elem.h
@@ -7,7 +7,8 @@
     int good_steps;
     int step;
     float found_inf;
-    float pad[3];
+    unsigned ticket;
+    float pad[2];
 };
 
 int imk_launch_bn_finalize(const float *partial, int n_part, int c, int cs, double count, const float *gamma,
@@ -49,6 +50,9 @@
 int imk_launch_ctl_init(ImkCtl *ctl, hipStream_t stream);
 int imk_launch_adamw(float *p, float *m, float *v, const float *g, long long n, ImkCtl *ctl, const float *stats,
                      float grad_scale, float lr, float wd, float b1, float b2, float eps, hipStream_t stream);
+int imk_launch_adamw_pack(float *p, float *m, float *v, const float *g, long long n, ImkCtl *ctl, const float *stats,
+                          float grad_scale, float lr, float wd, float b1, float b2, float eps, const uint32_t *slot_begin,
+                          const uint32_t *slots, long long n_slots, f16 *packed, hipStream_t stream);
 
 int imk_launch_concat_pool(const f16 *za, const float *sca, const float *sha, int csa, const f16 *zb, const float *scb,
                            const float *shb, int csb, int B, int Hh, int Wh, f16 *cat, hipStream_t stream, int a_div = 1);
diff --git a/inconsistencymasks_amd/csrc/imk_elem.hip b/inconsistencymasks_amd/csrc/imk_elem.hip
--- a/inconsistencymasks_amd/csrc/imk_elem.hip
+++ b/inconsistencymasks_amd/csrc/imk_elem.hip
@@ -479,24 +479,49 @@
     ctl->good_steps = 0;
     ctl->step = 0;
     ctl->found_inf = 0.f;
-}
-
-__global__ __launch_bounds__(256) void adamw_kernel(float *__restrict__ p, float *__restrict__ m, float *__restrict__ v,
-                                                    const float *__restrict__ g, long long n, const ImkCtl *__restrict__ ctl,
-                                                    const float *__restrict__ stats, float grad_scale, float lr, float wd,
-                                                    float b1, float b2, float eps) {
-    if (stats[1] != 0.f) return;
-    const long long i = (long long)blockIdx.x * 256 + threadIdx.x;
-    if (i >= n) return;
-    const float t = (float)(ctl->step + 1);
+    ctl->ticket = 0;
+}
+
+__device__ __forceinline__ float adamw_update(float *__restrict__ p, float *__restrict__ m, float *__restrict__ v,
+                                              const float *__restrict__ g, long long i, int step, float grad_scale, float lr, float wd,
+                                              float b1, float b2, float eps) {
+#pragma clang fp contract(off)
+    const float t = (float)(step + 1);
     const float lr_t = lr * sqrtf(1.0f - powf(b2, t)) / (1.0f - powf(b1, t));
     const float gi = g[i] * grad_scale;
     float pi = p[i];
-    pi -= wd * pi;
+    pi = __builtin_fmaf(-wd, pi, pi);
     const float mi = b1 * m[i] + (1.0f - b1) * gi;
     const float vi = b2 * v[i] + (1.0f - b2) * gi * gi;
     pi -= lr_t * mi / (sqrtf(vi) + eps);
     p[i] = pi; m[i] = mi; v[i] = vi;
+    return pi;
+}
+
+__global__ __launch_bounds__(256) void adamw_kernel(float *__restrict__ p, float *__restrict__ m, float *__restrict__ v,
+                                                    const float *__restrict__ g, long long n, ImkCtl *ctl, const float *stats,
+                                                    float grad_scale, float lr, float wd, float b1, float b2, float eps,
+                                                    const uint32_t *__restrict__ slot_begin, const uint32_t *__restrict__ slots,
+                                                    f16 *__restrict__ packed) {
+    const long long i = (long long)blockIdx.x * 256 + threadIdx.x;
+    if (stats[1] == 0.f && i < n) {
+        const float pi = adamw_update(p, m, v, g, i, ctl->step, grad_scale, lr, wd, b1, b2, eps);
+        if (slot_begin) {
+            const f16 h = (f16)pi;
+            const uint32_t s1 = slot_begin[i + 1];
+            for (uint32_t s = slot_begin[i]; s < s1; ++s) packed[slots[s]] = h;
+        }
+    }
+    if (!slot_begin) return;
+    __syncthreads();
+    if (threadIdx.x == 0) {
+        __threadfence();
+        if (atomicAdd(&ctl->ticket, 1u) == gridDim.x - 1) {
+            __threadfence();
+            ctl->ticket = 0;
+            imk_ctl_end_step(ctl, stats);
+        }
+    }
 }
 
 __global__ __launch_bounds__(256) void concat_pool_kernel(const f16 *__restrict__ za, const float *__restrict__ sca,
@@ -868,7 +893,19 @@
 int imk_launch_adamw(float *p, float *m, float *v, const float *g, long long n, ImkCtl *ctl, const float *stats,
                      float grad_scale, float lr, float wd, float b1, float b2, float eps, hipStream_t stream) {
     ImkProfScope prof(PF_STEP_TAIL, (double)n * 28, stream);
-    imk_klaunch(adamw_kernel, dim3((int)((n + 255) / 256)), dim3(256), 0, stream, p, m, v, g, n, ctl, stats, grad_scale, lr, wd, b1, b2, eps);
+    imk_klaunch(adamw_kernel, dim3((int)((n + 255) / 256)), dim3(256), 0, stream, p, m, v, g, n, ctl, stats, grad_scale, lr, wd, b1, b2, eps,
+                (const uint32_t *)nullptr, (const uint32_t *)nullptr, (f16 *)nullptr);
+    IMK_LAUNCH_CHECK();
+    return IMK_OK;
+}
+
+int imk_launch_adamw_pack(float *p, float *m, float *v, const float *g, long long n, ImkCtl *ctl, const float *stats,
+                          float grad_scale, float lr, float wd, float b1, float b2, float eps, const uint32_t *slot_begin,
+                          const uint32_t *slots, long long n_slots, f16 *packed, hipStream_t stream) {
+    IMK_CHECK_ARG(n > 0 && slot_begin && slots && packed);
+    ImkProfScope prof(PF_STEP_TAIL, (double)n * 32 + (double)n_slots * 6, stream);
+    imk_klaunch(adamw_kernel, dim3((int)((n + 255) / 256)), dim3(256), 0, stream, p, m, v, g, n, ctl, stats, grad_scale, lr, wd,
+                b1, b2, eps, slot_begin, slots, packed);
     IMK_LAUNCH_CHECK();
     return IMK_OK;
 }
diff --git a/inconsistencymasks_amd/csrc/imk_kernels.h b/inconsistencymasks_amd/csrc/imk_kernels.h
--- a/inconsistencymasks_amd/csrc/imk_kernels.h
+++ b/inconsistencymasks_amd/csrc/imk_kernels.h
@@ -1,4 +1,7 @@
 #pragma once
+#include <functional>
+#include <string>
+#include <vector>
 #include "imk_common.h"
 
 enum ImkLoadMode {
@@ -135,6 +138,11 @@
     const float *stats;
 };
 int imk_launch_pack_jobs(const ImkPackJobs &jobs, hipStream_t stream);
+void imk_pack_inverse_cached(const std::string &key, const std::function<bool(std::vector<uint32_t> &, std::vector<uint32_t> &)> &build,
+                             uint32_t **begin, uint32_t **slots, int64_t *n_slots);
+long long imk_pack_slot_source_host(int ksize, int cin, int cout, int transposed, int pair, long long i);
+void imk_pack_inverse_add(int ksize, int cin, int cout, int transposed, int pair, int64_t w_off, int64_t dst_half, uint32_t *count_or_cursor,
+                          uint32_t *slots);
 
 #define IMK_WGF_MAX_JOBS 32
 struct ImkWgFinalJob {
diff --git a/inconsistencymasks_amd/csrc/imk_net.h b/inconsistencymasks_amd/csrc/imk_net.h
--- a/inconsistencymasks_amd/csrc/imk_net.h
+++ b/inconsistencymasks_amd/csrc/imk_net.h
@@ -4,6 +4,7 @@
 #include <cstring>
 #include <mutex>
 #include <new>
+#include <vector>
 #include "imk_elem.h"
 #include "imk_kernels.h"
 #include "imk_plan.h"
@@ -536,6 +537,51 @@
     return true;
 }
 
+template <typename Fn>
+inline void for_each_pack_job(const ImkLayer &l, Fn &&fn) {
+    if (l.kind != 0 || (l.flags & IMK_LF_DENSE)) return;
+    for (int tr = 0; tr < 3; ++tr) {
+        if (tr == 0 && (l.flags & IMK_LF_HEAD)) continue;
+        if (tr == 2 && (l.pk_chain < 0 || (l.flags & IMK_LF_HEAD))) continue;
+        const int pair = tr == 2 ? (imk_conv_pair_layout(l.cin, l.cout, false) && l.cin <= 8)
+                                 : (tr ? imk_conv_pair_layout(l.cout, l.cin, false) : imk_conv_pair_layout(l.cin, l.cout, l.lmode == LM_U8));
+        fn(l, tr, pair, tr == 2 ? l.pk_chain : (tr ? l.pk_bwd : l.pk_fwd));
+    }
+}
+
+inline bool build_pack_inverse(const imk_unet_plan *plan, std::vector<uint32_t> &begin, std::vector<uint32_t> &slots) {
+    const size_t n = (size_t)plan->n_trainable;
+    if (plan->packed_bytes / 2 >= (int64_t)1 << 32) return false;
+    begin.assign(n + 1, 0);
+    for (const ImkLayer &l : plan->layers)
+        for_each_pack_job(l, [&](const ImkLayer &ll, int tr, int pair, int64_t off) {
+            imk_pack_inverse_add(ll.ksize, ll.cin, ll.cout, tr, pair, ll.off_w + 1, off / 2, begin.data(), nullptr);
+        });
+    for (size_t i = 0; i < n; ++i) begin[i + 1] += begin[i];
+    slots.assign(begin[n], 0);
+    std::vector<uint32_t> cursor(begin.begin(), begin.end() - 1);
+    for (const ImkLayer &l : plan->layers)
+        for_each_pack_job(l, [&](const ImkLayer &ll, int tr, int pair, int64_t off) {
+            imk_pack_inverse_add(ll.ksize, ll.cin, ll.cout, tr, pair, ll.off_w, off / 2, cursor.data(), slots.data());
+        });
+    return true;
+}
+
+inline bool ensure_pack_inverse(const imk_unet_plan *plan) {
+    std::call_once(plan->inv_once, [plan]() {
+        int dev = 0;
+        (void)hipGetDevice(&dev);
+        std::string key = std::to_string(dev) + ":" + std::to_string(plan->n_trainable) + ":" + std::to_string(plan->packed_bytes);
+        for (const ImkLayer &l : plan->layers)
+            for (int64_t v : {(int64_t)l.kind, (int64_t)l.ksize, (int64_t)l.cin, (int64_t)l.cout, l.off_w, l.pk_fwd, l.pk_bwd, l.pk_chain,
+                              (int64_t)l.flags, (int64_t)l.lmode})
+                key += "," + std::to_string(v);
+        imk_pack_inverse_cached(key, [plan](std::vector<uint32_t> &b, std::vector<uint32_t> &s) { return build_pack_inverse(plan, b, s); },
+                                &plan->inv_begin, &plan->inv_slots, &plan->inv_n_slots);
+    });
+    return plan->inv_begin != nullptr;
+}
+
 inline int pack_weights(const imk_unet_plan *plan, const float *params, void *packed, hipStream_t stream, ImkCtl *ctl,
                         const float *stats, bool fold_bn) {
     IMK_CHECK_ARG(plan && params && packed);
@@ -547,16 +593,13 @@
     for (size_t i = 0; i < plan->layers.size(); ++i) {
         const ImkLayer &l = plan->layers[i];
         if (l.kind == 0) {
-            if (l.flags & IMK_LF_DENSE) continue;
-            for (int tr = 0; tr < 3; ++tr) {
-                if (tr == 0 && (l.flags & IMK_LF_HEAD)) continue;
-                if (tr == 2 && (l.pk_chain < 0 || (l.flags & IMK_LF_HEAD))) continue;
-                f16 *dst = (f16 *)(pk + (tr == 2 ? l.pk_chain : (tr ? l.pk_bwd : l.pk_fwd)));
-                const int pair = tr == 2 ? (imk_conv_pair_layout(l.cin, l.cout, false) && l.cin <= 8)
-                                         : (tr ? imk_conv_pair_layout(l.cout, l.cin, false) : imk_conv_pair_layout(l.cin, l.cout, l.lmode == LM_U8));
-                pj.j[pj.n++] = ImkPackJob{params + l.off_w, dst, l.ksize, l.cin, l.cout, tr, pair};
-                if (pj.n == IMK_PACK_MAX_JOBS) { int rc = flush_pack(); if (rc) return rc; }
-            }
+            int rc = IMK_OK;
+            for_each_pack_job(l, [&](const ImkLayer &ll, int tr, int pair, int64_t off) {
+                if (rc) return;
+                pj.j[pj.n++] = ImkPackJob{params + ll.off_w, (f16 *)(pk + off), ll.ksize, ll.cin, ll.cout, tr, pair};
+                if (pj.n == IMK_PACK_MAX_JOBS) rc = flush_pack();
+            });
+            if (rc) return rc;
         } else {
             if (fj.n == IMK_FOLD_MAX_JOBS) return IMK_EUNSUPPORTED;
             fj.j[fj.n++] = ImkFoldJob{params + l.off_w, params + l.off_b, params + l.off_mean, params + l.off_var,
diff --git a/inconsistencymasks_amd/csrc/imk_plan.h b/inconsistencymasks_amd/csrc/imk_plan.h
--- a/inconsistencymasks_amd/csrc/imk_plan.h
+++ b/inconsistencymasks_amd/csrc/imk_plan.h
@@ -44,6 +44,9 @@
     mutable hipEvent_t ev_join[MAX_SIDE] = {};
     mutable hipEvent_t ev_ring[128] = {};
     mutable bool side_ok = false;
+    mutable std::once_flag inv_once;
+    mutable uint32_t *inv_begin = nullptr, *inv_slots = nullptr;
+    mutable int64_t inv_n_slots = 0;
     bool dbg_materialize = false, dbg_single_stream = false;
     float bn_momentum = 0.99f;
     int find(const char *name) const {
diff --git a/inconsistencymasks_amd/csrc/imk_stage.h b/inconsistencymasks_amd/csrc/imk_stage.h
--- a/inconsistencymasks_amd/csrc/imk_stage.h
+++ b/inconsistencymasks_amd/csrc/imk_stage.h
@@ -35,6 +35,62 @@
     if (nc8 <= IMK_PASS_CAP) return nc8;
     const int n_pass = imk_cdiv_d(nc8, IMK_PASS_CAP);
     return imk_cdiv_d(nc8, n_pass);
+}
+
+__host__ __device__ inline long long imk_pack_slots(int ksize, int cin, int cout, int transposed, int pair) {
+    if (transposed == 2) return 512;
+    const int T = ksize == 3 ? 9 : 1;
+    const int m_dim = transposed ? cin : cout, k_dim = transposed ? cout : cin;
+    const int nc8 = ((k_dim + 7) & ~7) / 8;
+    if (pair) return (long long)(T == 9 ? 3 * nc8 : (nc8 + 1) / 2) * 512;
+    const int nc8p = imk_pass_chunks(nc8);
+    const int ns = imk_cdiv_d(nc8, nc8p) * ((T * nc8p + 3) / 4);
+    return (long long)((m_dim + 15) / 16) * ns * 512;
+}
+__host__ __device__ inline long long imk_pack_slot_source(int ksize, int cin, int cout, int transposed, int pair, int i) {
+    const int j = i & 7, lane = (i >> 3) & 63;
+    const int m = lane & 15, g = lane >> 4;
+    if (transposed == 2) {
+        if (!pair) {
+            const int ci = 4 * g + j;
+            return (j < 4 && ci < cin && m < cout) ? (long long)ci * cout + m : -1;
+        }
+        const int ci = 4 * (g & 1) + j, co = m & 7;
+        return (j < 4 && (m >> 3) == (g >> 1) && ci < cin && co < cout) ? (long long)ci * cout + co : -1;
+    }
+    const int T = ksize == 3 ? 9 : 1;
+    const int m_dim = transposed ? cin : cout, k_dim = transposed ? cout : cin;
+    const int nc8 = ((k_dim + 7) & ~7) / 8;
+    int tap, mi, ki;
+    if (pair && T == 9) {
+        const int st = i >> 9;
+        const int q = 4 * st + g;
+        const int ut = q / nc8, c8 = q - ut * nc8;
+        const int r = ut / 3, c = ut - 3 * r, ky = r - (m >> 3);
+        mi = m & 7; ki = c8 * 8 + j;
+        if (!(ky >= 0 && ky <= 2 && mi < m_dim && ki < k_dim)) return -1;
+        tap = ky * 3 + c;
+    } else if (pair) {
+        const int nq = T * nc8;
+        const int st = i >> 9;
+        const int q = 2 * st + (g & 1);
+        tap = q / nc8;
+        const int c8 = q - tap * nc8;
+        mi = m & 7; ki = c8 * 8 + j;
+        if (!(q < nq && (m >> 3) == (g >> 1) && mi < m_dim && ki < k_dim)) return -1;
+    } else {
+        const int nc8p = imk_pass_chunks(nc8), nsp = (T * nc8p + 3) / 4;
+        const int ns = imk_cdiv_d(nc8, nc8p) * nsp;
+        const int cs = i >> 9;
+        const int s = cs % ns, ct = cs / ns;
+        const int pass = s / nsp, q = 4 * (s - pass * nsp) + g;
+        tap = q / nc8p;
+        const int c8 = pass * nc8p + (q - tap * nc8p);
+        mi = ct * 16 + m; ki = c8 < nc8 ? c8 * 8 + j : k_dim;
+        if (!(tap < T && mi < m_dim && ki < k_dim)) return -1;
+    }
+    if (!transposed) return ((long long)tap * cin + ki) * cout + mi;
+    return ((long long)(T - 1 - tap) * cin + mi) * cout + ki;
 }
 
 __device__ __forceinline__ unsigned fast_div(unsigned n, unsigned d, float inv_d) {
diff --git a/inconsistencymasks_amd/csrc/imk_switches.cpp b/inconsistencymasks_amd/csrc/imk_switches.cpp
--- a/inconsistencymasks_amd/csrc/imk_switches.cpp
+++ b/inconsistencymasks_amd/csrc/imk_switches.cpp
@@ -30,6 +30,7 @@
         v.student_fused = on_unless_zero("IMK_STUDENT_FUSED");
         v.consistency_fused = on_unless_zero("IMK_CONSISTENCY_FUSED");
         v.select_shared = on_unless_zero("IMK_SELECT_SHARED");
+        v.adamw_pack = on_unless_zero("IMK_ADAMW_PACK");
         const int n = int_or("IMK_SIDE_STREAMS", 1);
         v.side_streams = n < 0 ? 0 : (n > imk_unet_plan::MAX_SIDE ? imk_unet_plan::MAX_SIDE : n);
         return v;
diff --git a/inconsistencymasks_amd/csrc/imk_switches.h b/inconsistencymasks_amd/csrc/imk_switches.h
--- a/inconsistencymasks_amd/csrc/imk_switches.h
+++ b/inconsistencymasks_amd/csrc/imk_switches.h
@@ -15,6 +15,7 @@
     bool student_fused;
     bool consistency_fused;
     bool select_shared;
+    bool adamw_pack;
     int side_streams;
 };
 
diff --git a/inconsistencymasks_amd/csrc/imk_unet.hip b/inconsistencymasks_amd/csrc/imk_unet.hip
--- a/inconsistencymasks_amd/csrc/imk_unet.hip
+++ b/inconsistencymasks_amd/csrc/imk_unet.hip
@@ -1,5 +1,6 @@
 #include <atomic>
 #include <cstdio>
+#include <map>
 #include "imk_net.h"
 #include "imk_head.h"
 #include "imk_switches.h"
@@ -181,6 +182,28 @@
     return pool.s[i];
 }
 
+void imk_pack_inverse_cached(const std::string &key, const std::function<bool(std::vector<uint32_t> &, std::vector<uint32_t> &)> &build,
+                             uint32_t **begin, uint32_t **slots, int64_t *n_slots) {
+    struct Entry { uint32_t *begin = nullptr, *slots = nullptr; int64_t n = 0; };
+    static std::mutex mu;
+    static std::map<std::string, Entry> cache;
+    std::lock_guard<std::mutex> lock(mu);
+    auto it = cache.find(key);
+    if (it == cache.end()) {
+        std::vector<uint32_t> b, s;
+        if (!build(b, s)) return;
+        uint32_t *dev = nullptr;
+        if (hipMalloc(&dev, (b.size() + s.size() + 1) * sizeof(uint32_t)) != hipSuccess) return;
+        if (hipMemcpy(dev, b.data(), b.size() * sizeof(uint32_t), hipMemcpyHostToDevice) != hipSuccess ||
+            (!s.empty() && hipMemcpy(dev + b.size(), s.data(), s.size() * sizeof(uint32_t), hipMemcpyHostToDevice) != hipSuccess)) {
+            (void)hipFree(dev);
+            return;
+        }
+        it = cache.emplace(key, Entry{dev, dev + b.size(), (int64_t)s.size()}).first;
+    }
+    *begin = it->second.begin; *slots = it->second.slots; *n_slots = it->second.n;
+}
+
 extern "C" int imk_runtime_warnings(void) { return g_runtime_warnings.load(); }
 
 extern "C" int imk_unet_plan_side_stream(const imk_unet_plan *plan, int i, void **stream_out) {
@@ -259,6 +282,29 @@
     IMK_CHECK_ARG(plan && params && packed);
     IMK_HIP(hipMemsetAsync(packed, 0, (size_t)plan->packed_bytes, (hipStream_t)stream_));
     return pack_weights(plan, params, packed, (hipStream_t)stream_, nullptr, nullptr, true);
+}
+
+extern "C" int64_t imk_unet_pack_maps(const imk_unet_plan *plan, int32_t *forward, uint32_t *begin, uint32_t *slots, int64_t slots_cap) {
+    if (!plan) return IMK_EINVAL;
+    std::vector<uint32_t> b, s;
+    if (!build_pack_inverse(plan, b, s)) return IMK_EUNSUPPORTED;
+    if (forward) {
+        for (int64_t i = 0; i < plan->packed_bytes / 2; ++i) forward[i] = -1;
+        for (const ImkLayer &l : plan->layers)
+            for_each_pack_job(l, [&](const ImkLayer &ll, int tr, int pair, int64_t off) {
+                const long long total = (long long)imk_packed_conv_halfs(ll.ksize, ll.cin, ll.cout, tr, pair != 0);
+                for (long long i = 0; i < total; ++i) {
+                    const long long src = imk_pack_slot_source_host(ll.ksize, ll.cin, ll.cout, tr, pair, i);
+                    if (src >= 0) forward[off / 2 + i] = (int32_t)(ll.off_w + src);
+                }
+            });
+    }
+    if (begin) memcpy(begin, b.data(), b.size() * sizeof(uint32_t));
+    if (slots) {
+        if (slots_cap < (int64_t)s.size()) return IMK_EINVAL;
+        if (!s.empty()) memcpy(slots, s.data(), s.size() * sizeof(uint32_t));
+    }
+    return (int64_t)s.size();
 }
 
 extern "C" int64_t imk_unet_workspace_bytes(const imk_unet_plan *plan, int batch, int mode) {
@@ -880,6 +926,9 @@
                                    float beta1, float beta2, float eps, void *stream_) {
     IMK_CHECK_ARG(plan && params && packed && state && grads && stats);
     const StateView sv = state_view(plan, state);
+    if (imk_switches().adamw_pack && ensure_pack_inverse(plan))
+        return imk_launch_adamw_pack(params, sv.m, sv.v, grads, plan->n_trainable, sv.ctl, stats, grad_scale, lr, wd, beta1, beta2, eps,
+                                     plan->inv_begin, plan->inv_slots, plan->inv_n_slots, (f16 *)packed, (hipStream_t)stream_);
     int rc = imk_launch_adamw(params, sv.m, sv.v, grads, plan->n_trainable, sv.ctl, stats, grad_scale, lr, wd, beta1, beta2,
                               eps, (hipStream_t)stream_);
     if (rc) return rc;
```

New measurement: 25050 images/s. 1.0% lower.
